# nirschl-lab/stain2stain

Hardware: AMD Instinct MI355X
Metric: paired 256x256 stain tiles/sec (full CFM optimisation step) (higher is better)
Workload: dtype bf16

## Files before the change

include/stain2stain_hip.h:

```cpp
#ifndef STAIN2STAIN_HIP_H
#define STAIN2STAIN_HIP_H

#ifdef __cplusplus
extern "C" {
#endif

#define S2S_OK 0
#define S2S_ERR_SHAPE (-1)
#define S2S_ERR_ALIGN (-2)
#define S2S_ERR_DTYPE (-3)
#define S2S_ERR_LAUNCH (-4)
#define S2S_ERR_NULL (-5)

#define S2S_BF16 0
#define S2S_F32 1

int s2s_conv3x3_stat_blocks(int dtype, int B, int H, int W, int Cout);
int s2s_conv3x3_nhwc(int dtype, const void* x0, int ld0, int c0, const void* x1, int ld1, int c1,
                     const void* w_packed, const float* bias, void* y, int ldy, float* stat_part,
                     const float* ep_scale, const float* ep_shift, int relu, int B, int H, int W, int Cout,
                     void* stream);

int s2s_conv3x3_ksplit(int dtype, int B, int H, int W, int Cout, int cin);
int s2s_conv3x3_nhwc_k(int dtype, const void* x0, int ld0, int c0, const void* x1, int ld1, int c1,
                       const void* w_packed, const float* bias, void* y, int ldy, float* stat_part,
                       const float* ep_scale, const float* ep_shift, int relu, float* kwork, int B, int H, int W,
                       int Cout, void* stream);
int s2s_conv3x3_stat_rows(int dtype, int B, int H, int W, int Cout, int c0, int c1, int ld0, int ld1, int has_bias);
int s2s_conv3x3_staged(int dtype, int B, int H, int W, int Cout, int c0, int c1, int ld0, int ld1, int ldy, int stats);
int s2s_conv3x3_family(int dtype, int B, int H, int W, int Cout, int c0, int c1, int ld0, int ld1, int ldy, int has_bias,
                       int has_affine, int stats, int stat_rows, int kwork);
int s2s_conv3x3_nhwc_s(int dtype, const void* x0, int ld0, int c0, const void* x1, int ld1, int c1, const void* w_packed,
                       const float* bias, void* y, int ldy, float* stat_part, int stat_rows, const float* ep_scale,
                       const float* ep_shift, int relu, float* kwork, int B, int H, int W, int Cout, void* stream);
int s2s_debug_conv_clock(long* out_host, int n);

int s2s_conv3x3_wgrad_splits(int dtype, int B, int H, int W, int Cin, int Cout);
int s2s_conv3x3_wgrad_nhwc(int dtype, const void* dy, int lddy, int Cout, const void* x0, int ld0, int c0,
                           const void* x1, int ld1, int c1, float* part, float* grad_oihw, int accumulate,
                           int B, int H, int W, void* stream);
int s2s_conv3x3_wgrad_phase(int dtype, const void* dy, int lddy, int Cout, const void* x0, int ld0, int c0,
                            const void* x1, int ld1, int c1, float* part, float* grad_oihw, int accumulate,
                            int B, int H, int W, int phases, void* stream);

int s2s_stem_stat_blocks(int B, int H, int W);
int s2s_stem_conv3x3_fwd(int dtype, const float* x_nchw, const float* w_oihw, const float* bias, void* y, int ldy,
                         float* stat_part, int B, int H, int W, int Cin, int Cout, void* stream);
int s2s_stem_wgrad_blocks(int B, int H, int W);
int s2s_stem_conv3x3_wgrad(int dtype, const void* dy, int lddy, const float* x_nchw, float* part, float* dw_oihw,
                           float* dbias, int accumulate, int B, int H, int W, int Cin, int Cout, void* stream);
int s2s_head_conv1x1_fwd(int dtype, const void* x, int ldx, const float* w, const float* bias, float* y_nchw, int B,
                         int H, int W, int C, int Cout, void* stream);
int s2s_head_wgrad_blocks(int B, int H, int W);
int s2s_head_conv1x1_bwd(int dtype, const float* dy_nchw, const void* x, int ldx, const float* w, void* dx, int lddx,
                         float* part, float* dw, float* dbias, int accumulate, int B, int H, int W, int C, int Cout,
                         void* stream);

int s2s_head_loss_blocks(int B, int H, int W);
int s2s_head_loss_fused(int dtype, const void* x, int ldx, const float* w, const float* bias, const float* u_nchw,
                        float* v_nchw, void* dx, int lddx, float grad_scale, float* part, double* lpart, float* dw,
                        float* dbias, float* loss, int accumulate, int B, int H, int W, int C, int Cout, void* stream);

int s2s_bn_finalize(const float* part, int nblk, int C, long count, const float* gamma, const float* beta,
                    float* running_mean, float* running_var, long* num_batches_tracked, float momentum, float eps,
                    float* mean, float* invstd, float* scale, float* shift, void* stream);
int s2s_bn_finalize_b(const float* part, int nblk, int C, long count, const float* gamma, const float* beta,
                      float* running_mean, float* running_var, long* num_batches_tracked, float momentum, float eps,
                      float* mean, float* invstd, float* scale, float* shift, const float* conv_bias, void* stream);
int s2s_bn_eval_prepare(int C, const float* gamma, const float* beta, const float* running_mean,
                        const float* running_var, float eps, float* scale, float* shift, void* stream);
int s2s_bn_relu_apply(int dtype, const void* x, int ldx, const float* scale, const float* shift, void* y, int ldy,
                      void* pool, int ldp, int B, int H, int W, int C, void* stream);
int s2s_maxpool2(int dtype, const void* x, int ldx, void* pool, int ldp, int B, int H, int W, int C, void* stream);
int s2s_bn_bwd_blocks(int B, int H, int W, int C);
int s2s_bn_relu_bwd(int dtype, const void* g1, int ldg1, const void* gp, int ldgp, const float* scale,
                    const float* shift, const void* x, int ldx, const float* mean, const float* invstd, const float* gamma, float* dgamma,
                    float* dbeta, float* dbias_conv, int accumulate, void* dx, int lddx, float* work, int B, int H,
                    int W, int C, void* stream);
int s2s_bn_partial_sums(const float* part, int nblk, int C, float* sums, void* stream);
int s2s_bn_relu_bwd_phase(int dtype, const void* g1, int ldg1, const void* gp, int ldgp, const float* scale,
                          const float* shift, const void* x, int ldx, const float* mean, const float* invstd,
                          const float* gamma, float* dgamma, float* dbeta, float* dbias_conv, int accumulate, void* dx,
                          int lddx, float* work, int B, int H, int W, int C, long count_total, int phases, void* stream);

int s2s_upsample2x_bilinear_ac_fwd(int dtype, const void* x, int ldx, const float* bias_nc, void* y, int ldy, int B,
                                   int Hin, int Win, int Hout, int Wout, int C, void* stream);
int s2s_upsample2x_bilinear_ac_bwd(int dtype, const void* dy, int lddy, void* dx, int lddx, int B, int Hin, int Win,
                                   int Hout, int Wout, int C, void* stream);
int s2s_pixel_sum(int dtype, const void* x, int ldx, float* out_nc, int B, int HW, int C, int accumulate,
                  void* stream);

int s2s_time_embedding(const float* t, float* out, int B, int dim, void* stream);
int s2s_linear_fwd(const float* x, const float* w, const float* bias, float* y, int B, int K, int N, void* stream);
int s2s_linear_bwd(const float* dy, const float* x, const float* w, float* dx, float* dw, float* db, int accumulate,
                   int B, int K, int N, void* stream);
int s2s_silu_fwd(const float* h, float* a, int n, void* stream);
int s2s_silu_bwd(const float* h, const float* da, float* dh, int n, void* stream);
int s2s_cfm_sample(const float* x0, const float* x1, const float* t, const float* eps, float sigma, float* xt,
                   float* ut, int B, long per_sample, void* stream);
int s2s_mse_loss(const float* v, const float* u, float* dv, float grad_scale, float* loss, double* work, long count,
                 void* stream);
int s2s_ode_error_norm(const float* e, const float* y0, const float* y1, float atol, float rtol, float* out,
                       double* work, long n, void* stream);
int s2s_axpy(float* x, const float* y, float a, long n, void* stream);
int s2s_dp_partials(long n);
int s2s_dp_init(int phase, const float* y, const float* k1, const float* fa, double* state, double* part, float* out,
                float* t_out, int* status, float atol, float rtol, int B, long n, void* stream);
int s2s_dp_stage(int i, const float* y, const float* k1, const float* k2, const float* k3, const float* k4,
                 const float* k5, const float* k6, const double* state, float* out, float* t_out, int B, long n,
                 void* stream);
int s2s_dp_error(const float* k1, const float* k2, const float* k3, const float* k4, const float* k5, const float* k6,
                 const float* k7, const float* y, const float* y_new, const double* state, double* part, float atol,
                 float rtol, int B, long n, void* stream);
int s2s_dp_control(double* state, const double* part, int* status, int max_steps, int B, long n, void* stream);
int s2s_dp_commit(float* y, const float* y_new, float* k1, const float* k7, const double* state, int B, long n,
                  void* stream);
int s2s_rk_stage(const float* x, const float* k1, const float* k2, const float* k3, float c1, float c2, float c3, int nk,
                 float* out, float* t_out, const float* table, const int* counter, int stages, int stage, int table_len,
                 int B, long n, void* stream);
int s2s_rk_combine(float* x, const float* k1, const float* k2, const float* k3, const float* k4, float c1, float c2,
                   float c3, float c4, int nk, int* counter, int B, long n, void* stream);
int s2s_fill_f32(float* x, float v, long n, void* stream);
int s2s_euler_tick(float* t, int n, const float* table, int* counter, void* stream);

int s2s_adam_step(float* p, const float* g, float* m, float* v, long n, int step, float lr, float beta1, float beta2,
                  float eps, float weight_decay, float grad_scale, void* stream);
int s2s_adam_step_dev(float* p, const float* g, float* m, float* v, long n, const float* hyper, void* stream);
long s2s_adam_multi_blocks(long n);
int s2s_adam_multi(const void* desc, int ntensors, long total, int step, float lr, float beta1, float beta2, float eps,
                   float weight_decay, float grad_scale, void* stream);
int s2s_adam_ema_step(float* p, const float* g, float* m, float* v, float* ema, long n, int step, float lr, float beta1,
                      float beta2, float eps, float weight_decay, float grad_scale, float ema_weight, void* stream);
int s2s_adam_ema_step_dev(float* p, const float* g, float* m, float* v, float* ema, long n, const float* hyper,
                          const float* ema_weight, void* stream);
long s2s_ema_multi_blocks(long n);
int s2s_ema_multi(const void* desc, int ntensors, long total, const float* weight, void* stream);
long s2s_pack_conv3x3_fwd_elems(int Cout, int Cin);
long s2s_pack_conv3x3_dgrad_elems(int Cout, int Cin);
int s2s_pack_conv3x3(int dtype, const float* w_oihw, void* w_fwd, void* w_dgrad, int Cout, int Cin, void* stream);
int s2s_pack_conv3x3_batched(int dtype, const void* desc, int nlayers, long total, void* stream);
int s2s_nchw_to_nhwc(int dtype, const float* x_nchw, void* y, int ldy, int B, int C, int H, int W, void* stream);
int s2s_nhwc_to_nchw(int dtype, const void* x, int ldx, float* y_nchw, int accumulate, int B, int C, int H, int W,
                     void* stream);

int s2s_paired_crop_flip_normalize(const void* src_u8, const void* tgt_u8, const int* params, float* out_src,
                                   float* out_tgt, int B, int Hs, int Ws, int S, void* stream);
int s2s_pil_resize_bilinear_normalize(const void* src_u8, void* tmp_u8, const int* bounds_h, const int* kk_h,
                                      int ksize_h, const int* bounds_v, const int* kk_v, int ksize_v, void* out_u8,
                                      float* out_f, int B, int Hs, int Ws, int Ho, int Wo, void* stream);

int s2s_region_gather(const void* img_u8, long pitch, int H, int W, int band_top, int band_h, const int* origins,
                      float* out, int B, int T, void* stream);
int s2s_region_blend(const float* tiles, int c0, const float* tiles1, int c1, const int* origins, int n, int T,
                     int overlap, float* acc, int band_rows, int H, int W, int r0, int r1, void* stream);
int s2s_region_finalize(float* acc, int band_rows, int W, int C, int r0, int r1, void* out_u8, long pitch_u8,
                        float* out_f, long pitch_f, int out_top, void* stream);

int s2s_region_tissue_count(const void* img_u8, long pitch, int H, int W, int band_top, int band_h, const int* origins,
                            int n, int T, int white, int black, int* counts, void* stream);
int s2s_region_skip_weight(const int* origins, int n, int T, int overlap, float* ws, int band_rows, int H, int W,
                           int r0, int r1, void* stream);
int s2s_region_finalize_mixed(float* acc, float* ws, int band_rows, int W, int C, int r0, int r1, const void* src_u8,
                              long src_pitch, int src_top, void* out_u8, long pitch_u8, float* out_f, long pitch_f,
                              int out_top, void* stream);

int s2s_seg_loss(const float* z, const float* g, float* dz, float* out, double* work, long n, float smooth,
                 float dice_weight, float grad_scale, void* stream);
int s2s_seg_loss_multiclass(const float* z, const long* target, float* dz, float* out, double* work, long B, long HW,
                            int C, int ignore_index, float smooth, float dice_weight, float grad_scale, void* stream);

int s2s_seg_eval_binary(const float* z, const float* g, float* out, long* counts, double* work, long n, float smooth,
                        float dice_weight, void* stream);
int s2s_seg_eval_multiclass(const float* z, const long* target, float* out, long* counts, double* work, long B,
                            long HW, int C, int ignore_index, float smooth, float dice_weight, void* stream);
int s2s_head_mse_eval_blocks(int B, int H, int W, int C);
int s2s_head_mse_eval(int dtype, const void* x, int ldx, const float* w, const float* bias, const float* u_nchw,
                      float* loss, double* lpart, int B, int H, int W, int C, int Cout, void* stream);

int s2s_image_quality_blocks(int H, int W, int win);
int s2s_image_quality_f32(const float* a, const float* b, int B, int C, int H, int W, int quantize, int win,
                          const float* taps, float k1, float k2, double* part, void* stream);
int s2s_image_quality_u8(const void* a, long pitch_a, long img_a, const void* b, long pitch_b, long img_b, int B,
                         int band_top, int band_h, int H, int W, int by0, int nby, int win, const float* taps, float k1,
                         float k2, double* part, void* stream);
int s2s_image_quality_finalize(const double* part, int B, int C, int H, int W, int win, float range, float* out,
                               void* stream);

int s2s_stain_quant_chunks(int cell_h, int cell_w);
int s2s_stain_quant_u8(const void* a, long pitch_a, long img_a, const void* b, long pitch_b, long img_b, int paired,
                       int B, int band_top, int band_h, int H, int W, int cell_h, int cell_w, int g0, int ng,
                       const float* od_table, const float* unmix, int white, int black, int stain, double* part,
                       void* stream);
int s2s_stain_quant_f32(const float* a, const float* b, int paired, int B, int H, int W, const float* od_table,
                        const float* unmix, int white, int black, int stain, double* part, void* stream);
int s2s_stain_quant_finalize(const double* part, long owners, int nchunk, int paired, long* counts, double* sums,
                             float* out, void* stream);
int s2s_stain_separate(const void* img, int is_f32, long pitch, long img_stride, int B, int H, int W,
                       const float* od_table, const float* unmix, float* out, void* stream);

int s2s_weighted_mse(const float* v, const float* u, const float* mask, float* dv, float* out, double* work, long B,
                     int C, long HW, float roi_lambda, float grad_scale, void* stream);
int s2s_charbonnier_roi(const float* pred, const float* truth, const float* mask, float* out, double* work, long B,
                        int C, long HW, float eps_charb, float eps_area, void* stream);
int s2s_class_embed_add(const float* temb, const float* table, const long* y, float* out, int B, int dim,
                        void* stream);
int s2s_class_embed_bwd(const float* dout, const long* y, float* dtable, int accumulate, int B, int dim,
                        int num_classes, void* stream);

int s2s_instnorm_blocks(int B, int H, int W, int C);
int s2s_instnorm_lrelu_fwd(int dtype, const void* x, int ldx, const float* gamma, const float* beta, void* y, int ldy,
                           float* work, float* stats, int B, int H, int W, int C, float eps, float slope,
                           void* stream);
int s2s_instnorm_lrelu_bwd(int dtype, const void* g, int ldg, const void* x, int ldx, const float* stats, void* dx,
                           int lddx, float* dgamma, float* dbeta, int accumulate, float* work, int B, int H, int W,
                           int C, float slope, void* stream);

int s2s_conv2x2_stat_blocks(int B, int H, int W, int Cout);
int s2s_conv2x2_nhwc(int dtype, const void* x, int ldx, int cin, const void* w_packed, const float* bias, void* y,
                     int ldy, float* stat_part, int B, int H, int W, int Cout, int pad, void* stream);
int s2s_space_to_depth_pad1(int dtype, const void* x, int ldx, void* xs, int ldxs, int inverse, int B, int H, int W,
                            int C, void* stream);
int s2s_channel_sum_blocks(long npix, int C);
int s2s_channel_sum(int dtype, const void* x, int ldx, float* work, float* out, long npix, int C, int accumulate,
                    void* stream);
int s2s_pack_conv4x4(const float* w_oihw, void* wf, void* wd, int Cout, int Cin, int stride, void* stream);
int s2s_conv4x4s1_nhwc(int dtype, const void* x, int ldx, int cin, const void* w_packed, const float* bias, void* y,
                       int ldy, float* stat_part, int B, int H, int W, int Cout, int pad, void* stream);
int s2s_conv4x4s1_wgrad_splits(int B, int H, int W, int Cin, int Cout);
int s2s_conv4x4s1_wgrad_nhwc(int dtype, const void* dy, int lddy, int Cout, const void* x, int ldx, int cin,
                             float* part, float* grad16, int accumulate, int B, int H, int W, void* stream);
int s2s_conv2x2_wgrad_splits(int B, int H, int W, int Cin, int Cout);
int s2s_conv2x2_wgrad_nhwc(int dtype, const void* dy, int lddy, int Cout, const void* x, int ldx, int cin, float* part,
                           float* grad2, int accumulate, int B, int H, int W, void* stream);

int s2s_convkxk_stat_blocks(int dtype, int B, int H, int W, int Cout, int ks);
int s2s_convkxk_nhwc(int dtype, const void* x, int ldx, int cin, const void* w_packed, const float* bias, int bias_mod,
                     void* y, int ldy, void* y2, int ldy2, int act, float act_slope, float* stat_part, float* kwork, int B,
                     int H, int W, int Cout, int ks, int pad, void* stream);
int s2s_convkxk_ksplit(int dtype, int B, int H, int W, int Cout, int cin, int ks);
int s2s_convkxk_wgrad_splits(int dtype, int B, int H, int W, int Cin, int Cout, int ks);
int s2s_convkxk_wgrad_nhwc(int dtype, const void* dy, int lddy, int Cout, const void* x, int ldx, int cin, float* part,
                           float* grad, int layout, int accumulate, int B, int H, int W, int ks, int x_plain, void* stream);
int s2s_conv4x4s2_ksplit(int B, int H, int W, int Cout, int Cin);
int s2s_conv4x4s2_nhwc(int dtype, const void* x, int ldx, int Cin, const void* wf, const float* bias, void* y, int ldy,
                       void* y2, int ldy2, int act, float act_slope, float* kwork, int B, int H, int W, int Cout,
                       void* stream);
int s2s_convt4x4s2_ksplit(int B, int h, int w, int C, int Cin);
int s2s_convt4x4s2_nhwc(int dtype, const void* x, int ldx, int Cin, const void* wd, const float* bias, void* y, int ldy,
                        float* kwork, int B, int h, int w, int C, void* stream);
int s2s_convsm_ok(int dtype, int mode, int B, int h, int w, int Cin, int Cout);
int s2s_convsm_nhwc(int dtype, int mode, const void* x, int ldx, int Cin, const void* w_packed, const float* bias, int epi,
                    int act, float slope, float eps, void* raw, int ldraw, void* y, int ldy, void* y2, int ldy2,
                    float* stats, const float* stats_in, const void* z, int ldz, const void* g2, int ldg2, int bwd_c0,
                    int B, int h, int w, int Cout, void* stream);
int s2s_instnorm_lrelu_fwd2(int dtype, const void* x, int ldx, const float* gamma, const float* beta, void* y, int ldy,
                            void* y2, int ldy2, float* work, float* stats, int B, int H, int W, int C, float eps,
                            float slope, void* stream);
int s2s_instnorm_lrelu_bwd2(int dtype, const void* g, int ldg, const void* g2, int ldg2, const void* x, int ldx,
                            const float* stats, void* dx, int lddx, float* dgamma, float* dbeta, int accumulate,
                            float* work, int B, int H, int W, int C, float slope, void* stream);
int s2s_instnorm_split_ok(int dtype, int H, int W, int C);
int s2s_instnorm_lrelu_fwd_split(int dtype, const float* slabs, int S, const float* bias, void* raw, int ldraw, void* y,
                                 int ldy, void* y2, int ldy2, float* stats, int B, int H, int W, int C, float eps,
                                 float slope, void* stream);
int s2s_instnorm_lrelu_bwd_split(int dtype, const float* gslabs, int S, const void* g2, int ldg2, const void* x, int ldx,
                                 const float* stats, void* dx, int lddx, int B, int H, int W, int C, float slope,
                                 void* stream);
int s2s_pack_conv4x4_t(int dtype, const float* w_oihw, void* wf, void* wd, int Cout, int Cin, int stride, void* stream);
long s2s_pack_conv4x4_blocks(int Cout, int Cin, int stride);
int s2s_pack_conv4x4_batched(int dtype, const void* desc, int nlayers, long total, void* stream);
int s2s_p2p_pack_input(int dtype, const float* a_nchw, int ca, const float* b_nchw, int cb, void* out, int ldo, int B,
                       int H, int W, void* stream);
int s2s_p2p_unpack(int dtype, const void* in, int ldi, int c0, int C, float* out_nchw, int B, int H, int W, void* stream);
int s2s_p2p_tanh_l1_blocks(int B, int H, int W);
int s2s_p2p_tanh_l1_fwd(int dtype, const void* h, int ldh, const float* src_nchw, const float* tgt_nchw, void* d_in,
                        int ldd, float* fake_nchw, float* l1_out, void* work, int B, int H, int W, int C, void* stream);
int s2s_p2p_tanh_l1_bwd(int dtype, const void* h, int ldh, const float* tgt_nchw, const void* gd, int ldg, float l1_scale,
                        void* dh, int lddh, int B, int H, int W, int C, void* stream);
int s2s_p2p_bce_logits(int dtype, const void* z, int ldz, int n_real, float w_real, float w_fake, void* dz, int lddz,
                       float* out2, int N, int HW, void* stream);
int s2s_p2p_bce_blocks(int N, int HW);
int s2s_p2p_bce_logits_w(int dtype, const void* z, int ldz, int n_real, float w_real, float w_fake, void* dz, int lddz,
                         float* out2, double* work, int N, int HW, void* stream);
int s2s_p2p_act_bwd_blocks(long npix, int C);
int s2s_p2p_act_bwd(int dtype, const void* g, int ldg, const void* g2, int ldg2, const void* a, int lda, float slope,
                    void* dz, int lddz, float* work, float* dbias, int accumulate, long npix, int C, void* stream);

int s2s_stream_create_cu_mask(const unsigned* mask_words, int n_words, long* out_stream);
int s2s_stream_destroy(void* stream);
int s2s_event_create(int timing_only, long* out_event);
int s2s_event_record(void* event, void* stream);
int s2s_event_elapsed_ms(void* start, void* stop, float* out_ms);
int s2s_event_synchronize(void* event);
int s2s_event_destroy(void* event);

#ifdef __cplusplus
}
#endif
#endif
```

stain2stain_amd/csrc/conv_edge.hip:

```cpp
#include "common.h"

namespace {

constexpr int STEM_MAX_CIN = 8;

typedef __attribute__((address_space(3))) s16x4 lds_s16x4;

__device__ __forceinline__ bf16x8 tr_frag8(const char* p) {
  s16x4 lo = __builtin_amdgcn_ds_read_tr16_b64_v4i16((lds_s16x4*)(p));
  s16x4 hi = __builtin_amdgcn_ds_read_tr16_b64_v4i16((lds_s16x4*)(p + 4 * 64));
  bf16x4 l4 = __builtin_bit_cast(bf16x4, lo), h4 = __builtin_bit_cast(bf16x4, hi);
  bf16x8 r;
#pragma unroll
  for (int i = 0; i < 4; ++i) { r[i] = l4[i]; r[4 + i] = h4[i]; }
  return r;
}

template <int NIMG>
__device__ __forceinline__ void split_store(char* base, int img_stride, int off, const float* v8) {
  bf16x8 h, m, l;
#pragma unroll
  for (int i = 0; i < 8; ++i) {
    h[i] = (bf16_t)v8[i];
    const float r1 = v8[i] - (float)h[i];
// ... 302 lines not shown
        for (int k = 0; k < 8; ++k) ab[k] = (bf16_t)a.v[k];
        *reinterpret_cast<bf16x8*>(al + threadIdx.x * AS + c8) = ab;
#pragma unroll
        for (int o = 0; o < HEAD_MAX_COUT; ++o)
          if (o < Cout)
#pragma unroll
            for (int k = 0; k < 8; ++k) vv[o] = fmaf(a.v[k], wl[o * C + c8 + k], vv[o]);
      }
      const long n = p / HW, q = p - n * HW;
#pragma unroll
      for (int o = 0; o < HEAD_MAX_COUT; ++o)
        if (o < Cout) {
          const float vo = vv[o] + (bias ? bias[o] : 0.f);
          const long idx = (n * Cout + o) * HW + q;
          if (v_out) v_out[idx] = vo;
          const float d = vo - u[idx];
          lsum += (double)(d * d);
          g[o] = coef * d;
        }
      for (int c8 = 0; c8 < C; c8 += 8) {
        f32x8 da;
#pragma unroll
        for (int k = 0; k < 8; ++k) {
          float s = 0.f;
#pragma unroll
          for (int o = 0; o < HEAD_MAX_COUT; ++o)
            if (o < Cout) s = fmaf(g[o], wl[o * C + c8 + k], s);
          da.v[k] = s;
        }
        store8(dx + p * lddx + c8, da);
      }
    } else {
      for (int c8 = 0; c8 < C; c8 += 8) {
        bf16x8 z;
#pragma unroll
        for (int k = 0; k < 8; ++k) z[k] = (bf16_t)0.f;
        *reinterpret_cast<bf16x8*>(al + threadIdx.x * AS + c8) = z;
      }
    }
#pragma unroll
    for (int o = 0; o < HEAD_MAX_COUT; ++o) gl[threadIdx.x * HEAD_MAX_COUT + o] = g[o];
    __syncthreads();
#pragma unroll
    for (int i = 0; i < 4; ++i) {
      const int id = threadIdx.x + i * 256;
      if (id < nout) {
        const int o = id / (C + 1), c = id - o * (C + 1);
        float a = acc[i];
        if (c < C) for (int pp = 0; pp < 256; ++pp) a = fmaf(gl[pp * HEAD_MAX_COUT + o], (float)al[pp * AS + c], a);
        else for (int pp = 0; pp < 256; ++pp) a += gl[pp * HEAD_MAX_COUT + o];
        acc[i] = a;
      }
    }
    __syncthreads();
  }
#pragma unroll
  for (int i = 0; i < 4; ++i) {
    const int id = threadIdx.x + i * 256;
    if (id < nout) part[(long)blockIdx.x * nout + id] = acc[i];
  }
  lred[threadIdx.x] = lsum;
  __syncthreads();
  for (int o = 128; o > 0; o >>= 1) {
    if (threadIdx.x < o) lred[threadIdx.x] += lred[threadIdx.x + o];
    __syncthreads();
  }
  if (threadIdx.x == 0) lpart[blockIdx.x] = lred[0];
}

template <typename T, int PCB>
__global__ __launch_bounds__(256) void head_loss_lanes_kernel(const T* __restrict__ x, int ldx,
                                                              const float* __restrict__ w,
                                                              const float* __restrict__ bias,
                                                              const float* __restrict__ u, float* __restrict__ v_out,
                                                              T* __restrict__ dx, int lddx, float coef,
                                                              float* __restrict__ part, double* __restrict__ lpart,
                                                              long npix, int HW, int Cout) {
  constexpr int C = PCB * 8, PPB = 256 / PCB, MO = HEAD_MAX_COUT;
  __shared__ float fold[256][MO * 8 + 1];
  __shared__ float dbf[PPB][MO];
  __shared__ double lred[256];
  const int tid = threadIdx.x, pc = tid & (PCB - 1), slot = tid / PCB;
  const int lane = tid & 63, grp0 = lane & ~(PCB - 1);
  float wr[MO][8], bo[MO];
#pragma unroll
  for (int o = 0; o < MO; ++o) {
    bo[o] = (o < Cout && bias) ? bias[o] : 0.f;
#pragma unroll
    for (int k = 0; k < 8; ++k) wr[o][k] = o < Cout ? w[o * C + pc * 8 + k] : 0.f;
  }
  float dwacc[MO][8], dbacc[MO];
#pragma unroll
  for (int o = 0; o < MO; ++o) {
    dbacc[o] = 0.f;
#pragma unroll
    for (int k = 0; k < 8; ++k) dwacc[o][k] = 0.f;
  }
  double lsum = 0.0;
  const int np = (int)npix, stride = (int)gridDim.x * PPB;
  f32x8 a_next;
  {
    const int pf = (int)blockIdx.x * PPB + slot;
#pragma unroll
    for (int k = 0; k < 8; ++k) a_next.v[k] = 0.f;
    if (pf < np) a_next = load8(x + (long)pf * ldx + pc * 8);
  }
  for (int p0 = (int)blockIdx.x * PPB; p0 < np; p0 += stride) {
    const int p = p0 + slot;
    const bool ok = p < np;
    const f32x8 a = a_next;
    {
      const int pn = p + stride;
#pragma unroll
      for (int k = 0; k < 8; ++k) a_next.v[k] = 0.f;
      if (p0 + stride < np && pn < np) a_next = load8(x + (long)pn * ldx + pc * 8);
    }
    float vv[MO];
#pragma unroll
    for (int o = 0; o < MO; ++o) {
      float t = 0.f;
#pragma unroll
      for (int k = 0; k < 8; ++k) t = fmaf(a.v[k], wr[o][k], t);
#pragma unroll
      for (int m = 1; m < PCB; m <<= 1) t += __shfl_xor(t, m, 64);
      vv[o] = t + bo[o];
    }
    const int n = p / HW, q = p - n * HW;
    float gm[MO];
#pragma unroll
    for (int o = 0; o < MO; ++o) {
      gm[o] = 0.f;
      if (ok && o < Cout && (o & (PCB - 1)) == pc) {
        const long idx = ((long)n * Cout + o) * HW + q;
        if (v_out) v_out[idx] = vv[o];
        const float d = vv[o] - u[idx];
        lsum += (double)(d * d);
        gm[o] = coef * d;
      }
    }
    float g[MO];
#pragma unroll
    for (int o = 0; o < MO; ++o) g[o] = __shfl(gm[o], grp0 + (o & (PCB - 1)), 64);
    if (ok) {
      f32x8 da;
#pragma unroll
      for (int k = 0; k < 8; ++k) {
        float t = 0.f;
#pragma unroll
        for (int o = 0; o < MO; ++o) t = fmaf(g[o], wr[o][k], t);
        da.v[k] = t;
      }
      store8(dx + (long)p * lddx + pc * 8, da);
    }
#pragma unroll
    for (int o = 0; o < MO; ++o) {
      if (pc == 0) dbacc[o] += g[o];
#pragma unroll
      for (int k = 0; k < 8; ++k) dwacc[o][k] = fmaf(g[o], a.v[k], dwacc[o][k]);
    }
  }
#pragma unroll
  for (int o = 0; o < MO; ++o) {
#pragma unroll
    for (int k = 0; k < 8; ++k) fold[tid][o * 8 + k] = dwacc[o][k];
    if (pc == 0) dbf[slot][o] = dbacc[o];
  }
  lred[tid] = lsum;
  __syncthreads();
  const int nout = Cout * (C + 1);
  for (int id = tid; id < nout; id += 256) {
    const int o = id / (C + 1), c = id - o * (C + 1);
    float t = 0.f;
    if (c < C) {
      const int cp = c >> 3, k = c & 7;
      for (int sl = 0; sl < PPB; ++sl) t += fold[sl * PCB + cp][o * 8 + k];
    } else {
      for (int sl = 0; sl < PPB; ++sl) t += dbf[sl][o];
    }
    part[(long)blockIdx.x * nout + id] = t;
  }
  for (int o = 128; o > 0; o >>= 1) {
    if (tid < o) lred[tid] += lred[tid + o];
    __syncthreads();
  }
  if (tid == 0) lpart[blockIdx.x] = lred[0];
}

template <typename T, int PCB, bool FWD>
__global__ __launch_bounds__(256) void head_lanes_kernel(const T* __restrict__ x, int ldx, const float* __restrict__ w,
                                                         const float* __restrict__ bias, const float* __restrict__ dy,
                                                         float* __restrict__ v_out, T* __restrict__ dx, int lddx,
                                                         float* __restrict__ part, long npix, int HW, int Cout) {
  constexpr int C = PCB * 8, PPB = 256 / PCB, MO = HEAD_MAX_COUT;
  __shared__ float fold[FWD ? 1 : 256][MO * 8 + 1];
  __shared__ float dbf[PPB][MO];
  const int tid = threadIdx.x, pc = tid & (PCB - 1), slot = tid / PCB;
  const int lane = tid & 63, grp0 = lane & ~(PCB - 1);
  float wr[MO][8], bo[MO];
#pragma unroll
  for (int o = 0; o < MO; ++o) {
    bo[o] = (o < Cout && bias) ? bias[o] : 0.f;
#pragma unroll
    for (int k = 0; k < 8; ++k) wr[o][k] = o < Cout ? w[o * C + pc * 8 + k] : 0.f;
  }
  float dwacc[MO][8], dbacc[MO];
#pragma unroll
  for (int o = 0; o < MO; ++o) {
    dbacc[o] = 0.f;
#pragma unroll
    for (int k = 0; k < 8; ++k) dwacc[o][k] = 0.f;
  }
  const int np = (int)npix, stride = (int)gridDim.x * PPB;
  f32x8 a_next;
  {
    const int pf = (int)blockIdx.x * PPB + slot;
#pragma unroll
    for (int k = 0; k < 8; ++k) a_next.v[k] = 0.f;
    if (pf < np) a_next = load8(x + (long)pf * ldx + pc * 8);
  }
  for (int p0 = (int)blockIdx.x * PPB; p0 < np; p0 += stride) {
    const int p = p0 + slot;
    const bool ok = p < np;
    const f32x8 a = a_next;
    {
      const int pn = p + stride;
#pragma unroll
      for (int k = 0; k < 8; ++k) a_next.v[k] = 0.f;
      if (p0 + stride < np && pn < np) a_next = load8(x + (long)pn * ldx + pc * 8);
    }
    const int n = p / HW, q = p - n * HW;
    if (FWD) {
#pragma unroll
      for (int o = 0; o < MO; ++o) {
        float t = 0.f;
#pragma unroll
        for (int k = 0; k < 8; ++k) t = fmaf(a.v[k], wr[o][k], t);
#pragma unroll
        for (int m = 1; m < PCB; m <<= 1) t += __shfl_xor(t, m, 64);
        if (ok && o < Cout && (o & (PCB - 1)) == pc) v_out[((long)n * Cout + o) * HW + q] = t + bo[o];
      }
    } else {
      float gm[MO], g[MO];
#pragma unroll
      for (int o = 0; o < MO; ++o) {
        gm[o] = 0.f;
        if (ok && o < Cout && (o & (PCB - 1)) == pc) gm[o] = dy[((long)n * Cout + o) * HW + q];
      }
#pragma unroll
      for (int o = 0; o < MO; ++o) g[o] = __shfl(gm[o], grp0 + (o & (PCB - 1)), 64);
      if (ok) {
        f32x8 da;
#pragma unroll
        for (int k = 0; k < 8; ++k) {
          float t = 0.f;
#pragma unroll
          for (int o = 0; o < MO; ++o) t = fmaf(g[o], wr[o][k], t);
          da.v[k] = t;
        }
        store8(dx + (long)p * lddx + pc * 8, da);
      }
#pragma unroll
      for (int o = 0; o < MO; ++o) {
        if (pc == 0) dbacc[o] += g[o];
#pragma unroll
        for (int k = 0; k < 8; ++k) dwacc[o][k] = fmaf(g[o], a.v[k], dwacc[o][k]);
      }
    }
  }
  if (FWD) return;
#pragma unroll
  for (int o = 0; o < MO; ++o) {
#pragma unroll
    for (int k = 0; k < 8; ++k) fold[tid][o * 8 + k] = dwacc[o][k];
    if (pc == 0) dbf[slot][o] = dbacc[o];
  }
  __syncthreads();
  const int nout = Cout * (C + 1);
  for (int id = tid; id < nout; id += 256) {
    const int o = id / (C + 1), c = id - o * (C + 1);
    float t = 0.f;
    if (c < C) {
      const int cp = c >> 3, k = c & 7;
      for (int sl = 0; sl < PPB; ++sl) t += fold[sl * PCB + cp][o * 8 + k];
    } else {
      for (int sl = 0; sl < PPB; ++sl) t += dbf[sl][o];
    }
    part[(long)blockIdx.x * nout + id] = t;
  }
}

template <typename T, bool FWD>
bool launch_head_lanes(const void* x, int ldx, const float* w, const float* bias, const float* dy, float* v, void* dx,
                       int lddx, float* part, int nb, long npix, int HW, int C, int Cout, hipStream_t s) {
  if (Cout > HEAD_MAX_COUT || (C % 8) || npix >= (1L << 31) - (1L << 20)) return false;
#define S2S_HLN(PP)                                                                                                  \
  hipLaunchKernelGGL((head_lanes_kernel<T, PP, FWD>), dim3(nb), dim3(256), 0, s, (const T*)x, ldx, w, bias, dy, v,   \
                     (T*)dx, lddx, part, npix, HW, Cout);                                                            \
  return true;
  switch (C / 8) {
    case 1: S2S_HLN(1) case 2: S2S_HLN(2) case 4: S2S_HLN(4) case 8: S2S_HLN(8) case 16: S2S_HLN(16) case 32: S2S_HLN(32)
    case 64: S2S_HLN(64) default: return false;
  }
#undef S2S_HLN
}

__global__ __launch_bounds__(256) void loss_finalize_kernel(const double* part, int n, double inv_count, float* loss) {
  __shared__ double red[256];
  double s = 0.0;
  for (int i = threadIdx.x; i < n; i += 256) s += part[i];
  red[threadIdx.x] = s;
  __syncthreads();
  for (int o = 128; o > 0; o >>= 1) {
    if (threadIdx.x < o) red[threadIdx.x] += red[threadIdx.x + o];
    __syncthreads();
  }
  if (threadIdx.x == 0) *loss = (float)(red[0] * inv_count);
}

}

int s2s_internal_stem_fwd(int dtype, const float* x_nchw, const float* w_oihw, const float* bias, void* y, int ldy,
                          float* stat_part, int B, int H, int W, int Cin, int Cout, hipStream_t s);

extern "C" int s2s_stem_stat_blocks(int B, int H, int W) {
  if (B <= 0 || H <= 0 || W <= 0) return S2S_ERR_SHAPE;
  return B * cdiv(H, 16) * cdiv(W, 16);
}

extern "C" int s2s_stem_conv3x3_fwd(int dtype, const float* x_nchw, const float* w_oihw, const float* bias, void* y,
                                    int ldy, float* stat_part, int B, int H, int W, int Cin, int Cout, void* stream) {
  if (!x_nchw || !w_oihw || !y) return S2S_ERR_NULL;
  if (B <= 0 || H <= 0 || W <= 0 || Cin <= 0 || Cin > 6 || Cout <= 0 || (Cout % 8) || (ldy % 8))
    return S2S_ERR_SHAPE;
  return s2s_internal_stem_fwd(dtype, x_nchw, w_oihw, bias, y, ldy, stat_part, B, H, W, Cin, Cout,
                               (hipStream_t)stream);
}

extern "C" int s2s_stem_wgrad_blocks(int B, int H, int W) {
  if (B <= 0 || H <= 0 || W <= 0) return S2S_ERR_SHAPE;
  const int nt = B * cdiv(H, 16) * cdiv(W, 16);
  constexpr int cap = 512;
  return nt < cap ? nt : cap;
}

extern "C" int s2s_stem_conv3x3_wgrad(int dtype, const void* dy, int lddy, const float* x_nchw, float* part,
                                      float* dw_oihw, float* dbias, int accumulate, int B, int H, int W, int Cin,
                                      int Cout, void* stream) {
  if (!dy || !x_nchw || !part || !dw_oihw) return S2S_ERR_NULL;
  if (B <= 0 || H <= 0 || W <= 0 || Cin <= 0 || Cin > 6 || Cout <= 0 || (Cout % 8) || (lddy % 8))
    return S2S_ERR_SHAPE;
  const int nb = s2s_stem_wgrad_blocks(B, H, W);
  hipStream_t s = (hipStream_t)stream;
  dim3 grid(nb, cdiv(Cout, 64), cdiv(Cin, 3));
  if (dtype == S2S_BF16) {
    const int lds = 1 * (2 * 256 * 64 + 256 * 64) + 3 * 324 * 4;
    hipLaunchKernelGGL(stem_wgrad_kernel<bf16_t>, grid, dim3(256), lds, s, (const bf16_t*)dy, lddy, x_nchw, part, B,
                       H, W, Cin, Cout, cdiv(H, 16), cdiv(W, 16));
  } else if (dtype == S2S_F32) {
    const int lds = 3 * (2 * 256 * 64 + 256 * 64) + 3 * 324 * 4;
    static unsigned long long attr_devs = 0;
    if (int rc = s2s_allow_dyn_lds(reinterpret_cast<const void*>(stem_wgrad_kernel<float>), lds, &attr_devs)) return rc;
    hipLaunchKernelGGL(stem_wgrad_kernel<float>, grid, dim3(256), lds, s, (const float*)dy, lddy, x_nchw, part, B, H,
                       W, Cin, Cout, cdiv(H, 16), cdiv(W, 16));
  } else return S2S_ERR_DTYPE;
  hipLaunchKernelGGL(stem_wgrad_reduce_kernel, dim3(Cout, cdiv(Cin, 3)), dim3(1024), 0, s, part, 2 * nb, Cout, Cin, dw_oihw, dbias,
                     accumulate);
  S2S_LAUNCH_CHECK();
  return S2S_OK;
}

extern "C" int s2s_head_conv1x1_fwd(int dtype, const void* x, int ldx, const float* w, const float* bias,
                                    float* y_nchw, int B, int H, int W, int C, int Cout, void* stream) {
  if (!x || !w || !y_nchw) return S2S_ERR_NULL;
  if (B <= 0 || H <= 0 || W <= 0 || C <= 0 || (C % 8) || (ldx % 8) || Cout <= 0 || Cout > HEAD_WIDE_COUT)
    return S2S_ERR_SHAPE;
  const long npix = (long)B * H * W;
  long grid = (npix + 255) / 256;
  if (grid > 4096) grid = 4096;
  hipStream_t s = (hipStream_t)stream;
  if (dtype != S2S_BF16 && dtype != S2S_F32) return S2S_ERR_DTYPE;
  {
    const int nbl = (int)(((npix + 255) / 256) < 2048 ? ((npix + 255) / 256) : 2048);
    const bool done = dtype == S2S_BF16
        ? launch_head_lanes<bf16_t, true>(x, ldx, w, bias, nullptr, y_nchw, nullptr, 8, nullptr, nbl, npix, H * W, C, Cout, s)
        : launch_head_lanes<float, true>(x, ldx, w, bias, nullptr, y_nchw, nullptr, 8, nullptr, nbl, npix, H * W, C, Cout, s);
    if (done) { S2S_LAUNCH_CHECK(); return S2S_OK; }
  }
#define S2S_HEAD_FWD(TT, MO)                                                                                        \
  hipLaunchKernelGGL((head_fwd_kernel<TT, MO>), dim3((int)grid), dim3(256), Cout * C * 4, s, (const TT*)x, ldx, w, \
                     bias, y_nchw, npix, H * W, C, Cout)
  if (dtype == S2S_BF16) { if (Cout <= 4) S2S_HEAD_FWD(bf16_t, 4); else S2S_HEAD_FWD(bf16_t, 8); }
  else if (dtype == S2S_F32) { if (Cout <= 4) S2S_HEAD_FWD(float, 4); else S2S_HEAD_FWD(float, 8); }
  else return S2S_ERR_DTYPE;
#undef S2S_HEAD_FWD
  S2S_LAUNCH_CHECK();
  return S2S_OK;
}

extern "C" int s2s_head_wgrad_blocks(int B, int H, int W) {
  if (B <= 0 || H <= 0 || W <= 0) return S2S_ERR_SHAPE;
  const long nb = ((long)B * H * W + 63) / 64;
  return (int)(nb < 512 ? nb : 512);
}

extern "C" int s2s_head_conv1x1_bwd(int dtype, const float* dy_nchw, const void* x, int ldx, const float* w, void* dx,
                                    int lddx, float* part, float* dw, float* dbias, int accumulate, int B, int H, int W,
                                    int C, int Cout, void* stream) {
  if (!dy_nchw || !x || !w || !dx || !part || !dw) return S2S_ERR_NULL;
  if (B <= 0 || H <= 0 || W <= 0 || C <= 0 || (C % 8) || (ldx % 8) || (lddx % 8) || Cout <= 0 || Cout > HEAD_WIDE_COUT)
    return S2S_ERR_SHAPE;
  if (Cout * (C + 1) > 2048) return S2S_ERR_SHAPE;
  const long npix = (long)B * H * W;
  long grid = (npix + 255) / 256;
  if (grid > 4096) grid = 4096;
  const int nb = s2s_head_wgrad_blocks(B, H, W);
  const int mo = Cout <= 4 ? 4 : 8;
  const int lds = (64 * (C + 1) + 64 * mo) * 4;
  hipStream_t s = (hipStream_t)stream;
  if (dtype != S2S_BF16 && dtype != S2S_F32) return S2S_ERR_DTYPE;
  {
    const bool done = dtype == S2S_BF16
        ? launch_head_lanes<bf16_t, false>(x, ldx, w, nullptr, dy_nchw, nullptr, dx, lddx, part, nb, npix, H * W, C, Cout, s)
        : launch_head_lanes<float, false>(x, ldx, w, nullptr, dy_nchw, nullptr, dx, lddx, part, nb, npix, H * W, C, Cout, s);
    if (done) {
      hipLaunchKernelGGL(head_wgrad_reduce_kernel, dim3(cdiv(Cout * (C + 1), 8)), dim3(256), 0, s, part, nb, Cout, C,
                         dw, dbias, accumulate);
      S2S_LAUNCH_CHECK();
      return S2S_OK;
    }
  }
#define S2S_HEAD_BWD(TT, MO)                                                                                       \
  hipLaunchKernelGGL((head_bwd_data_kernel<TT, MO>), dim3((int)grid), dim3(256), Cout * C * 4, s, dy_nchw, w,      \
                     (TT*)dx, lddx, npix, H * W, C, Cout);                                                         \
  hipLaunchKernelGGL((head_wgrad_kernel<TT, MO>), dim3(nb), dim3(256), lds, s, dy_nchw, (const TT*)x, ldx, part,   \
                     npix, H * W, C, Cout);
  if (dtype == S2S_BF16) { if (mo == 4) { S2S_HEAD_BWD(bf16_t, 4) } else { S2S_HEAD_BWD(bf16_t, 8) } }
  else if (dtype == S2S_F32) { if (mo == 4) { S2S_HEAD_BWD(float, 4) } else { S2S_HEAD_BWD(float, 8) } }
  else return S2S_ERR_DTYPE;
#undef S2S_HEAD_BWD
  hipLaunchKernelGGL(head_wgrad_reduce_kernel, dim3(cdiv(Cout * (C + 1), 8)), dim3(256), 0, s, part, nb, Cout, C,
                     dw, dbias, accumulate);
  S2S_LAUNCH_CHECK();
  return S2S_OK;
}

extern "C" int s2s_head_loss_blocks(int B, int H, int W) {
  if (B <= 0 || H <= 0 || W <= 0) return S2S_ERR_SHAPE;
  const long nb = ((long)B * H * W + 255) / 256;
  return (int)(nb < 1024 ? nb : 1024);
}

extern "C" int s2s_head_loss_fused(int dtype, const void* x, int ldx, const float* w, const float* bias,
                                   const float* u_nchw, float* v_nchw, void* dx, int lddx, float grad_scale,
                                   float* part, double* lpart, float* dw, float* dbias, float* loss, int accumulate,
                                   int B, int H, int W, int C, int Cout, void* stream) {
  if (!x || !w || !u_nchw || !dx || !part || !lpart || !dw || !loss) return S2S_ERR_NULL;
  if (B <= 0 || H <= 0 || W <= 0 || C <= 0 || (C % 8) || (ldx % 8) || (lddx % 8) || Cout <= 0 || Cout > HEAD_MAX_COUT)
    return S2S_ERR_SHAPE;
  if (Cout * (C + 1) > 1024) return S2S_ERR_SHAPE;
  const long npix = (long)B * H * W;
  if (npix >= (1L << 31) - (1L << 20)) return S2S_ERR_SHAPE;
  const double count = (double)npix * Cout;
  const int nb = s2s_head_loss_blocks(B, H, W);
  const int lds = (HEAD_MAX_COUT * C + 256 * HEAD_MAX_COUT) * 4 + 256 * (C + 8) * 2;
  if (lds > 60 * 1024) return S2S_ERR_SHAPE;
  hipStream_t s = (hipStream_t)stream;
  const float coef = (float)(2.0 * (double)grad_scale / count);
  if (dtype != S2S_BF16 && dtype != S2S_F32) return S2S_ERR_DTYPE;
  const int pcb = C / 8;
  bool done = false;
#define S2S_HL(TT, PP)                                                                                              \
  hipLaunchKernelGGL((head_loss_lanes_kernel<TT, PP>), dim3(nb), dim3(256), 0, s, (const TT*)x, ldx, w, bias, u_nchw, \
                     v_nchw, (TT*)dx, lddx, coef, part, lpart, npix, H * W, Cout);                                 \
  done = true;
#define S2S_HL_T(TT)                                                                                    \
  switch (pcb) {                                                                                        \
    case 1: { S2S_HL(TT, 1) } break;  case 2: { S2S_HL(TT, 2) } break;  case 4: { S2S_HL(TT, 4) } break;    \
    case 8: { S2S_HL(TT, 8) } break;  case 16: { S2S_HL(TT, 16) } break; case 32: { S2S_HL(TT, 32) } break;  \
    case 64: { S2S_HL(TT, 64) } break; default: break;                                                  \
  }
  if (dtype == S2S_BF16) { S2S_HL_T(bf16_t) } else { S2S_HL_T(float) }
#undef S2S_HL_T
#undef S2S_HL
  if (!done) {
    if (dtype == S2S_BF16)
      hipLaunchKernelGGL(head_loss_fused_kernel<bf16_t>, dim3(nb), dim3(256), lds, s, (const bf16_t*)x, ldx, w, bias,
                         u_nchw, v_nchw, (bf16_t*)dx, lddx, coef, part, lpart, npix, H * W, C, Cout);
    else
      hipLaunchKernelGGL(head_loss_fused_kernel<float>, dim3(nb), dim3(256), lds, s, (const float*)x, ldx, w, bias,
                         u_nchw, v_nchw, (float*)dx, lddx, coef, part, lpart, npix, H * W, C, Cout);
  }
  hipLaunchKernelGGL(head_wgrad_reduce_kernel, dim3(cdiv(Cout * (C + 1), 8)), dim3(256), 0, s, part, nb, Cout, C,
                     dw, dbias, accumulate);
  hipLaunchKernelGGL(loss_finalize_kernel, dim3(1), dim3(256), 0, s, lpart, nb, 1.0 / count, loss);
  S2S_LAUNCH_CHECK();
  return S2S_OK;
}
```

stain2stain_amd/csrc/norm_act.hip:

```cpp
#include "common.h"
#include <type_traits>

namespace {

constexpr int RED_ROWS = 8;

constexpr int PRE_R = 16;
__global__ __launch_bounds__(1024) void prereduce_rows_kernel(float* __restrict__ part, int nrows, int ncols) {
  __shared__ double s1[32][33];
  const int cl = threadIdx.x & 31, rg = threadIdx.x >> 5;
  const int c = blockIdx.x * 32 + cl, r = blockIdx.y;
  double a = 0.0;
  if (c < ncols)
    for (int i = r + PRE_R * rg; i < nrows; i += PRE_R * 32) a += (double)part[(long)i * ncols + c];
  s1[rg][cl] = a;
  __syncthreads();
  if (rg == 0 && c < ncols) {
    for (int k = 1; k < 32; ++k) a += s1[k][cl];
    part[(long)r * ncols + c] = (float)a;
  }
}

inline int prereduce(float* part, int nrows, int ncols, hipStream_t s) {
  if (nrows <= 4 * PRE_R) return nrows;
// ... 86 lines not shown
  const int cp = C >> 3;
  const int Hw = (H + 1) >> 1, Ww = (W + 1) >> 1, Hp = H >> 1, Wp = W >> 1;
  const long total = (long)B * Hw * Ww * cp;
  for (long i = (long)blockIdx.x * blockDim.x + threadIdx.x; i < total; i += (long)gridDim.x * blockDim.x) {
    const int c8 = (int)(i % cp) * 8;
    long t = i / cp;
    const int wx = (int)(t % Ww); t /= Ww;
    const int wy = (int)(t % Hw);
    const int n = (int)(t / Hw);
    float sc[8], sh[8], mx[8];
#pragma unroll
    for (int k = 0; k < 8; ++k) { sc[k] = scale[c8 + k]; sh[k] = shift[c8 + k]; mx[k] = 0.f; }
#pragma unroll
    for (int dy = 0; dy < 2; ++dy)
#pragma unroll
      for (int dx = 0; dx < 2; ++dx) {
        const int yy = wy * 2 + dy, xx = wx * 2 + dx;
        if (yy < H && xx < W) {
          const long pix = ((long)n * H + yy) * W + xx;
          f32x8 v = load8(x + pix * ldx + c8);
#pragma unroll
          for (int k = 0; k < 8; ++k) {
            v.v[k] = fmaxf(fmaf(v.v[k], sc[k], sh[k]), 0.f);
            const float st = to_f32(from_f32<T>(v.v[k]));
            mx[k] = fmaxf(mx[k], st);
          }
          store8(y + pix * ldy + c8, v);
        }
      }
    if (pool && wy < Hp && wx < Wp) {
      f32x8 m;
#pragma unroll
      for (int k = 0; k < 8; ++k) m.v[k] = mx[k];
      store8(pool + (((long)n * Hp + wy) * Wp + wx) * ldp + c8, m);
    }
  }
}

template <typename T>
__global__ void maxpool2_kernel(const T* __restrict__ x, int ldx, T* __restrict__ pool, int ldp, int B, int H,
                                int W, int C) {
  const int cp = C >> 3, Hp = H >> 1, Wp = W >> 1;
  const long total = (long)B * Hp * Wp * cp;
  for (long i = (long)blockIdx.x * blockDim.x + threadIdx.x; i < total; i += (long)gridDim.x * blockDim.x) {
    const int c8 = (int)(i % cp) * 8;
    long t = i / cp;
    const int wx = (int)(t % Wp); t /= Wp;
    const int wy = (int)(t % Hp);
    const int n = (int)(t / Hp);
    f32x8 m;
#pragma unroll
    for (int k = 0; k < 8; ++k) m.v[k] = -INFINITY;
#pragma unroll
    for (int dy = 0; dy < 2; ++dy)
#pragma unroll
      for (int dx = 0; dx < 2; ++dx) {
        const long pix = ((long)n * H + wy * 2 + dy) * W + wx * 2 + dx;
        const f32x8 v = load8(x + pix * ldx + c8);
#pragma unroll
        for (int k = 0; k < 8; ++k) m.v[k] = fmaxf(m.v[k], v.v[k]);
      }
    store8(pool + (((long)n * Hp + wy) * Wp + wx) * ldp + c8, m);
  }
}

typedef __attribute__((ext_vector_type(8))) float f32x8v;
template <typename T> struct Vec8;
template <> struct Vec8<bf16_t> { typedef bf16x8 type; };
template <> struct Vec8<float> { typedef f32x8v type; };

__device__ __forceinline__ bf16x8 vload8(const bf16_t* p) { return *reinterpret_cast<const bf16x8*>(p); }
__device__ __forceinline__ f32x8v vload8(const float* p) {
  const f32x4 a = *reinterpret_cast<const f32x4*>(p), b = *reinterpret_cast<const f32x4*>(p + 4);
  return __builtin_shufflevector(a, b, 0, 1, 2, 3, 4, 5, 6, 7);
}
__device__ __forceinline__ void vstore8(bf16_t* p, bf16x8 v) { *reinterpret_cast<bf16x8*>(p) = v; }
__device__ __forceinline__ void vstore8(float* p, f32x8v v) {
  *reinterpret_cast<f32x4*>(p) = __builtin_shufflevector(v, v, 0, 1, 2, 3);
  *reinterpret_cast<f32x4*>(p + 4) = __builtin_shufflevector(v, v, 4, 5, 6, 7);
}

template <typename T>
struct WindowGrad {
  typedef typename Vec8<T>::type V;
  V x0, x1, x2, x3, g0, g1v, g2, g3, pr;
  int okmask;
  __device__ __forceinline__ void load(const T* __restrict__ g1, int ldg1, const T* __restrict__ gp, int ldgp,
                                       const T* __restrict__ x, int ldx, int n, int wy, int wx, int H, int W,
                                       int c8) {
    const int Hp = H >> 1, Wp = W >> 1;
    const V zero = {};
    const int yy = wy * 2, xx = wx * 2;
    const bool r1 = yy + 1 < H, c1 = xx + 1 < W;
    okmask = 1 | (c1 ? 2 : 0) | (r1 ? 4 : 0) | ((r1 && c1) ? 8 : 0);
    const long p00 = ((long)n * H + yy) * W + xx;
    x0 = vload8(x + p00 * ldx + c8);
    x1 = c1 ? vload8(x + (p00 + 1) * ldx + c8) : zero;
    x2 = r1 ? vload8(x + (p00 + W) * ldx + c8) : zero;
    x3 = (r1 && c1) ? vload8(x + (p00 + W + 1) * ldx + c8) : zero;
    if (g1) {
      g0 = vload8(g1 + p00 * ldg1 + c8);
      g1v = c1 ? vload8(g1 + (p00 + 1) * ldg1 + c8) : zero;
      g2 = r1 ? vload8(g1 + (p00 + W) * ldg1 + c8) : zero;
      g3 = (r1 && c1) ? vload8(g1 + (p00 + W + 1) * ldg1 + c8) : zero;
    } else {
      g0 = zero; g1v = zero; g2 = zero; g3 = zero;
    }
    const bool pooled = gp && wy < Hp && wx < Wp;
    okmask |= pooled ? 16 : 0;
    pr = pooled ? vload8(gp + (((long)n * Hp + wy) * Wp + wx) * ldgp + c8) : zero;
  }
  __device__ __forceinline__ bool ok(int q) const { return (okmask >> q) & 1; }
  __device__ __forceinline__ void eval(int k, float sc, float sh, float mu, float is, float (&dz)[4],
                                       float (&xh)[4]) const {
    const float b[4] = {(float)x0[k], (float)x1[k], (float)x2[k], (float)x3[k]};
    dz[0] = (float)g0[k]; dz[1] = (float)g1v[k]; dz[2] = (float)g2[k]; dz[3] = (float)g3[k];
    float yv[4];
#pragma unroll
    for (int q = 0; q < 4; ++q) {
      yv[q] = ok(q) ? to_f32(from_f32<T>(fmaxf(fmaf(b[q], sc, sh), 0.f))) : 0.f;
      xh[q] = ok(q) ? (b[q] - mu) * is : 0.f;
    }
    if (okmask & 16) {
      int best = 0;
      float bv = yv[0];
#pragma unroll
      for (int q = 1; q < 4; ++q)
        if (yv[q] > bv) { bv = yv[q]; best = q; }
      const float p = (float)pr[k];
#pragma unroll
      for (int q = 0; q < 4; ++q) dz[q] += (q == best) ? p : 0.f;
    }
#pragma unroll
    for (int q = 0; q < 4; ++q)
      if (!(yv[q] > 0.f)) dz[q] = 0.f;
  }
};

__device__ __forceinline__ int pcb_of(int C) {
  int p = 1;
  while (p < 32 && p * 8 < C) p <<= 1;
  return p;
}

template <typename T>
__global__ __launch_bounds__(256) void bn_relu_bwd_reduce_kernel(const T* g1, int ldg1, const T* gp, int ldgp, const float* scale, const float* shift,
                                          const T* x, int ldx, const float* mean, const float* invstd,
                                          float* part, int B, int H, int W, int C) {
  const int Hw = (H + 1) >> 1, Ww = (W + 1) >> 1;
  const long nwin = (long)B * Hw * Ww;
  const int PCB = pcb_of(C), WL = 256 / PCB;
  const int pc = threadIdx.x & (PCB - 1), wl = threadIdx.x / PCB;
  const int c8 = (blockIdx.x * PCB + pc) * 8;
  using Acc = typename std::conditional<std::is_same<T, float>::value, double, float>::type;
  Acc s1[8], s2[8];
#pragma unroll
  for (int k = 0; k < 8; ++k) { s1[k] = 0; s2[k] = 0; }
  __shared__ float kc[4][256];
  for (int i = threadIdx.x; i < PCB * 8; i += 256) {
    const int c = blockIdx.x * PCB * 8 + i;
    const bool in = c < C;
    kc[0][i] = in ? scale[c] : 0.f; kc[1][i] = in ? shift[c] : 0.f;
    kc[2][i] = in ? mean[c] : 0.f;  kc[3][i] = in ? invstd[c] : 0.f;
  }
  __syncthreads();
  if (c8 < C) {
    for (int w = blockIdx.y * WL + wl; w < (int)nwin; w += gridDim.y * WL) {
      const int t1 = w / Ww, wx = w - t1 * Ww;
      const int n = t1 / Hw, wy = t1 - n * Hw;
      WindowGrad<T> wg;
      wg.load(g1, ldg1, gp, ldgp, x, ldx, n, wy, wx, H, W, c8);
#pragma unroll
      for (int k = 0; k < 8; ++k) {
        float dz[4], xh[4];
        const int ci = pc * 8 + k;
        wg.eval(k, kc[0][ci], kc[1][ci], kc[2][ci], kc[3][ci], dz, xh);
        float a = 0.f, b = 0.f;
#pragma unroll
        for (int q = 0; q < 4; ++q) { a += dz[q]; b += dz[q] * xh[q]; }
        s1[k] += (Acc)a;
        s2[k] += (Acc)b;
        __builtin_amdgcn_sched_barrier(0);
      }
    }
  }
  __shared__ Acc red[2][2304];
  const int rowlen = PCB * 8 + 1;
#pragma unroll
  for (int k = 0; k < 8; ++k) { red[0][wl * rowlen + pc * 8 + k] = s1[k]; red[1][wl * rowlen + pc * 8 + k] = s2[k]; }
  __syncthreads();
  for (int i = threadIdx.x; i < 2 * PCB * 8; i += 256) {
    const int which = i / (PCB * 8), cl = i - which * (PCB * 8);
    Acc s = 0;
    for (int r = 0; r < WL; ++r) s += red[which][r * rowlen + cl];
    const int c = blockIdx.x * PCB * 8 + cl;
    if (c < C) part[((long)which * C + c) * gridDim.y + blockIdx.y] = (float)s;
  }
}

template <int TPC>
__global__ __launch_bounds__(256) void bn_bwd_finalize_kernel(const float* part, int nblk, int C, double count, float* dgamma,
                                       float* dbeta, int accumulate, float* c1, float* c2, float* zero_out) {
  const int c = blockIdx.x * (256 / TPC) + threadIdx.x / TPC, li = threadIdx.x % TPC;
  if (c >= C) return;
  double a, b;
  channel_sums<TPC>(part, nblk, C, c, li, a, b);
  if (li == 0) {
    dbeta[c] = accumulate ? dbeta[c] + (float)a : (float)a;
    dgamma[c] = accumulate ? dgamma[c] + (float)b : (float)b;
    c1[c] = (float)(a / count);
    c2[c] = (float)(b / count);
    if (zero_out) zero_out[c] = 0.f;
  }
}

template <typename T>
__global__ __launch_bounds__(256) void bn_relu_bwd_apply_kernel(const T* g1, int ldg1, const T* gp, int ldgp, const float* scale, const float* shift,
                                         const T* x, int ldx, const float* mean, const float* invstd,
                                         const float* gamma, const float* c1, const float* c2, T* dx, int lddx,
                                         float* dxsum_part, int B, int H, int W, int C) {
  const int Hw = (H + 1) >> 1, Ww = (W + 1) >> 1;
  const long nwin = (long)B * Hw * Ww;
  const int PCB = pcb_of(C), WL = 256 / PCB;
  const int pc = threadIdx.x & (PCB - 1), wl = threadIdx.x / PCB;
  const int c8 = (blockIdx.x * PCB + pc) * 8;
  float s[8];
#pragma unroll
  for (int k = 0; k < 8; ++k) s[k] = 0.f;
  __shared__ float kc[7][256];
  for (int i = threadIdx.x; i < PCB * 8; i += 256) {
    const int c = blockIdx.x * PCB * 8 + i;
    const bool in = c < C;
    kc[0][i] = in ? scale[c] : 0.f; kc[1][i] = in ? shift[c] : 0.f;
    kc[2][i] = in ? mean[c] : 0.f;  kc[3][i] = in ? invstd[c] : 0.f;
    kc[4][i] = in ? gamma[c] * invstd[c] : 0.f;
    kc[5][i] = in ? c1[c] : 0.f;    kc[6][i] = in ? c2[c] : 0.f;
  }
  __syncthreads();
  if (c8 < C) {
    for (int w = blockIdx.y * WL + wl; w < (int)nwin; w += gridDim.y * WL) {
      const int t1 = w / Ww, wx = w - t1 * Ww;
      const int n = t1 / Hw, wy = t1 - n * Hw;
      WindowGrad<T> wg;
      wg.load(g1, ldg1, gp, ldgp, x, ldx, n, wy, wx, H, W, c8);
      typename Vec8<T>::type o0, o1, o2, o3;
#pragma unroll
      for (int k = 0; k < 8; ++k) {
        float dz[4], xh[4];
        const int ci = pc * 8 + k;
        wg.eval(k, kc[0][ci], kc[1][ci], kc[2][ci], kc[3][ci], dz, xh);
        const float gak = kc[4][ci], k1k = kc[5][ci], k2k = kc[6][ci];
        float v[4];
#pragma unroll
        for (int q = 0; q < 4; ++q) {
          v[q] = gak * (dz[q] - k1k - xh[q] * k2k);
          if (wg.ok(q)) s[k] += v[q];
        }
        o0[k] = from_f32<T>(v[0]); o1[k] = from_f32<T>(v[1]); o2[k] = from_f32<T>(v[2]); o3[k] = from_f32<T>(v[3]);
        __builtin_amdgcn_sched_barrier(0);
      }
      T* const d00 = dx + (((long)n * H + wy * 2) * W + wx * 2) * lddx + c8;
      vstore8(d00, o0);
      if (wg.ok(1)) vstore8(d00 + lddx, o1);
      if (wg.ok(2)) vstore8(d00 + (long)W * lddx, o2);
      if (wg.ok(3)) vstore8(d00 + (long)(W + 1) * lddx, o3);
    }
  }
  if (dxsum_part) {
    __shared__ float red[2304];
    const int rowlen = PCB * 8 + 1;
#pragma unroll
    for (int k = 0; k < 8; ++k) red[wl * rowlen + pc * 8 + k] = s[k];
    __syncthreads();
    for (int cl = threadIdx.x; cl < PCB * 8; cl += 256) {
      float t = 0.f;
      for (int r = 0; r < WL; ++r) t += red[r * rowlen + cl];
      const int c = blockIdx.x * PCB * 8 + cl;
      if (c < C) dxsum_part[(long)blockIdx.y * C + c] = t;
    }
  }
}

template <typename T>
__global__ __launch_bounds__(256) void bn_relu_bwd_reduce_flat_kernel(const T* __restrict__ g1, int ldg1, const float* __restrict__ scale, const float* __restrict__ shift,
                                               const T* __restrict__ x, int ldx, const float* mean, const float* invstd,
                                               float* part, long npix, int C) {
  const int PCB = pcb_of(C), WL = 256 / PCB;
  const int pc = threadIdx.x & (PCB - 1), wl = threadIdx.x / PCB;
  const int c8 = (blockIdx.x * PCB + pc) * 8;
  using Acc = typename std::conditional<std::is_same<T, float>::value, double, float>::type;
  Acc s1[8], s2[8];
#pragma unroll
  for (int k = 0; k < 8; ++k) { s1[k] = 0; s2[k] = 0; }
  if (c8 < C) {
    float mu[8], is[8], sc[8], sh[8];
#pragma unroll
    for (int k = 0; k < 8; ++k) { mu[k] = mean[c8 + k]; is[k] = invstd[c8 + k]; sc[k] = scale[c8 + k]; sh[k] = shift[c8 + k]; }
    for (long p = (long)blockIdx.y * WL + wl; p < npix; p += (long)gridDim.y * WL) {
      const f32x8 g = load8(g1 + p * ldg1 + c8);
      const f32x8 b = load8(x + p * ldx + c8);
#pragma unroll
      for (int k = 0; k < 8; ++k) {
        const float dz = fmaf(b.v[k], sc[k], sh[k]) > 0.f ? g.v[k] : 0.f;
        s1[k] += (Acc)dz;
        s2[k] += (Acc)(dz * ((b.v[k] - mu[k]) * is[k]));
      }
    }
  }
  __shared__ Acc red[2][2304];
  const int rowlen = PCB * 8 + 1;
#pragma unroll
  for (int k = 0; k < 8; ++k) { red[0][wl * rowlen + pc * 8 + k] = s1[k]; red[1][wl * rowlen + pc * 8 + k] = s2[k]; }
  __syncthreads();
  for (int i = threadIdx.x; i < 2 * PCB * 8; i += 256) {
    const int which = i / (PCB * 8), cl = i - which * (PCB * 8);
    Acc s = 0;
    for (int r = 0; r < WL; ++r) s += red[which][r * rowlen + cl];
    const int c = blockIdx.x * PCB * 8 + cl;
    if (c < C) part[((long)which * C + c) * gridDim.y + blockIdx.y] = (float)s;
  }
}

template <typename T>
__global__ __launch_bounds__(256) void bn_relu_bwd_apply_flat_kernel(const T* __restrict__ g1, int ldg1, const float* __restrict__ scale, const float* __restrict__ shift,
                                              const T* __restrict__ x, int ldx, const float* mean, const float* invstd,
                                              const float* gamma, const float* c1, const float* c2, T* __restrict__ dx,
                                              int lddx, float* dxsum_part, long npix, int C, int rev) {
  const int PCB = pcb_of(C), WL = 256 / PCB;
  const int pc = threadIdx.x & (PCB - 1), wl = threadIdx.x / PCB;
  const int c8 = (blockIdx.x * PCB + pc) * 8;
  float s[8];
#pragma unroll
  for (int k = 0; k < 8; ++k) s[k] = 0.f;
  if (c8 < C) {
    float ga[8], k1[8], k2[8], mu[8], is[8], sc[8], sh[8];
#pragma unroll
    for (int k = 0; k < 8; ++k) {
      mu[k] = mean[c8 + k]; is[k] = invstd[c8 + k]; sc[k] = scale[c8 + k]; sh[k] = shift[c8 + k];
      ga[k] = gamma[c8 + k] * is[k]; k1[k] = c1[c8 + k]; k2[k] = c2[c8 + k];
    }
    const long p0 = (long)blockIdx.y * WL + wl, pstep = (long)gridDim.y * WL;
    const long nit = p0 < npix ? (npix - p0 + pstep - 1) / pstep : 0;
    for (long it = 0; it < nit; ++it) {
      const long p = p0 + (rev ? nit - 1 - it : it) * pstep;
      const f32x8 g = load8(g1 + p * ldg1 + c8);
      const f32x8 b = load8(x + p * ldx + c8);
      f32x8 o;
#pragma unroll
      for (int k = 0; k < 8; ++k) {
        const float dz = fmaf(b.v[k], sc[k], sh[k]) > 0.f ? g.v[k] : 0.f;
        o.v[k] = ga[k] * (dz - k1[k] - ((b.v[k] - mu[k]) * is[k]) * k2[k]);
        s[k] += o.v[k];
      }
      store8(dx + p * lddx + c8, o);
    }
  }
  if (dxsum_part) {
    __shared__ float red[2304];
    const int rowlen = PCB * 8 + 1;
#pragma unroll
    for (int k = 0; k < 8; ++k) red[wl * rowlen + pc * 8 + k] = s[k];
    __syncthreads();
    for (int cl = threadIdx.x; cl < PCB * 8; cl += 256) {
      float t = 0.f;
      for (int r = 0; r < WL; ++r) t += red[r * rowlen + cl];
      const int c = blockIdx.x * PCB * 8 + cl;
      if (c < C) dxsum_part[(long)blockIdx.y * C + c] = t;
    }
  }
}

__global__ __launch_bounds__(1024) void colsum_finalize_kernel(const float* part, int nblk, int C, float* out, int accumulate) {
  __shared__ double s1[32][33];
  const int cl = threadIdx.x & 31, rg = threadIdx.x >> 5;
  const int c = blockIdx.x * 32 + cl;
  double a = 0.0;
  if (c < C)
    for (int i = rg; i < nblk; i += 32) a += (double)part[(long)i * C + c];
  s1[rg][cl] = a;
  __syncthreads();
  if (rg == 0 && c < C) {
    for (int k = 1; k < 32; ++k) a += s1[k][cl];
    out[c] = accumulate ? out[c] + (float)a : (float)a;
  }
}

inline int ew_grid(long total) {
  long b = (total + 255) / 256;
  if (b > 2048 * 4) b = 2048 * 4;
  if (b < 1) b = 1;
  return (int)b;
}

inline int host_pcb(int C) {
  int p = 1;
  while (p < 32 && p * 8 < C) p <<= 1;
  return p;
}

inline int red_blocks(int B, int H, int W, int C) {
  const long nwin = (long)B * ((H + 1) / 2) * ((W + 1) / 2);
  const int pcb = host_pcb(C), wl = 256 / pcb;
  long want = 1536 / cdiv(C / 8, pcb);
  if (want < 1) want = 1;
  long nb = (nwin + wl - 1) / wl;
  if (nb > want) nb = want;
  if (nb < 1) nb = 1;
  return (int)nb;
}

}

extern "C" int s2s_bn_finalize_b(const float* part, int nblk, int C, long count, const float* gamma,
                                 const float* beta, float* running_mean, float* running_var, long* num_batches,
                                 float momentum, float eps, float* mean, float* invstd, float* scale, float* shift,
                                 const float* conv_bias, void* stream) {
  if (!part || !gamma || !beta || !mean || !invstd || !scale || !shift) return S2S_ERR_NULL;
  if (nblk <= 0 || C <= 0 || count <= 0) return S2S_ERR_SHAPE;
  if (finalize_tpc(nblk) == 256)
    hipLaunchKernelGGL(bn_finalize_kernel<256>, dim3(C), dim3(256), 0, (hipStream_t)stream, part, nblk, C,
                       (double)count, gamma, beta, running_mean, running_var, num_batches, momentum, eps, mean,
                       invstd, scale, shift, conv_bias);
  else
    hipLaunchKernelGGL(bn_finalize_kernel<64>, dim3(cdiv(C, 4)), dim3(256), 0, (hipStream_t)stream, part, nblk, C,
                       (double)count, gamma, beta, running_mean, running_var, num_batches, momentum, eps, mean,
                       invstd, scale, shift, conv_bias);
  S2S_LAUNCH_CHECK();
  return S2S_OK;
}

extern "C" int s2s_bn_finalize(const float* part, int nblk, int C, long count, const float* gamma,
                               const float* beta, float* running_mean, float* running_var, long* num_batches,
                               float momentum, float eps, float* mean, float* invstd, float* scale, float* shift,
                               void* stream) {
  return s2s_bn_finalize_b(part, nblk, C, count, gamma, beta, running_mean, running_var, num_batches, momentum, eps, mean,
                           invstd, scale, shift, nullptr, stream);
}

extern "C" int s2s_bn_partial_sums(const float* part, int nblk, int C, float* sums, void* stream) {
  if (!part || !sums) return S2S_ERR_NULL;
  if (nblk <= 0 || C <= 0) return S2S_ERR_SHAPE;
  if (finalize_tpc(nblk) == 256)
    hipLaunchKernelGGL(bn_partial_sums_kernel<256>, dim3(C), dim3(256), 0, (hipStream_t)stream, part, nblk, C, sums);
  else
    hipLaunchKernelGGL(bn_partial_sums_kernel<64>, dim3(cdiv(C, 4)), dim3(256), 0, (hipStream_t)stream, part, nblk, C, sums);
  S2S_LAUNCH_CHECK();
  return S2S_OK;
}

extern "C" int s2s_bn_eval_prepare(int C, const float* gamma, const float* beta, const float* rmean,
                                   const float* rvar, float eps, float* scale, float* shift, void* stream) {
  if (!gamma || !beta || !rmean || !rvar || !scale || !shift) return S2S_ERR_NULL;
  if (C <= 0) return S2S_ERR_SHAPE;
  hipLaunchKernelGGL(bn_eval_prepare_kernel, dim3(cdiv(C, 256)), dim3(256), 0, (hipStream_t)stream, C, gamma, beta,
                     rmean, rvar, eps, scale, shift);
  S2S_LAUNCH_CHECK();
  return S2S_OK;
}

extern "C" int s2s_bn_relu_apply(int dtype, const void* x, int ldx, const float* scale, const float* shift, void* y,
                                 int ldy, void* pool, int ldp, int B, int H, int W, int C, void* stream) {
  if (!x || !scale || !shift || !y) return S2S_ERR_NULL;
  if (B <= 0 || H <= 0 || W <= 0 || C <= 0 || (C % 8) || (ldx % 8) || (ldy % 8) || (pool && (ldp % 8)))
    return S2S_ERR_SHAPE;
  const long total = (long)B * ((H + 1) / 2) * ((W + 1) / 2) * (C / 8);
  hipStream_t s = (hipStream_t)stream;
  if (dtype == S2S_BF16)
    hipLaunchKernelGGL(bn_relu_apply_kernel<bf16_t>, dim3(ew_grid(total)), dim3(256), 0, s, (const bf16_t*)x, ldx,
                       scale, shift, (bf16_t*)y, ldy, (bf16_t*)pool, ldp, B, H, W, C);
  else if (dtype == S2S_F32)
    hipLaunchKernelGGL(bn_relu_apply_kernel<float>, dim3(ew_grid(total)), dim3(256), 0, s, (const float*)x, ldx,
                       scale, shift, (float*)y, ldy, (float*)pool, ldp, B, H, W, C);
  else return S2S_ERR_DTYPE;
  S2S_LAUNCH_CHECK();
  return S2S_OK;
}

extern "C" int s2s_maxpool2(int dtype, const void* x, int ldx, void* pool, int ldp, int B, int H, int W, int C,
                            void* stream) {
  if (!x || !pool) return S2S_ERR_NULL;
  if (B <= 0 || H < 2 || W < 2 || C <= 0 || (C % 8) || (ldx % 8) || (ldp % 8)) return S2S_ERR_SHAPE;
  const long total = (long)B * (H / 2) * (W / 2) * (C / 8);
  hipStream_t s = (hipStream_t)stream;
  if (dtype == S2S_BF16)
    hipLaunchKernelGGL(maxpool2_kernel<bf16_t>, dim3(ew_grid(total)), dim3(256), 0, s, (const bf16_t*)x, ldx,
                       (bf16_t*)pool, ldp, B, H, W, C);
  else if (dtype == S2S_F32)
    hipLaunchKernelGGL(maxpool2_kernel<float>, dim3(ew_grid(total)), dim3(256), 0, s, (const float*)x, ldx,
                       (float*)pool, ldp, B, H, W, C);
  else return S2S_ERR_DTYPE;
  S2S_LAUNCH_CHECK();
  return S2S_OK;
}

extern "C" int s2s_bn_bwd_blocks(int B, int H, int W, int C) {
  if (B <= 0 || H <= 0 || W <= 0 || C <= 0) return S2S_ERR_SHAPE;
  return red_blocks(B, H, W, C);
}

extern "C" int s2s_bn_relu_bwd_phase(int dtype, const void* g1, int ldg1, const void* gp, int ldgp, const float* scale,
                               const float* shift, const void* x, int ldx, const float* mean, const float* invstd, const float* gamma,
                               float* dgamma, float* dbeta, float* dbias_conv, int accumulate, void* dx, int lddx,
                               float* work, int B, int H, int W, int C, long count_total, int phases, void* stream) {
  if (phases < 1 || phases > 3 || count_total < (long)B * H * W) return S2S_ERR_SHAPE;
  if ((!g1 && !gp) || !scale || !shift || !x || !mean || !invstd || !gamma || !dgamma || !dbeta || !dx || !work) return S2S_ERR_NULL;
  if (B <= 0 || H <= 0 || W <= 0 || C <= 0 || (C % 8) || (ldx % 8) || (lddx % 8) ||
      (g1 && (ldg1 % 8)) || (gp && (ldgp % 8)))
    return S2S_ERR_SHAPE;
  if ((long)B * ((H + 1) / 2) * ((W + 1) / 2) >= (1L << 31) - (1 << 20)) return S2S_ERR_SHAPE;
  const int nb = red_blocks(B, H, W, C);
  float* part = work;
  float* part2 = work + (long)nb * 2 * C;
  float* c1 = part2 + (long)nb * 2 * C;
  float* c2 = c1 + C;
  const double count = (double)count_total;
  hipStream_t s = (hipStream_t)stream;
  float* const dbias_zero = (dbias_conv && !accumulate) ? dbias_conv : nullptr;
  dbias_conv = nullptr;
  dim3 grid(cdiv(C / 8, host_pcb(C)), nb);
  constexpr int bn_rev = 1;
#define S2S_BN_BWD(TT)                                                                                             \
  if (!(phases & 1)) {                                                                                             \
  } else if (gp) {                                                                                                 \
    hipLaunchKernelGGL(bn_relu_bwd_reduce_kernel<TT>, grid, dim3(256), 0, s, (const TT*)g1, ldg1, (const TT*)gp,   \
                       ldgp, scale, shift, (const TT*)x, ldx, mean, invstd, part, B, H, W, C);                \
  } else {                                                                                                         \
    hipLaunchKernelGGL(bn_relu_bwd_reduce_flat_kernel<TT>, grid, dim3(256), 0, s, (const TT*)g1, ldg1,             \
                       scale, shift, (const TT*)x, ldx, mean, invstd, part, (long)B * H * W, C);              \
  }                                                                                                                \
  if (!(phases & 1)) {                                                                                             \
  } else if (finalize_tpc(nb) == 256)                                                                              \
    hipLaunchKernelGGL(bn_bwd_finalize_kernel<256>, dim3(C), dim3(256), 0, s, part, nb, C, count, dgamma, dbeta,   \
                       accumulate, c1, c2, dbias_zero);                                                            \
  else                                                                                                             \
    hipLaunchKernelGGL(bn_bwd_finalize_kernel<64>, dim3(cdiv(C, 4)), dim3(256), 0, s, part, nb, C, count, dgamma,  \
                       dbeta, accumulate, c1, c2, dbias_zero);                                                     \
  if (!(phases & 2)) {                                                                                             \
  } else if (gp) {                                                                                                 \
    hipLaunchKernelGGL(bn_relu_bwd_apply_kernel<TT>, grid, dim3(256), 0, s, (const TT*)g1, ldg1, (const TT*)gp,    \
                       ldgp, scale, shift, (const TT*)x, ldx, mean, invstd, gamma, c1, c2, (TT*)dx, lddx,     \
                       dbias_conv ? part2 : nullptr, B, H, W, C);                                                  \
  } else {                                                                                                         \
    hipLaunchKernelGGL(bn_relu_bwd_apply_flat_kernel<TT>, grid, dim3(256), 0, s, (const TT*)g1, ldg1,              \
                       scale, shift, (const TT*)x, ldx, mean, invstd, gamma, c1, c2, (TT*)dx, lddx,           \
                       dbias_conv ? part2 : nullptr, (long)B * H * W, C, bn_rev);                                  \
  }
  if (dtype == S2S_BF16) { S2S_BN_BWD(bf16_t) }
  else if (dtype == S2S_F32) { S2S_BN_BWD(float) }
  else return S2S_ERR_DTYPE;
#undef S2S_BN_BWD
  if (dbias_conv && (phases & 2))
    hipLaunchKernelGGL(colsum_finalize_kernel, dim3(cdiv(C, 32)), dim3(1024), 0, s, part2, prereduce(part2, nb, C, s),
                       C, dbias_conv, accumulate);
  S2S_LAUNCH_CHECK();
  return S2S_OK;
}

extern "C" int s2s_bn_relu_bwd(int dtype, const void* g1, int ldg1, const void* gp, int ldgp, const float* scale,
                               const float* shift, const void* x, int ldx, const float* mean, const float* invstd, const float* gamma,
                               float* dgamma, float* dbeta, float* dbias_conv, int accumulate, void* dx, int lddx,
                               float* work, int B, int H, int W, int C, void* stream) {
  return s2s_bn_relu_bwd_phase(dtype, g1, ldg1, gp, ldgp, scale, shift, x, ldx, mean, invstd, gamma, dgamma, dbeta,
                               dbias_conv, accumulate, dx, lddx, work, B, H, W, C, (long)B * H * W, 3, stream);
}
```

stain2stain_amd/engine.py:

```python
from __future__ import annotations

from dataclasses import dataclass, field
from typing import Dict, List, Optional, Sequence, Tuple

import contextlib
import threading

import torch
import torch.distributed as dist

from . import ops

BN_EPS = 1e-5
BN_MOMENTUM = 0.1


class SyncBNExchange:

    def __init__(self, process_group=None):
        if not (dist.is_available() and dist.is_initialized()):
            raise RuntimeError("stain2stain_amd: SyncBatchNorm needs an initialised torch.distributed process group")
        self.pg = process_group
        self.world = dist.get_world_size(process_group)
        self._host = dist.get_backend(process_group) != "nccl"

    def __call__(self, t: torch.Tensor) -> None:
        if self._host and t.is_cuda:
            h = t.cpu()
            dist.all_reduce(h, op=dist.ReduceOp.SUM, group=self.pg)
            t.copy_(h)
        else:
            dist.all_reduce(t, op=dist.ReduceOp.SUM, group=self.pg)


sync_bn: Optional[SyncBNExchange] = None
_module_exchanges: Dict[int, SyncBNExchange] = {}


def _module_exchange(bn: torch.nn.Module) -> Optional[SyncBNExchange]:
    if not isinstance(bn, torch.nn.SyncBatchNorm) or not (dist.is_available() and dist.is_initialized()):
        return None
    pg = bn.process_group
    import os
    if dist.get_world_size(pg) < 2 and os.environ.get("S2S_FORCE_DDP") != "1":
        return None
    key = id(pg) if pg is not None else 0
    ex = _module_exchanges.get(key)
    if ex is None or ex.pg is not pg:
        ex = _module_exchanges[key] = SyncBNExchange(pg)
    return ex


@contextlib.contextmanager
def sync_batchnorm(exchange: Optional[SyncBNExchange]):
    global sync_bn
    prev, sync_bn = sync_bn, exchange
    try:
        yield
    finally:
        sync_bn = prev


mutation_epoch = [0]


class ConvBN:

    def __init__(self, prefix: str, i_conv: str, i_bn: str, seq: torch.nn.Sequential):
        self.prefix = prefix
        self.idx = (i_conv, i_bn)
        self._seq = seq
        self._pack: Dict[torch.dtype, Tuple] = {}
        self._pack_key: Dict[torch.dtype, Tuple] = {}
        self._eval_key, self._eval_ss = None, None

    @property
    def conv(self) -> torch.nn.Conv2d:
        return self._seq._modules[self.idx[0]]

    @property
    def bn(self) -> torch.nn.BatchNorm2d:
        return self._seq._modules[self.idx[1]]

    @property
    def cout(self) -> int:
        return self.conv.weight.shape[0]

    @property
    def cin(self) -> int:
        return self.conv.weight.shape[1]

    def packed(self, dtype: torch.dtype):
        w = self.conv.weight
        key = (w.data_ptr(), w._version, w.device)
        if self._pack_key.get(dtype) != key:
            old = self._pack.get(dtype)
            reuse = old if (old is not None and old[0].device == w.device) else None
            self._pack[dtype] = ops.pack_conv3x3(w.detach(), dtype, want_dgrad=True, out=reuse)
            self._pack_key[dtype] = key
        return self._pack[dtype]

    def invalidate(self) -> None:
        self._pack_key.clear()

    def eval_affine(self):
        bn = self.bn
        ts = (bn.weight, bn.bias, bn.running_mean, bn.running_var)
        key = (mutation_epoch[0],) + tuple((t.data_ptr(), t._version) for t in ts)
        if self._eval_key != key:
            self._eval_ss = ops.bn_eval_prepare(bn.weight.detach(), bn.bias.detach(), bn.running_mean,
                                                bn.running_var, bn.eps)
            self._eval_key = key
        return self._eval_ss

    def ensure_buffers(self, dtype: torch.dtype):
        old = self._pack.get(dtype)
        w = self.conv.weight
        if old is None or old[0].device != w.device:
            L = ops._L()
            wf = torch.empty((L.s2s_pack_conv3x3_fwd_elems(self.cout, self.cin),), dtype=dtype, device=w.device)
            wd = torch.empty((L.s2s_pack_conv3x3_dgrad_elems(self.cout, self.cin),), dtype=dtype, device=w.device)
            self._pack[dtype] = (wf, wd)
            self._pack_key.pop(dtype, None)
        return self._pack[dtype]

    def mark_packed(self, dtype: torch.dtype) -> None:
        w = self.conv.weight
        self._pack_key[dtype] = (w.data_ptr(), w._version, w.device)


def _pack_table(cbs: Sequence[ConvBN], dtype: torch.dtype) -> Tuple[torch.Tensor, int]:
    rows, start = [], 0
    for cb in cbs:
        wf, wd = cb.ensure_buffers(dtype)
        rows.append([cb.conv.weight.data_ptr(), wf.data_ptr(), wd.data_ptr(), cb.cout, cb.cin, start])
        start += ((cb.cout + 31) // 32) * ((cb.cin + 31) // 32)
    return torch.tensor(rows, dtype=torch.int64, device=cbs[0].conv.weight.device), start


class Conv3x3Packer:

    def __init__(self, blocks: Sequence[Tuple[ConvBN, ConvBN]], dtype: torch.dtype):
        stem = blocks[0][0]
        self.convs = [cb for pair in blocks for cb in pair
                      if cb is not stem or (dtype == torch.bfloat16 and cb.cin <= 8)]
        self.dtype = dtype
        self.desc, self.total = _pack_table(self.convs, dtype)
        self.repack()

    def repack(self) -> None:
        ops.pack_conv3x3_batched(self.desc, self.total, self.dtype)
        for cb in self.convs:
            cb.mark_packed(self.dtype)


_REPACK_DESC: Dict[tuple, Tuple[torch.Tensor, int]] = {}


def repack_stale(cbs: Sequence[ConvBN], dtype: torch.dtype) -> None:
    stale = []
    for cb in cbs:
        w = cb.conv.weight
        if not w.is_cuda:
            return
        if cb._pack_key.get(dtype) != (w.data_ptr(), w._version, w.device):
            stale.append(cb)
    if len(stale) < 2:
        return
    bufs = [cb.ensure_buffers(dtype) for cb in stale]
    key = (dtype,) + tuple((cb.conv.weight.data_ptr(), b[0].data_ptr(), b[1].data_ptr(), cb.cout, cb.cin)
                           for cb, b in zip(stale, bufs))
    hit = _REPACK_DESC.get(key)
    if hit is None:
        if len(_REPACK_DESC) > 64:
            _REPACK_DESC.clear()
        hit = _REPACK_DESC[key] = _pack_table(stale, dtype)
    ops.pack_conv3x3_batched(hit[0], hit[1], dtype)
    for cb in stale:
        cb.mark_packed(dtype)


@dataclass
class LayerCtx:
    x0: Optional[torch.Tensor]
    x1: Optional[torch.Tensor]
    raw: torch.Tensor
    act: torch.Tensor
    stats: torch.Tensor
    count: Optional[int] = None
    sync: Optional["SyncBNExchange"] = None


@dataclass
class EncCtx:
    dtype: torch.dtype
    x_nchw: torch.Tensor
    layers: List[Tuple[LayerCtx, LayerCtx]] = field(default_factory=list)
    feats: List[torch.Tensor] = field(default_factory=list)


@dataclass
class DecCtx:
    dtype: torch.dtype
    t_emb: torch.Tensor
    h1: torch.Tensor = None
    a1: torch.Tensor = None
    h2: torch.Tensor = None
    lows: List[torch.Tensor] = field(default_factory=list)
    ups: List[torch.Tensor] = field(default_factory=list)
    skips: List[torch.Tensor] = field(default_factory=list)
    layers: List[Tuple[LayerCtx, LayerCtx]] = field(default_factory=list)
    v: torch.Tensor = None


def _stem_as_conv(x_nchw: torch.Tensor, dtype: torch.dtype) -> bool:
    return dtype == torch.bfloat16 and x_nchw.shape[1] <= 8


def _stem_image(x_nchw: torch.Tensor, dtype: torch.dtype) -> torch.Tensor:
    B, _, H, W = x_nchw.shape
    return ops.p2p_pack_input(x_nchw, None, torch.empty((B, H, W, 8), dtype=dtype, device=x_nchw.device))


def _conv_bn_relu(cb: ConvBN, x0, x1, dtype, training: bool, want_pool: bool = False, stem: bool = False):
    bn = cb.bn
    bias = cb.conv.bias.detach() if cb.conv.bias is not None else None
    if training:
        late_bias = None
        if stem and _stem_as_conv(x0, dtype):
            raw, stat = ops.conv3x3(_stem_image(x0, dtype), None, cb.packed(dtype)[0], None, cb.cout, want_stats=True)
            late_bias = bias
        elif stem:
            raw, stat = ops.stem_fwd(x0, cb.conv.weight.detach(), bias, dtype, want_stats=True)
        elif dtype == torch.bfloat16 and bias is not None:
            raw, stat = ops.conv3x3(x0, x1, cb.packed(dtype)[0], None, cb.cout, want_stats=True)
            late_bias = bias
        else:
            raw, stat = ops.conv3x3(x0, x1, cb.packed(dtype)[0], bias, cb.cout, want_stats=True)
        count = raw.shape[0] * raw.shape[1] * raw.shape[2]
        sx = sync_bn if sync_bn is not None else _module_exchange(bn)
        if sx is not None:
            sums = ops.bn_partial_sums(stat)
            sx(sums)
            stat = sums.view(2, -1, 1)
            count *= sx.world
        if count <= 1:
            raise ValueError(f"Expected more than 1 value per channel when training, got input size "
                             f"{[raw.shape[0], raw.shape[3], raw.shape[1], raw.shape[2]]}")
        track = bn.track_running_stats and bn.running_mean is not None
        mutation_epoch[0] += 1
        st = ops.bn_finalize(stat, count, bn.weight.detach(), bn.bias.detach(),
                             bn.running_mean if track else None, bn.running_var if track else None,
                             bn.num_batches_tracked if track else None,
                             BN_MOMENTUM if bn.momentum is None else bn.momentum, bn.eps, conv_bias=late_bias)
        act, pooled = ops.bn_relu_apply(raw, st[2], st[3], want_pool=want_pool)
        return LayerCtx(x0, x1, raw, act, st, count if sx is not None else None, sx), act, pooled
    ss = cb.eval_affine()
    if stem and _stem_as_conv(x0, dtype):
        act, _ = ops.conv3x3(_stem_image(x0, dtype), None, cb.packed(dtype)[0], bias, cb.cout, scale=ss[0], shift=ss[1], relu=True)
        pooled = ops.maxpool2(act) if want_pool else None
    elif stem:
        raw, _ = ops.stem_fwd(x0, cb.conv.weight.detach(), bias, dtype, want_stats=False)
        act, pooled = ops.bn_relu_apply(raw, ss[0], ss[1], want_pool=want_pool)
    else:
        act, _ = ops.conv3x3(x0, x1, cb.packed(dtype)[0], bias, cb.cout, scale=ss[0], shift=ss[1], relu=True)
        pooled = ops.maxpool2(act) if want_pool else None
    return None, act, pooled


class _SideState(threading.local):
    stream: Optional[torch.cuda.Stream] = None
    keep: Optional[List[torch.Tensor]] = None


_side = _SideState()


@contextlib.contextmanager
def side_scope(stream: Optional[torch.cuda.Stream]):
    prev = _side.stream, _side.keep
    _side.stream, _side.keep = stream, []
    try:
        yield
    finally:
        try:
            join_side(stream)
        finally:
            _side.stream, _side.keep = prev


def current_side() -> Optional[torch.cuda.Stream]:
    return _side.stream


def run_on_side(fn, keep=()) -> None:
    side = _side.stream
    if side is None:
        fn()
        return
    ev = torch.cuda.Event()
    ev.record()
    with torch.cuda.stream(side):
        side.wait_event(ev)
        fn()
    _side.keep.extend(t for t in keep if t is not None)


def join_side(side: Optional[torch.cuda.Stream]) -> None:
    if side is not None:
        torch.cuda.current_stream().wait_stream(side)


def _g(grads: Dict[str, torch.Tensor], name: str) -> torch.Tensor:
    try:
        return grads[name]
    except KeyError as e:
        raise RuntimeError(f"stain2stain_amd: no gradient buffer for parameter {name!r}") from e


def _conv_bn_relu_bwd(cb: ConvBN, lc: LayerCtx, g1, gp, grads, accumulate: bool, need_dx: bool, stem: bool = False):
    p = cb.prefix
    i_conv, i_bn = cb.idx
    dgamma = _g(grads, f"{p}.{i_bn}.weight")
    dbeta = _g(grads, f"{p}.{i_bn}.bias")
    dbias = _g(grads, f"{p}.{i_conv}.bias") if cb.conv.bias is not None else None
    draw = ops.bn_relu_bwd(g1, gp, lc.raw, lc.stats, cb.bn.weight.detach(), dgamma, dbeta, dbias, accumulate,
                           exchange=lc.sync, count_total=lc.count)
    dw = _g(grads, f"{p}.{i_conv}.weight")
    if stem:
        run_on_side(lambda: ops.stem_wgrad(draw, lc.x0, dw, None, accumulate), (draw,))
        return None
    run_on_side(lambda: ops.conv3x3_wgrad(draw, lc.x0, lc.x1, dw, accumulate), (draw,))
    if not need_dx:
        return None
    dx, _ = ops.conv3x3(draw, None, cb.packed(draw.dtype)[1], None, cb.cin)
    return dx


def encoder_forward(blocks: Sequence[Tuple[ConvBN, ConvBN]], x_nchw: torch.Tensor, dtype: torch.dtype,
                    training: bool) -> EncCtx:
    ctx = EncCtx(dtype, x_nchw)
    nlev = len(blocks)
    repack_stale([cb for l, pair in enumerate(blocks) for j, cb in enumerate(pair)
                  if (l, j) != (0, 0) or _stem_as_conv(x_nchw, dtype)], dtype)
    inp = x_nchw
    for l, (c1, c2) in enumerate(blocks):
        lc1, a1, _ = _conv_bn_relu(c1, inp, None, dtype, training, stem=(l == 0))
        lc2, a2, pooled = _conv_bn_relu(c2, a1, None, dtype, training, want_pool=(l + 1 < nlev))
        ctx.layers.append((lc1, lc2))
        ctx.feats.append(a2)
        inp = pooled
    return ctx


def encoder_backward(blocks: Sequence[Tuple[ConvBN, ConvBN]], ctx: EncCtx, dfeats: Sequence[Optional[torch.Tensor]],
                     grads: Dict[str, torch.Tensor], accumulate: bool = False, on_group_done=None) -> None:
    gpool = None
    nlev = len(blocks)
    for l in range(len(blocks) - 1, -1, -1):
        c1, c2 = blocks[l]
        lc1, lc2 = ctx.layers[l]
        g1 = dfeats[l]
        if g1 is None and gpool is None:
            raise RuntimeError("stain2stain_amd: encoder level without any incoming gradient")
        ga1 = _conv_bn_relu_bwd(c2, lc2, g1, gpool, grads, accumulate, need_dx=True)
        if on_group_done is not None:
            on_group_done()
        gpool = _conv_bn_relu_bwd(c1, lc1, ga1, None, grads, accumulate, need_dx=(l > 0), stem=(l == 0))
        if on_group_done is not None:
            on_group_done()


def decoder_forward(dec, bottleneck: torch.Tensor, skips: Sequence[torch.Tensor], t_emb: torch.Tensor,
                    dtype: torch.dtype, training: bool, with_head: bool = True) -> DecCtx:
    ctx = DecCtx(dtype, t_emb)
    repack_stale([cb for pair in dec.up_blocks for cb in pair], dtype)
    tbias = None
    if getattr(dec, "time_mlp", None) is not None:
        l0, l2 = dec.time_mlp[0], dec.time_mlp[2]
        ctx.h1 = ops.linear_fwd(t_emb, l0.weight.detach(), l0.bias.detach())
        ctx.a1 = ops.silu_fwd(ctx.h1)
        ctx.h2 = ops.linear_fwd(ctx.a1, l2.weight.detach(), l2.bias.detach())
        tbias = ops.linear_fwd(ctx.h2, dec.time_proj.weight.detach(), dec.time_proj.bias.detach())
    x = bottleneck
    for i, ((c1, c2), skip) in enumerate(zip(dec.up_blocks, skips)):
        B, Hs, Ws, _ = skip.shape
        up = torch.empty((B, Hs, Ws, x.shape[3]), dtype=dtype, device=x.device)
        ops.upsample2x_fwd(x, up, tbias if i == 0 else None)
        lc1, a1, _ = _conv_bn_relu(c1, skip, up, dtype, training)
        lc2, a2, _ = _conv_bn_relu(c2, a1, None, dtype, training)
        ctx.lows.append(x); ctx.ups.append(up); ctx.skips.append(skip); ctx.layers.append((lc1, lc2))
        x = a2
    ctx.lows.append(x)
    if not with_head:
        return ctx
    ctx.v = ops.head_fwd(x, dec.outc.weight.detach(), dec.outc.bias.detach() if dec.outc.bias is not None else None)
    return ctx


def decoder_backward(dec, ctx: DecCtx, dv: Optional[torch.Tensor], grads: Dict[str, torch.Tensor],
                     accumulate: bool = False, need_dt_emb: bool = False, on_group_done=None,
                     g_head: Optional[torch.Tensor] = None):
    if g_head is not None:
        g = g_head
    else:
        g = ops.head_bwd(dv, ctx.lows[-1], dec.outc.weight.detach(), _g(grads, "outc.weight"),
                         _g(grads, "outc.bias") if dec.outc.bias is not None else None, accumulate)
    if on_group_done is not None:
        on_group_done()
    nup = len(ctx.layers)
    dskips: List[torch.Tensor] = [None] * len(ctx.layers)
    for i in range(len(ctx.layers) - 1, -1, -1):
        c1, c2 = dec.up_blocks[i]
        lc1, lc2 = ctx.layers[i]
        ga1 = _conv_bn_relu_bwd(c2, lc2, g, None, grads, accumulate, need_dx=True)
        if on_group_done is not None:
            on_group_done()
        dcat = _conv_bn_relu_bwd(c1, lc1, ga1, None, grads, accumulate, need_dx=True)
        cs = ctx.skips[i].shape[3]
        dskips[i] = dcat[..., :cs]
        low = ctx.lows[i]
        g = ops.upsample2x_bwd(dcat[..., cs:], low.shape[1], low.shape[2])
        if on_group_done is not None:
            on_group_done()
    dbott = g
    if getattr(dec, "time_mlp", None) is None:
        return dbott, dskips, None
    dtb = ops.pixel_sum(g)
    l0, l2 = dec.time_mlp[0], dec.time_mlp[2]
    dh2 = ops.linear_bwd(dtb, ctx.h2, dec.time_proj.weight.detach(), _g(grads, "time_proj.weight"),
                         _g(grads, "time_proj.bias"), True, accumulate)
    da1 = ops.linear_bwd(dh2, ctx.a1, l2.weight.detach(), _g(grads, "time_mlp.2.weight"),
                         _g(grads, "time_mlp.2.bias"), True, accumulate)
    dh1 = ops.silu_bwd(ctx.h1, da1)
    dt_emb = ops.linear_bwd(dh1, ctx.t_emb, l0.weight.detach(), _g(grads, "time_mlp.0.weight"),
                            _g(grads, "time_mlp.0.bias"), need_dt_emb, accumulate)
    if on_group_done is not None:
        on_group_done()
    return dbott, dskips, dt_emb
```

stain2stain_amd/multitask_trainer.py:

```python
from __future__ import annotations

from typing import Dict, List, Optional, Tuple

import torch
import torch.distributed as dist

from . import engine, evaluation, ops
from .components import FlowMatchingDecoder, SegmentationDecoder, SharedEncoder
from .ddp import all_reduce_mean_scalar
from .ema import TrainerEMA
from .fused_step import FlatParams


def _layer_groups(named: Dict[str, torch.nn.Parameter], prefix: str, owner: str) -> List[List[Tuple[str, torch.nn.Parameter]]]:
    out = []
    for idx in (("3.", "4."), ("0.", "1.")):
        out.append([(f"{owner}.{n}", p) for n, p in named.items() if any(n.startswith(prefix + i) for i in idx)])
    return out


def _decoder_groups(dec, owner: str) -> List[List[Tuple[str, torch.nn.Parameter]]]:
    named = dict(dec.named_parameters())
    groups = [[(f"{owner}.{n}", p) for n, p in named.items() if n.startswith("outc.")]]
    for i in range(len(dec.ups) - 1, -1, -1):
        groups += _layer_groups(named, f"ups.{i}.conv.double_conv.", owner)
    if getattr(dec, "time_mlp", None) is not None:
        groups.append([(f"{owner}.{n}", p) for n, p in named.items() if n.startswith("time_")])
    return groups


def _encoder_groups(enc, owner: str) -> List[List[Tuple[str, torch.nn.Parameter]]]:
    named = dict(enc.named_parameters())
    groups = []
    for i in range(len(enc.downs) - 1, -1, -1):
        groups += _layer_groups(named, f"downs.{i}.maxpool_conv.1.double_conv.", owner)
    return groups + _layer_groups(named, "inc.double_conv.", owner)


class MultiTaskTrainer:

    def __init__(self, encoder: SharedEncoder, flow_decoder: FlowMatchingDecoder, seg_decoder: SegmentationDecoder,
                 time_emb_dim: int = 256, lr: float = 1e-4, weight_decay: float = 1e-5,
                 betas: Tuple[float, float] = (0.9, 0.999), eps: float = 1e-8, seg_loss_weight: float = 1.0,
                 dice_weight: float = 0.5, dice_smooth: float = 1.0, num_classes: Optional[int] = None,
                 ignore_index: int = -100, sigma: float = 0.0, bucket_mb: float = 4.0, process_group=None,
                 sync_loss: bool = True, max_bucket_mb: float = 16.0, sharded_optimizer: bool = False,
                 ema_decay: Optional[float] = None, ema_buffers: bool = True):
        dev = next(encoder.parameters()).device
        if dev.type != "cuda":
            raise RuntimeError("stain2stain_amd: MultiTaskTrainer needs the networks on a GPU (HIP-only implementation)")
        if not (encoder.compute_dtype == flow_decoder.compute_dtype == seg_decoder.compute_dtype):
            raise ValueError("encoder and decoders must share one precision")
        self.encoder, self.flow_decoder, self.seg_decoder = encoder, flow_decoder, seg_decoder
        self.time_emb_dim, self.sigma = time_emb_dim, sigma
        self.lr, self.wd, self.betas, self.eps = lr, weight_decay, tuple(betas), eps
        self.seg_loss_weight, self.dice_weight, self.dice_smooth = seg_loss_weight, dice_weight, dice_smooth
        self.num_classes, self.ignore_index = num_classes, ignore_index
        self.pg, self.sync_loss = process_group, sync_loss
        self._dtype = encoder.compute_dtype
        groups = _decoder_groups(seg_decoder, "seg_decoder") + _decoder_groups(flow_decoder, "flow_decoder") \
            + _encoder_groups(encoder, "encoder")
        n_named = sum(1 for m in (encoder, flow_decoder, seg_decoder) for _ in m.parameters())
        if sum(len(g) for g in groups) != n_named or any(not g for g in groups):
            raise RuntimeError("parameter grouping does not cover the networks")
        self.fp = FlatParams(groups, bucket_mb, process_group, max_bucket_mb, sharded_optimizer)
        gr = self.fp.grads
        self.grads_enc = {k[len("encoder."):]: v for k, v in gr.items() if k.startswith("encoder.")}
        self.grads_flow = {k[len("flow_decoder."):]: v for k, v in gr.items() if k.startswith("flow_decoder.")}
        self.grads_seg = {k[len("seg_decoder."):]: v for k, v in gr.items() if k.startswith("seg_decoder.")}
        from .ddp import broadcast_from_rank0
        broadcast_from_rank0([b for m in (encoder, flow_decoder, seg_decoder) for b in m.buffers()], process_group)
        self.packer = engine.Conv3x3Packer(list(encoder._blocks) + list(flow_decoder.up_blocks)
                                           + list(seg_decoder.up_blocks), self._dtype)
        self._side = ops.side_stream_for(dev)
        self.overlap_wgrad = True
        self._group = 0
        self._eval_owner = object()
        self._generation = evaluation.GenerationEval()
        self._ema = None
        if ema_decay is not None:
            self.fp.enable_ema(ema_decay)
            self._ema = TrainerEMA(self.fp, [encoder, flow_decoder, seg_decoder], ema_buffers)

    @property
    def step_count(self) -> int:
        return self.fp.step_count

    def _group_done(self) -> None:
        self.fp.bucketer.mark_ready_ordered(self._group, self._side if self.overlap_wgrad else None)
        self._group += 1

    def forward_backward(self, source: torch.Tensor, target: torch.Tensor, mask: torch.Tensor,
                         t: Optional[torch.Tensor] = None, want_outputs: bool = False):
        enc, fdec, sdec = self.encoder, self.flow_decoder, self.seg_decoder
        dt = self._dtype
        x0, x1 = source.float().contiguous(), target.float().contiguous()
        B = x0.shape[0]
        if t is None:
            t = torch.rand(B, device=x0.device, dtype=torch.float32)
        t = t.float().contiguous()
        eps_noise = torch.randn_like(x0) if self.sigma != 0.0 else None
        xt, ut = ops.cfm_sample(x0, x1, t, self.sigma, eps_noise)
        ectx1 = engine.encoder_forward(enc._blocks, xt, dt, True)
        temb = ops.time_embedding(t, self.time_emb_dim)
        f1 = ectx1.feats
        dctx_f = engine.decoder_forward(fdec, f1[-1], f1[:-1][::-1], temb, dt, True, with_head=False)
        ectx2 = engine.encoder_forward(enc._blocks, x0, dt, True)
        f2 = ectx2.feats
        dctx_s = engine.decoder_forward(sdec, f2[-1], f2[:-1][::-1], None, dt, True)
        logits = dctx_s.v
        flow, g_head, v = ops.head_loss_fused(dctx_f.lows[-1], fdec.outc.weight.detach(),
                                              fdec.outc.bias.detach() if fdec.outc.bias is not None else None, ut,
                                              self.grads_flow["outc.weight"], self.grads_flow.get("outc.bias"),
                                              want_v=want_outputs)
        w = float(self.seg_loss_weight)
        if self.num_classes is not None:
            tgt = mask[:, 0] if (mask.dim() == 4 and mask.shape[1] == 1) else mask
            seg3, dz = ops.seg_loss_multiclass(logits, tgt.long(), self.ignore_index, self.dice_smooth, self.dice_weight,
                                               want_grad=True, grad_scale=w, validate=False)
        else:
            seg3, dz = ops.seg_loss(logits, mask.float().reshape(logits.shape), self.dice_smooth, self.dice_weight,
                                    want_grad=True, grad_scale=w)
        total = flow + w * seg3[0]
        self.fp.bucketer.start_step()
        self._group = 0
        with engine.side_scope(self._side if self.overlap_wgrad else None):
            L = len(f1) - 1
            dbs, dss, _ = engine.decoder_backward(sdec, dctx_s, dz, self.grads_seg, on_group_done=self._group_done)
            dbf, dsf, _ = engine.decoder_backward(fdec, dctx_f, None, self.grads_flow, g_head=g_head,
                                                  on_group_done=self._group_done)
            engine.encoder_backward(enc._blocks, ectx2, [dss[L - 1 - l] for l in range(L)] + [dbs], self.grads_enc)
            engine.encoder_backward(enc._blocks, ectx1, [dsf[L - 1 - l] for l in range(L)] + [dbf], self.grads_enc,
                                    accumulate=True, on_group_done=self._group_done)
        second = "seg_ce" if self.num_classes is not None else "seg_bce"
        losses = {"total": total, "flow": flow, "seg": seg3[0], "seg_dice": seg3[1], second: seg3[2]}
        return losses, ({"v": v, "logits": logits} if want_outputs else None)

    def optimizer_step(self) -> None:
        engine.join_side(self._side)
        self.fp.adam(self.lr, self.betas, self.eps, self.wd)
        if self._ema is not None:
            self._ema.update_buffers()
        self.packer.repack()
        engine.mutation_epoch[0] += 1
        if self._ema is not None:
            self._ema.after_step()

    def _ema_on(self) -> TrainerEMA:
        if self._ema is None:
            raise RuntimeError("stain2stain_amd: this trainer keeps no EMA (construct it with ema_decay=...)")
        return self._ema

    def ema_model(self) -> Tuple[SharedEncoder, FlowMatchingDecoder, SegmentationDecoder]:
        return tuple(self._ema_on().modules())

    def _ema_container(self) -> torch.nn.ModuleDict:
        enc, fdec, sdec = self._ema_on().copies
        return torch.nn.ModuleDict(dict(encoder=enc, flow_decoder=fdec, seg_decoder=sdec))

    def ema_state_dict(self) -> Dict[str, torch.Tensor]:
        ema = self._ema_on()
        ema.modules()
        return ema.state_dict(self._ema_container().state_dict())

    def load_ema_state_dict(self, sd: Dict[str, torch.Tensor]) -> None:
        self._ema_on().load_state_dict(sd, self._ema_container())

    def step(self, source: torch.Tensor, target: torch.Tensor, mask: torch.Tensor,
             t: Optional[torch.Tensor] = None) -> torch.Tensor:
        losses, _ = self.forward_backward(source, target, mask, t)
        total = losses["total"]
        work = all_reduce_mean_scalar(total, self.pg) if self.sync_loss else None
        self.optimizer_step()
        if work is not None:
            work.wait()
            total = total / dist.get_world_size(self.pg)
        return total

    def evaluate(self, source: torch.Tensor, target: torch.Tensor, mask: torch.Tensor, t: Optional[torch.Tensor] = None,
                 accumulator: Optional[evaluation.EvalAccumulator] = None,
                 use_ema: bool = False) -> Dict[str, torch.Tensor]:
        with ops.workspace_owner(self._eval_owner), evaluation.eval_grad_mode():
            x0, x1 = source.float().contiguous(), target.float().contiguous()
            if t is None:
                t = torch.rand(x0.shape[0], device=x0.device, dtype=torch.float32)
            t = t.float().contiguous()
            eps_noise = torch.randn_like(x0) if self.sigma != 0.0 else None
            xt, ut = ops.cfm_sample(x0, x1, t, self.sigma, eps_noise)
            enc, fdec, sdec = self.ema_model() if use_ema else (self.encoder, self.flow_decoder, self.seg_decoder)
            flow = evaluation.flow_loss(enc, fdec, self.time_emb_dim, xt, t, ut)
            logits = evaluation.mask_logits(enc, sdec, x0)
            d = evaluation.segmentation_values(logits, mask, self.num_classes, self.ignore_index, self.dice_smooth,
                                               self.dice_weight)
            second = "seg_ce" if self.num_classes is not None else "seg_bce"
            out = {"loss": flow + float(self.seg_loss_weight) * d["seg"], "flow_loss": flow, "seg_loss": d["seg"],
                   "seg_dice": d["seg_dice"], second: d[second], "dice_coef": d["dice_coef"], "iou": d["iou"]}
        if accumulator is not None:
            accumulator.add(out, x0.shape[0])
        return out

    def evaluate_generation(self, source: torch.Tensor, target: torch.Tensor, num_steps: int = 50,
                            method: str = "euler", graph: bool = False, use_ema: bool = False,
                            accumulator: Optional[evaluation.EvalAccumulator] = None,
                            quantize: bool = True, stain: Optional[dict] = None) -> Dict[str, torch.Tensor]:
        enc, fdec, _ = self.ema_model() if use_ema else (self.encoder, self.flow_decoder, self.seg_decoder)
        with ops.workspace_owner(self._eval_owner), evaluation.eval_grad_mode():
            return evaluation.generation_values(self._generation, bool(use_ema), enc, fdec, self.time_emb_dim, source,
                                                target, num_steps, method, graph, quantize, accumulator, stain)

    def close(self) -> None:
        self._generation.close()
        ops.release_workspaces(self._eval_owner)

    def __del__(self):
        try:
            self.close()
        except Exception:
            pass
```

stain2stain_amd/ops.py:

```python
from __future__ import annotations

import contextlib
import ctypes
import os
import sys
from typing import Optional, Tuple

import torch

from . import _native

BF16, F32 = 0, 1


def _dt(t: torch.Tensor) -> int:
    if t.dtype == torch.bfloat16:
        return BF16
    if t.dtype == torch.float32:
        return F32
    raise RuntimeError(f"stain2stain_amd: unsupported activation dtype {t.dtype}")


_raw_stream = getattr(torch._C, "_cuda_getCurrentRawStream", None)
_raw_device = getattr(torch._C, "_cuda_getDevice", None)
# ... 69 lines not shown

    def __exit__(self, *exc):
        global _WS_OWNER
        _WS_OWNER = self.prev
        return False


def release_workspaces(owner) -> None:
    k = id(owner)
    for key in [key for key in _WORKSPACE if key[3] == k]:
        del _WORKSPACE[key]


def _workspace(device: torch.device, numel: int, tag: str) -> torch.Tensor:
    key = (device.index if device.index is not None else torch.cuda.current_device(), tag, _stream(), _WS_OWNER)
    buf = _WORKSPACE.get(key)
    if buf is None or buf.numel() < numel:
        buf = torch.empty((max(numel, 1 << 20),), dtype=torch.float32, device=device)
        _WORKSPACE[key] = buf
    return buf[:numel]


_PROFILE: Optional[list] = None
_PROFILE_ONLY: Optional[set] = None
PROFILE_TAG = ""


@contextlib.contextmanager
def profile_tag(tag: str):
    global PROFILE_TAG
    prev, PROFILE_TAG = PROFILE_TAG, tag
    try:
        yield
    finally:
        PROFILE_TAG = prev


def profile_start(only=None) -> None:
    global _PROFILE, _PROFILE_ONLY
    _PROFILE = []
    _PROFILE_ONLY = set(only) if only else None


def cu_masked_stream(device, spec: str) -> torch.cuda.Stream:
    k, m = (int(v) for v in spec.split(":"))
    if not 0 < k <= m:
        raise ValueError("CU mask spec K:M needs 0 < K <= M")
    dev = torch.device(device)
    key = (dev.index if dev.index is not None else torch.cuda.current_device(), k, m)
    if key in _MASKED_STREAMS:
        return _MASKED_STREAMS[key]
    n = torch.cuda.get_device_properties(dev).multi_processor_count
    words = (ctypes.c_uint32 * ((n + 31) // 32))()
    for i in range(n):
        if i % m < k:
            words[i // 32] |= 1 << (i % 32)
    out = ctypes.c_long(0)
    with torch.cuda.device(dev):
        _native.check(_L().s2s_stream_create_cu_mask(ctypes.addressof(words), len(words), ctypes.addressof(out)),
                      "stream_create_cu_mask")
    stream = torch.cuda.ExternalStream(out.value, device=dev)
    _MASKED_STREAMS[key] = stream
    return stream


_MASKED_STREAMS = {}


def side_stream_for(device) -> Optional[torch.cuda.Stream]:
    import os
    if os.environ.get("S2S_WGRAD_STREAM", "1") == "0":
        return None
    spec = os.environ.get("S2S_WGRAD_CUS", "")
    if spec and spec != "0":
        return cu_masked_stream(device, spec)
    return torch.cuda.Stream(device=device)


_SHARED_SIDE = {}


def shared_side_stream(device) -> Optional[torch.cuda.Stream]:
    dev = torch.device(device)
    key = dev.index if dev.index is not None else torch.cuda.current_device()
    if key not in _SHARED_SIDE:
        _SHARED_SIDE[key] = side_stream_for(dev)
    return _SHARED_SIDE[key]


class TimingEvent:

    def __init__(self):
        out = ctypes.c_long(0)
        _native.check(_L().s2s_event_create(1, ctypes.addressof(out)), "event_create")
        self._e = out.value

    def record(self) -> None:
        _native.check(_L().s2s_event_record(self._e, _stream()), "event_record")

    def elapsed_time(self, end: "TimingEvent") -> float:
        ms = ctypes.c_float(0.0)
        _native.check(_L().s2s_event_synchronize(end._e), "event_synchronize")
        _native.check(_L().s2s_event_elapsed_ms(self._e, end._e, ctypes.addressof(ms)), "event_elapsed")
        return float(ms.value)

    def __del__(self):
        try:
            if self._e and not sys.is_finalizing():
                _L().s2s_event_destroy(self._e)
        except Exception:
            pass


def _timing_event():
    if os.environ.get("S2S_TIMING_EVENTS", "1") == "0":
        return torch.cuda.Event(enable_timing=True)
    return TimingEvent()


def profile_stop() -> list:
    global _PROFILE
    out, _PROFILE = _PROFILE or [], None
    return out


def _timed(name: str, work_fn=None):
    def deco(fn):
        def wrapped(*args, **kwargs):
            if _PROFILE is None or (_PROFILE_ONLY is not None and name not in _PROFILE_ONLY):
                return fn(*args, **kwargs)
            e0 = _timing_event()
            e1 = _timing_event()
            e0.record()
            out = fn(*args, **kwargs)
            e1.record()
            _PROFILE.append((name + ("@" + PROFILE_TAG if PROFILE_TAG else ""), work_fn(*args, **kwargs) if work_fn else 0.0, e0, e1))
            return out
        wrapped.__name__ = fn.__name__
        wrapped.__doc__ = fn.__doc__
        return wrapped
    return deco


def _conv_flops(x0, x1, w_packed, bias, cout, **kw) -> float:
    B, H, W, c0 = x0.shape
    cin = c0 + (x1.shape[3] if x1 is not None else 0)
    return 2.0 * B * H * W * cout * 9 * cin


def _wgrad_flops(dy, x0, x1, grad_oihw, accumulate=False) -> float:
    B, H, W, cout = dy.shape
    cin = x0.shape[3] + (x1.shape[3] if x1 is not None else 0)
    return 2.0 * B * H * W * cout * 9 * cin


@_timed("conv3x3_mfma", _conv_flops)
def conv3x3(x0: torch.Tensor, x1: Optional[torch.Tensor], w_packed: torch.Tensor, bias: Optional[torch.Tensor],
            cout: int, *, want_stats: bool = False, scale: Optional[torch.Tensor] = None,
            shift: Optional[torch.Tensor] = None, relu: bool = False, out: Optional[torch.Tensor] = None):
    B, H, W, c0 = x0.shape
    dt = _dt(x0)
    p0, ld0 = _nhwc(x0)
    p1, ld1, c1 = 0, 8, 0
    if x1 is not None:
        if x1.shape[:3] != x0.shape[:3] or x1.dtype != x0.dtype:
            raise RuntimeError("stain2stain_amd: conv3x3 sources disagree in shape/dtype")
        p1, ld1 = _nhwc(x1)
        c1 = x1.shape[3]
    if w_packed.dtype != x0.dtype or w_packed.numel() != _L().s2s_pack_conv3x3_fwd_elems(cout, c0 + c1):
        raise RuntimeError("stain2stain_amd: packed weight does not match (cout, cin, dtype)")
    if out is None:
        out = torch.empty((B, H, W, cout), dtype=x0.dtype, device=x0.device)
    elif out.shape != (B, H, W, cout) or out.dtype != x0.dtype:
        raise RuntimeError("stain2stain_amd: conv3x3 output buffer mismatch")
    py, ldy = _nhwc(out)
    stat, nb = None, 0
    if want_stats:
        nb = _L().s2s_conv3x3_stat_rows(dt, B, H, W, cout, c0, c1, ld0, ld1, int(bias is not None))
        _native.check(min(nb, 0), "conv3x3_stat_rows")
        stat = torch.empty((2, cout, nb), dtype=torch.float32, device=x0.device)
    kwork = None
    if not want_stats:
        nsplit = _L().s2s_conv3x3_ksplit(dt, B, H, W, cout, c0 + c1)
        if nsplit > 1:
            kwork = torch.empty((nsplit, B * H * W, cout), dtype=torch.float32, device=x0.device)
    rc = _L().s2s_conv3x3_nhwc_s(dt, p0, ld0, c0, p1, ld1, c1, _ptr(w_packed), _f32(bias), py, ldy, _f32(stat), nb,
                                 _f32(scale), _f32(shift), int(relu), _f32(kwork), B, H, W, cout, _stream())
    _native.check(rc, "conv3x3")
    return out, stat


def conv3x3_wgrad(dy: torch.Tensor, x0: torch.Tensor, x1: Optional[torch.Tensor], grad_oihw: torch.Tensor,
                  accumulate: bool = False) -> None:
    B, H, W, cout = dy.shape
    c0 = x0.shape[3]
    dt = _dt(dy)
    if x0.dtype != dy.dtype or x0.shape[:3] != dy.shape[:3]:
        raise RuntimeError("stain2stain_amd: conv3x3_wgrad operand mismatch")
    pdy, lddy = _nhwc(dy)
    p0, ld0 = _nhwc(x0)
    p1, ld1, c1 = 0, 8, 0
    if x1 is not None:
        p1, ld1 = _nhwc(x1)
        c1 = x1.shape[3]
    if tuple(grad_oihw.shape) != (cout, c0 + c1, 3, 3):
        raise RuntimeError("stain2stain_amd: conv3x3_wgrad gradient buffer has the wrong shape")
    s = _L().s2s_conv3x3_wgrad_splits(dt, B, H, W, c0 + c1, cout)
    part = _workspace(dy.device, s * 9 * cout * (c0 + c1), "wgrad")
    if _PROFILE is not None and (_PROFILE_ONLY is None or "conv3x3_wgrad_mfma" in _PROFILE_ONLY):
        for name, phase, work in (("conv3x3_wgrad_mfma", 1, _wgrad_flops(dy, x0, x1, grad_oihw)), ("wgrad_fold", 2, 0.0)):
            e0 = _timing_event()
            e1 = _timing_event()
            e0.record()
            rc = _L().s2s_conv3x3_wgrad_phase(dt, pdy, lddy, cout, p0, ld0, c0, p1, ld1, c1, _f32(part), _f32(grad_oihw),
                                              int(accumulate), B, H, W, phase, _stream())
            e1.record()
            _native.check(rc, "conv3x3_wgrad")
            _PROFILE.append((name, work, e0, e1))
        return
    rc = _L().s2s_conv3x3_wgrad_nhwc(dt, pdy, lddy, cout, p0, ld0, c0, p1, ld1, c1, _f32(part), _f32(grad_oihw),
                                     int(accumulate), B, H, W, _stream())
    _native.check(rc, "conv3x3_wgrad")


@_timed("stem_fwd")
def stem_fwd(x_nchw: torch.Tensor, w: torch.Tensor, bias: Optional[torch.Tensor], dtype: torch.dtype,
             want_stats: bool = True):
    B, cin, H, W = x_nchw.shape
    cout = w.shape[0]
    if tuple(w.shape) != (cout, cin, 3, 3):
        raise RuntimeError("stain2stain_amd: stem weight shape")
    y = torch.empty((B, H, W, cout), dtype=dtype, device=x_nchw.device)
    stat = None
    if want_stats:
        stat = torch.empty((2, cout, _L().s2s_stem_stat_blocks(B, H, W)), dtype=torch.float32, device=y.device)
    rc = _L().s2s_stem_conv3x3_fwd(_dt(y), _f32(x_nchw), _f32(w), _f32(bias), y.data_ptr(), cout, _f32(stat), B, H, W,
                                   cin, cout, _stream())
    _native.check(rc, "stem_conv3x3_fwd")
    return y, stat


@_timed("stem_wgrad")
def stem_wgrad(dy: torch.Tensor, x_nchw: torch.Tensor, dw: torch.Tensor, dbias: Optional[torch.Tensor],
               accumulate: bool = False) -> None:
    B, H, W, cout = dy.shape
    cin = x_nchw.shape[1]
    pdy, lddy = _nhwc(dy)
    nb = _L().s2s_stem_wgrad_blocks(B, H, W)
    part = torch.empty(((cin + 2) // 3, 2 * nb, cout, 32), dtype=torch.float32, device=dy.device)
    rc = _L().s2s_stem_conv3x3_wgrad(_dt(dy), pdy, lddy, _f32(x_nchw), _f32(part), _f32(dw), _f32(dbias),
                                     int(accumulate), B, H, W, cin, cout, _stream())
    _native.check(rc, "stem_conv3x3_wgrad")


@_timed("head_fwd")
def head_fwd(x: torch.Tensor, w: torch.Tensor, bias: Optional[torch.Tensor]) -> torch.Tensor:
    B, H, W, C = x.shape
    cout = w.shape[0]
    px, ldx = _nhwc(x)
    y = torch.empty((B, cout, H, W), dtype=torch.float32, device=x.device)
    rc = _L().s2s_head_conv1x1_fwd(_dt(x), px, ldx, _f32(w.reshape(cout, C)), _f32(bias), _f32(y), B, H, W, C, cout,
                                   _stream())
    _native.check(rc, "head_conv1x1_fwd")
    return y


@_timed("head_bwd")
def head_bwd(dy_nchw: torch.Tensor, x: torch.Tensor, w: torch.Tensor, dw: torch.Tensor, dbias: Optional[torch.Tensor],
             accumulate: bool = False) -> torch.Tensor:
    B, H, W, C = x.shape
    cout = w.shape[0]
    px, ldx = _nhwc(x)
    dx = torch.empty((B, H, W, C), dtype=x.dtype, device=x.device)
    nb = _L().s2s_head_wgrad_blocks(B, H, W)
    part = torch.empty((nb, cout, C + 1), dtype=torch.float32, device=x.device)
    rc = _L().s2s_head_conv1x1_bwd(_dt(x), _f32(dy_nchw), px, ldx, _f32(w.reshape(cout, C)), dx.data_ptr(), C,
                                   _f32(part), _f32(dw.reshape(cout, C)), _f32(dbias), int(accumulate), B, H, W, C,
                                   cout, _stream())
    _native.check(rc, "head_conv1x1_bwd")
    return dx


@_timed("head_loss_fused")
def head_loss_fused(x: torch.Tensor, w: torch.Tensor, bias: Optional[torch.Tensor], u_nchw: torch.Tensor,
                    dw: torch.Tensor, dbias: Optional[torch.Tensor], want_v: bool = False, grad_scale: float = 1.0,
                    accumulate: bool = False):
    B, H, W, C = x.shape
    cout = w.shape[0]
    px, ldx = _nhwc(x)
    dx = torch.empty((B, H, W, C), dtype=x.dtype, device=x.device)
    v = torch.empty((B, cout, H, W), dtype=torch.float32, device=x.device) if want_v else None
    nb = _L().s2s_head_loss_blocks(B, H, W)
    part = torch.empty((nb, cout, C + 1), dtype=torch.float32, device=x.device)
    lpart = torch.empty((nb,), dtype=torch.float64, device=x.device)
    loss = torch.empty((), dtype=torch.float32, device=x.device)
    rc = _L().s2s_head_loss_fused(_dt(x), px, ldx, _f32(w.reshape(cout, C)), _f32(bias), _f32(u_nchw), _f32(v),
                                  dx.data_ptr(), C, float(grad_scale), _f32(part), lpart.data_ptr(),
                                  _f32(dw.reshape(cout, C)), _f32(dbias), loss.data_ptr(), int(accumulate), B, H, W, C,
                                  cout, _stream())
    _native.check(rc, "head_loss_fused")
    return loss, dx, v


@_timed("bn_finalize")
def bn_finalize(stat: torch.Tensor, count: int, gamma, beta, running_mean, running_var, num_batches,
                momentum: float = 0.1, eps: float = 1e-5, conv_bias: Optional[torch.Tensor] = None):
    _, C, nblk = stat.shape
    dev = stat.device
    out = torch.empty((4, C), dtype=torch.float32, device=dev)
    rc = _L().s2s_bn_finalize_b(_f32(stat), nblk, C, count, _f32(gamma), _f32(beta), _f32(running_mean),
                                _f32(running_var), 0 if num_batches is None else num_batches.data_ptr(), momentum, eps,
                                out[0].data_ptr(), out[1].data_ptr(), out[2].data_ptr(), out[3].data_ptr(),
                                _f32(conv_bias), _stream())
    _native.check(rc, "bn_finalize")
    return out


def bn_partial_sums(stat: torch.Tensor) -> torch.Tensor:
    _, C, nblk = stat.shape
    sums = torch.empty((2, C), dtype=torch.float32, device=stat.device)
    _native.check(_L().s2s_bn_partial_sums(_f32(stat), nblk, C, _f32(sums), _stream()), "bn_partial_sums")
    return sums


def bn_eval_prepare(gamma, beta, rmean, rvar, eps: float = 1e-5):
    C = gamma.numel()
    out = torch.empty((2, C), dtype=torch.float32, device=gamma.device)
    rc = _L().s2s_bn_eval_prepare(C, _f32(gamma), _f32(beta), _f32(rmean), _f32(rvar), eps, out[0].data_ptr(),
                                  out[1].data_ptr(), _stream())
    _native.check(rc, "bn_eval_prepare")
    return out


@_timed("bn_relu_apply")
def bn_relu_apply(x: torch.Tensor, scale: torch.Tensor, shift: torch.Tensor, out: Optional[torch.Tensor] = None,
                  pool: Optional[torch.Tensor] = None, want_pool: bool = False):
    B, H, W, C = x.shape
    px, ldx = _nhwc(x)
    if out is None:
        out = torch.empty((B, H, W, C), dtype=x.dtype, device=x.device)
    py, ldy = _nhwc(out)
    pp, ldp = 0, 8
    if want_pool and pool is None:
        pool = torch.empty((B, H // 2, W // 2, C), dtype=x.dtype, device=x.device)
    if pool is not None:
        pp, ldp = _nhwc(pool)
    rc = _L().s2s_bn_relu_apply(_dt(x), px, ldx, _f32(scale), _f32(shift), py, ldy, pp, ldp, B, H, W, C, _stream())
    _native.check(rc, "bn_relu_apply")
    return out, pool


@_timed("maxpool2")
def maxpool2(x: torch.Tensor) -> torch.Tensor:
    B, H, W, C = x.shape
    px, ldx = _nhwc(x)
    pool = torch.empty((B, H // 2, W // 2, C), dtype=x.dtype, device=x.device)
    rc = _L().s2s_maxpool2(_dt(x), px, ldx, pool.data_ptr(), C, B, H, W, C, _stream())
    _native.check(rc, "maxpool2")
    return pool


@_timed("bn_relu_bwd")
def bn_relu_bwd(g1: Optional[torch.Tensor], gp: Optional[torch.Tensor], x: torch.Tensor,
                stats: torch.Tensor, gamma: torch.Tensor, dgamma: torch.Tensor, dbeta: torch.Tensor,
                dbias_conv: Optional[torch.Tensor], accumulate: bool = False, exchange=None,
                count_total: Optional[int] = None) -> torch.Tensor:
    B, H, W, C = x.shape
    px, ldx = _nhwc(x)
    p1, ld1 = (0, 8) if g1 is None else _nhwc(g1)
    p2, ld2 = (0, 8) if gp is None else _nhwc(gp)
    dx = torch.empty((B, H, W, C), dtype=x.dtype, device=x.device)
    nb = _L().s2s_bn_bwd_blocks(B, H, W, C)
    work = torch.empty((4 * nb * C + 2 * C,), dtype=torch.float32, device=x.device)
    if exchange is not None:
        for phase in (1, 2):
            rc = _L().s2s_bn_relu_bwd_phase(_dt(x), p1, ld1, p2, ld2, stats[2].data_ptr(), stats[3].data_ptr(), px, ldx,
                                            stats[0].data_ptr(), stats[1].data_ptr(),
                                            _f32(gamma), _f32(dgamma), _f32(dbeta), _f32(dbias_conv), int(accumulate),
                                            dx.data_ptr(), C, _f32(work), B, H, W, C,
                                            int(count_total if count_total is not None else B * H * W), phase, _stream())
            _native.check(rc, "bn_relu_bwd")
            if phase == 1:
                exchange(work[4 * nb * C:])
        return dx
    rc = _L().s2s_bn_relu_bwd(_dt(x), p1, ld1, p2, ld2, stats[2].data_ptr(), stats[3].data_ptr(), px, ldx,
                              stats[0].data_ptr(), stats[1].data_ptr(),
                              _f32(gamma), _f32(dgamma), _f32(dbeta), _f32(dbias_conv), int(accumulate),
                              dx.data_ptr(), C, _f32(work), B, H, W, C, _stream())
    _native.check(rc, "bn_relu_bwd")
    return dx


@_timed("upsample2x_fwd")
def upsample2x_fwd(x: torch.Tensor, out: torch.Tensor, bias_nc: Optional[torch.Tensor] = None) -> None:
    B, Hin, Win, C = x.shape
    _, Hout, Wout, Co = out.shape
    if Co != C or out.dtype != x.dtype:
        raise RuntimeError("stain2stain_amd: upsample output slice mismatch")
    px, ldx = _nhwc(x)
    py, ldy = _nhwc(out)
    rc = _L().s2s_upsample2x_bilinear_ac_fwd(_dt(x), px, ldx, _f32(bias_nc), py, ldy, B, Hin, Win, Hout, Wout, C,
                                             _stream())
    _native.check(rc, "upsample2x_fwd")


@_timed("upsample2x_bwd")
def upsample2x_bwd(dy: torch.Tensor, hin: int, win: int) -> torch.Tensor:
    B, Hout, Wout, C = dy.shape
    pdy, lddy = _nhwc(dy)
    dx = torch.empty((B, hin, win, C), dtype=dy.dtype, device=dy.device)
    rc = _L().s2s_upsample2x_bilinear_ac_bwd(_dt(dy), pdy, lddy, dx.data_ptr(), C, B, hin, win, Hout, Wout, C,
                                             _stream())
    _native.check(rc, "upsample2x_bwd")
    return dx


def pixel_sum(x: torch.Tensor) -> torch.Tensor:
    B, H, W, C = x.shape
    px, ldx = _nhwc(x)
    out = torch.empty((B, C), dtype=torch.float32, device=x.device)
    rc = _L().s2s_pixel_sum(_dt(x), px, ldx, _f32(out), B, H * W, C, 0, _stream())
    _native.check(rc, "pixel_sum")
    return out


def time_embedding(t: torch.Tensor, dim: int) -> torch.Tensor:
    t = t.reshape(-1).to(torch.float32).contiguous()
    out = torch.empty((t.numel(), dim), dtype=torch.float32, device=t.device)
    _native.check(_L().s2s_time_embedding(_f32(t), _f32(out), t.numel(), dim, _stream()), "time_embedding")
    return out


def linear_fwd(x: torch.Tensor, w: torch.Tensor, b: Optional[torch.Tensor]) -> torch.Tensor:
    B, K = x.shape
    N = w.shape[0]
    y = torch.empty((B, N), dtype=torch.float32, device=x.device)
    _native.check(_L().s2s_linear_fwd(_f32(x), _f32(w), _f32(b), _f32(y), B, K, N, _stream()), "linear_fwd")
    return y


def linear_bwd(dy: torch.Tensor, x: torch.Tensor, w: torch.Tensor, dw: torch.Tensor, db: Optional[torch.Tensor],
               need_dx: bool = True, accumulate: bool = False) -> Optional[torch.Tensor]:
    B, K = x.shape
    N = w.shape[0]
    dx = torch.empty((B, K), dtype=torch.float32, device=x.device) if need_dx else None
    _native.check(_L().s2s_linear_bwd(_f32(dy), _f32(x), _f32(w), _f32(dx), _f32(dw), _f32(db), int(accumulate), B, K,
                                      N, _stream()), "linear_bwd")
    return dx


def silu_fwd(h: torch.Tensor) -> torch.Tensor:
    a = torch.empty_like(h)
    _native.check(_L().s2s_silu_fwd(_f32(h), _f32(a), h.numel(), _stream()), "silu_fwd")
    return a


def silu_bwd(h: torch.Tensor, da: torch.Tensor) -> torch.Tensor:
    dh = torch.empty_like(h)
    _native.check(_L().s2s_silu_bwd(_f32(h), _f32(da), _f32(dh), h.numel(), _stream()), "silu_bwd")
    return dh


@_timed("cfm_sample")
def cfm_sample(x0: torch.Tensor, x1: torch.Tensor, t: torch.Tensor, sigma: float = 0.0,
               eps: Optional[torch.Tensor] = None):
    xt = torch.empty_like(x0)
    ut = torch.empty_like(x0)
    B = x0.shape[0]
    _native.check(_L().s2s_cfm_sample(_f32(x0), _f32(x1), _f32(t), _f32(eps), float(sigma), _f32(xt), _f32(ut), B,
                                      x0.numel() // B, _stream()), "cfm_sample")
    return xt, ut


@_timed("mse_loss")
def mse_loss(v: torch.Tensor, u: torch.Tensor, want_grad: bool = True, grad_scale: float = 1.0):
    loss = torch.empty((), dtype=torch.float32, device=v.device)
    dv = torch.empty_like(v) if want_grad else None
    work = torch.empty((1024,), dtype=torch.float64, device=v.device)
    _native.check(_L().s2s_mse_loss(_f32(v), _f32(u), _f32(dv), float(grad_scale), loss.data_ptr(), work.data_ptr(),
                                    v.numel(), _stream()), "mse_loss")
    return loss, dv


def seg_loss(z: torch.Tensor, g: torch.Tensor, smooth: float = 1.0, dice_weight: float = 0.5, want_grad: bool = True,
             grad_scale: float = 1.0):
    z = z.contiguous()
    g = g.to(torch.float32).contiguous()
    out = torch.empty((3,), dtype=torch.float32, device=z.device)
    dz = torch.empty_like(z) if want_grad else None
    work = torch.empty((512 * 4 + 4,), dtype=torch.float64, device=z.device)
    _native.check(_L().s2s_seg_loss(_f32(z), _f32(g), _f32(dz), _f32(out), work.data_ptr(), z.numel(), float(smooth),
                                    float(dice_weight), float(grad_scale), _stream()), "seg_loss")
    return out, dz


def seg_loss_multiclass(z: torch.Tensor, target: torch.Tensor, ignore_index: int = -100, smooth: float = 1.0,
                        dice_weight: float = 0.5, want_grad: bool = True, grad_scale: float = 1.0,
                        validate: bool = True):
    if z.dim() != 4 or target.dim() != 3 or target.shape != (z.shape[0], z.shape[2], z.shape[3]):
        raise RuntimeError("stain2stain_amd: seg_loss_multiclass wants logits [B,C,H,W] and target [B,H,W]")
    B, C, H, W = z.shape
    z = z.contiguous()
    target = target.to(torch.int64).contiguous()
    if validate:
        lo, hi = int(target.min()), int(target.max())
        if lo < 0 or hi >= C:
            raise RuntimeError(f"stain2stain_amd: class index out of range [0, {C}) in segmentation target "
                               f"(min {lo}, max {hi})")
    out = torch.empty((3,), dtype=torch.float32, device=z.device)
    dz = torch.empty_like(z) if want_grad else None
    work = torch.empty((513 * 26,), dtype=torch.float64, device=z.device)
    _native.check(_L().s2s_seg_loss_multiclass(_f32(z), target.data_ptr(), _f32(dz), _f32(out), work.data_ptr(), B,
                                               H * W, C, int(ignore_index), float(smooth), float(dice_weight),
                                               float(grad_scale), _stream()), "seg_loss_multiclass")
    return out, dz


EV_BLOCKS = 512


def _gpu_f32_operand(t: torch.Tensor, what: str) -> torch.Tensor:
    if not t.is_cuda:
        raise RuntimeError(f"stain2stain_amd: {what} is not on the GPU (there is no CPU path)")
    if t.dtype != torch.float32:
        raise RuntimeError(f"stain2stain_amd: {what} must be float32, got {t.dtype}")
    return t.contiguous()


def _binary_mask(g: torch.Tensor) -> torch.Tensor:
    if g.dtype in (torch.bool, torch.uint8):
        return g.to(torch.float32).contiguous()
    if g.dtype != torch.float32:
        raise RuntimeError(f"stain2stain_amd: mask must be float32 (0/1), uint8 or bool, got {g.dtype}")
    return g.contiguous()


@_timed("seg_eval_binary")
def seg_eval_binary(z: torch.Tensor, g: torch.Tensor, smooth: float = 1.0, dice_weight: float = 0.5):
    if z.dim() != 4 or z.shape[1] != 1:
        raise RuntimeError(f"stain2stain_amd: seg_eval_binary wants logits [B,1,H,W], got {tuple(z.shape)}")
    if g.dim() == 3:
        g = g.unsqueeze(1)
    if tuple(g.shape) != tuple(z.shape):
        raise RuntimeError(f"stain2stain_amd: mask shape {tuple(g.shape)} does not match logits {tuple(z.shape)}")
    if g.device != z.device:
        raise RuntimeError("stain2stain_amd: logits and mask are on different devices")
    z, g = _gpu_f32_operand(z, "logits"), _binary_mask(g)
    out = torch.empty((5,), dtype=torch.float32, device=z.device)
    counts = torch.empty((4,), dtype=torch.int64, device=z.device)
    work = _workspace(z.device, 2 * EV_BLOCKS * 8, "seg_eval").view(torch.float64)
    _native.check(_L().s2s_seg_eval_binary(_f32(z), _f32(g), _f32(out), counts.data_ptr(), work.data_ptr(), z.numel(),
                                           float(smooth), float(dice_weight), _stream()), "seg_eval_binary")
    return out, counts


@_timed("seg_eval_multiclass")
def seg_eval_multiclass(z: torch.Tensor, target: torch.Tensor, ignore_index: int = -100, smooth: float = 1.0,
                        dice_weight: float = 0.5):
    if z.dim() != 4:
        raise RuntimeError(f"stain2stain_amd: seg_eval_multiclass wants logits [B,C,H,W], got {tuple(z.shape)}")
    B, C, H, W = z.shape
    if not 2 <= C <= 8:
        raise RuntimeError(f"stain2stain_amd: seg_eval_multiclass supports 2 <= C <= 8 classes, got {C}")
    if target.dim() == 4 and target.shape[1] == 1:
        target = target[:, 0]
    if tuple(target.shape) != (B, H, W):
        raise RuntimeError(f"stain2stain_amd: target shape {tuple(target.shape)} does not match logits {tuple(z.shape)}")
    if target.dtype.is_floating_point or target.dtype == torch.bool or target.dtype.is_complex:
        raise RuntimeError(f"stain2stain_amd: target must hold integer class indices, got {target.dtype}")
    if target.device != z.device:
        raise RuntimeError("stain2stain_amd: logits and target are on different devices")
    z = _gpu_f32_operand(z, "logits")
    target = target.to(torch.int64).contiguous()
    out = torch.empty((5,), dtype=torch.float32, device=z.device)
    counts = torch.empty((32,), dtype=torch.int64, device=z.device)
    work = _workspace(z.device, 2 * EV_BLOCKS * 58, "seg_eval").view(torch.float64)
    _native.check(_L().s2s_seg_eval_multiclass(_f32(z), target.data_ptr(), _f32(out), counts.data_ptr(),
                                               work.data_ptr(), B, H * W, C, int(ignore_index), float(smooth),
                                               float(dice_weight), _stream()), "seg_eval_multiclass")
    return out, counts.view(4, 8)[:, :C]


@_timed("head_mse_eval")
def head_mse_eval(x: torch.Tensor, w: torch.Tensor, bias: Optional[torch.Tensor], u_nchw: torch.Tensor) -> torch.Tensor:
    if x.dim() != 4:
        raise RuntimeError("stain2stain_amd: head_mse_eval wants an NHWC activation [B,H,W,C]")
    B, H, W, C = x.shape
    cout = w.shape[0]
    if w.numel() != cout * C:
        raise RuntimeError(f"stain2stain_amd: head weight {tuple(w.shape)} does not match {C} input channels")
    if not 1 <= cout <= 8 or C % 8:
        raise RuntimeError(f"stain2stain_amd: head_mse_eval supports C % 8 == 0 and 1 <= Cout <= 8 (C={C}, Cout={cout})")
    if tuple(u_nchw.shape) != (B, cout, H, W):
        raise RuntimeError(f"stain2stain_amd: target shape {tuple(u_nchw.shape)} != {(B, cout, H, W)}")
    if bias is not None and bias.numel() != cout:
        raise RuntimeError("stain2stain_amd: head bias does not match its weight")
    px, ldx = _nhwc(x)
    u = _gpu_f32_operand(u_nchw, "flow target")
    nb = _L().s2s_head_mse_eval_blocks(B, H, W, C)
    _native.check(nb if nb < 0 else 0, "head_mse_eval_blocks")
    lpart = _workspace(x.device, 2 * nb, "head_mse_eval").view(torch.float64)
    loss = torch.empty((), dtype=torch.float32, device=x.device)
    _native.check(_L().s2s_head_mse_eval(_dt(x), px, ldx, _f32(w.detach().reshape(cout, C).contiguous()),
                                         _f32(None if bias is None else bias.detach().contiguous()), _f32(u),
                                         loss.data_ptr(), lpart.data_ptr(), B, H, W, C, cout, _stream()),
                  "head_mse_eval")
# ... 1054 lines not shown
```

stain2stain_amd/trainer.py:

```python
from __future__ import annotations

from typing import Dict, List, Optional, Tuple

import torch
import torch.distributed as dist

from . import engine, evaluation, ops
from .components import FlowUNet
from .ema import TrainerEMA
from .ddp import all_reduce_mean_scalar, broadcast_from_rank0
from .fused_step import CapturedStep, FlatParams


def _param_groups(net: FlowUNet) -> List[List[Tuple[str, str, torch.nn.Parameter]]]:
    dec, enc = net.flow_decoder, net.encoder
    dnamed = dict(dec.named_parameters())
    enamed = dict(enc.named_parameters())
    groups: List[List[Tuple[str, str, torch.nn.Parameter]]] = []

    def layer(owner, named, prefix):
        for idx in (("3.", "4."), ("0.", "1.")):
            groups.append([(owner, n, p) for n, p in named.items()
                           if any(n.startswith(prefix + i) for i in idx)])

    groups.append([("dec", n, p) for n, p in dnamed.items() if n.startswith("outc.")])
    for i in range(len(dec.ups) - 1, -1, -1):
        layer("dec", dnamed, f"ups.{i}.conv.double_conv.")
    groups.append([("dec", n, p) for n, p in dnamed.items() if n.startswith("time_")])
    for i in range(len(enc.downs) - 1, -1, -1):
        layer("enc", enamed, f"downs.{i}.maxpool_conv.1.double_conv.")
    layer("enc", enamed, "inc.double_conv.")
    groups = [g for g in groups if g] if getattr(dec, "time_mlp", None) is None else groups
    seen = sum(len(g) for g in groups)
    if seen != len(dnamed) + len(enamed) or any(not g for g in groups):
        raise RuntimeError("parameter grouping does not cover the network")
    return groups


class FusedAdamHandle(torch.optim.Optimizer):

    def __init__(self, trainer: "CFMTrainer", lr, betas, eps, weight_decay):
        self._trainer = trainer
        super().__init__([trainer.fp.p], dict(lr=lr, betas=tuple(betas), eps=eps, weight_decay=weight_decay))

    @torch.no_grad()
    def step(self, closure=None):
        loss = closure() if closure is not None else None
        self._trainer.optimizer_step()
        return loss

    def zero_grad(self, set_to_none: bool = False) -> None:
        pass

    def state_dict(self):
        return self._trainer.optimizer_state_dict()

    def load_state_dict(self, state_dict) -> None:
        self._trainer.load_optimizer_state_dict(state_dict)


class CFMTrainer:
    def __init__(self, net: FlowUNet, lr: float = 1e-4, weight_decay: float = 1e-5,
                 betas: Tuple[float, float] = (0.9, 0.999), eps: float = 1e-8, sigma: float = 0.0,
                 bucket_mb: float = 4.0, process_group=None, sync_loss: bool = True, max_bucket_mb: float = 16.0,
                 sharded_optimizer: bool = False, sync_batchnorm: bool = False, graph: bool = False,
                 ema_decay: Optional[float] = None, ema_buffers: bool = True):
        dev = next(net.parameters()).device
        if dev.type != "cuda":
            raise RuntimeError("stain2stain_amd: CFMTrainer needs the network on a GPU (HIP-only implementation)")
        self.net = net
        self.sigma = sigma
        self.pg = process_group
        self.sync_loss = sync_loss
        groups = [[(f"{owner}.{name}", p) for owner, name, p in g] for g in _param_groups(net)]
        self.fp = FlatParams(groups, bucket_mb, process_group, max_bucket_mb, sharded_optimizer)
        self.grads_enc = {k[len("enc."):]: v for k, v in self.fp.grads.items() if k.startswith("enc.")}
        self.grads_dec = {k[len("dec."):]: v for k, v in self.fp.grads.items() if k.startswith("dec.")}
        names = {id(p): name for g in groups for name, p in g}
        self._names = [names[id(p)] for p in net.parameters()]
        self.optimizer = FusedAdamHandle(self, lr, betas, eps, weight_decay)
        self.n_params = sum(p.numel() for g in groups for _, p in g)
        self._group = 0
        self._sync_bn = engine.SyncBNExchange(process_group) if sync_batchnorm and self.bucketer.enabled else None
        broadcast_from_rank0(list(net.buffers()), process_group)
        self._dtype = net.encoder.compute_dtype
        self.packer = engine.Conv3x3Packer(list(net.encoder._blocks) + list(net.flow_decoder.up_blocks), self._dtype)
        self._side = ops.side_stream_for(dev)
        self.overlap_wgrad = True
        self.graph = graph
        self._graph_step = CapturedStep()
        self._ema = None
        if ema_decay is not None:
            self.fp.enable_ema(ema_decay)
            self._ema = TrainerEMA(self.fp, [net], ema_buffers)
        self._eval_owner = object()
        self._generation = evaluation.GenerationEval()

    step_count = property(lambda self: self.fp.step_count)
    bucketer = property(lambda self: self.fp.bucketer)
    flat_p = property(lambda self: self.fp.p)
    flat_g = property(lambda self: self.fp.g)
    _captured = property(lambda self: self._graph_step.graph)

    @property
    def _hp(self):
        return self.optimizer.param_groups[0]

    lr = property(lambda self: self._hp["lr"], lambda self, v: self._hp.__setitem__("lr", v))
    wd = property(lambda self: self._hp["weight_decay"], lambda self, v: self._hp.__setitem__("weight_decay", v))
    betas = property(lambda self: self._hp["betas"], lambda self, v: self._hp.__setitem__("betas", tuple(v)))
    eps = property(lambda self: self._hp["eps"], lambda self, v: self._hp.__setitem__("eps", v))

    def forward_backward(self, x0: torch.Tensor, x1: torch.Tensor, t: Optional[torch.Tensor] = None,
                         want_v: bool = True):
        net = self.net
        enc, dec = net.encoder, net.flow_decoder
        dt = enc.compute_dtype
        B = x0.shape[0]
        x0, x1 = x0.float().contiguous(), x1.float().contiguous()
        if t is None:
            t = torch.rand(B, device=x0.device, dtype=torch.float32)
        t = t.float().contiguous()
        eps_noise = torch.randn_like(x0) if self.sigma != 0.0 else None
        xt, ut = ops.cfm_sample(x0, x1, t, self.sigma, eps_noise)
        with engine.sync_batchnorm(self._sync_bn):
            ectx = engine.encoder_forward(enc._blocks, xt, dt, True)
            temb = ops.time_embedding(t, net.time_embedding.dim)
            feats = ectx.feats
            dctx = engine.decoder_forward(dec, feats[-1], feats[:-1][::-1], temb, dt, True, with_head=False)
        loss, g_head, v = ops.head_loss_fused(dctx.lows[-1], dec.outc.weight.detach(),
                                              dec.outc.bias.detach() if dec.outc.bias is not None else None, ut,
                                              self.grads_dec["outc.weight"], self.grads_dec.get("outc.bias"),
                                              want_v=want_v)
        dctx.v = v
        self.bucketer.start_step()
        self._group = 0
        with engine.side_scope(self._side if self.overlap_wgrad else None):
            dbott, dskips, _ = engine.decoder_backward(dec, dctx, None, self.grads_dec, g_head=g_head,
                                                       on_group_done=self._group_done)
            L = len(feats) - 1
            dfeats = [dskips[L - 1 - l] for l in range(L)] + [dbott]
            engine.encoder_backward(enc._blocks, ectx, dfeats, self.grads_enc, on_group_done=self._group_done)
        return loss, dctx.v

    def _group_done(self) -> None:
        self.bucketer.mark_ready_ordered(self._group, self._side if self.overlap_wgrad else None)
        self._group += 1

    def optimizer_step(self) -> None:
        self._enqueue_optimizer(None)
        self._after_step()

    def _after_step(self) -> None:
        engine.mutation_epoch[0] += 1
        if self._ema is not None:
            self._ema.after_step()

    def _enqueue_optimizer(self, hyper_dev: Optional[torch.Tensor]) -> None:
        engine.join_side(self._side)
        self.fp.adam(self.lr, self.betas, self.eps, self.wd, hyper_dev)
        if self._ema is not None:
            self._ema.update_buffers()
        self._repack()

    def _repack(self) -> None:
        self.packer.repack()

    def optimizer_state_dict(self) -> Dict:
        sd = self.fp.state_dict()
        state = {}
        if self.step_count > 0:
            for i, name in enumerate(self._names):
                state[i] = {"step": torch.tensor(float(self.step_count)),
                            "exp_avg": sd["exp_avg"][name], "exp_avg_sq": sd["exp_avg_sq"][name]}
        group = {"lr": self.lr, "betas": tuple(self.betas), "eps": self.eps, "weight_decay": self.wd,
                 "amsgrad": False, "maximize": False, "foreach": None, "capturable": False, "differentiable": False,
                 "fused": None, "params": list(range(len(self._names)))}
        return {"state": state, "param_groups": [group]}

    def load_optimizer_state_dict(self, sd: Dict) -> None:
        groups = sd["param_groups"]
        if len(groups) != 1 or len(groups[0]["params"]) != len(self._names):
            raise ValueError("optimizer state does not match this network (one group over net.parameters() expected)")
        if groups[0].get("amsgrad", False) or groups[0].get("maximize", False):
            raise ValueError("amsgrad / maximize Adam states are not supported")
        g = groups[0]
        self.lr, self.betas, self.eps, self.wd = g["lr"], tuple(g["betas"]), g["eps"], g["weight_decay"]
        steps = set()
        fp = self.fp
        fp.m.zero_()
        fp.v.zero_()
        for i, (p, name) in enumerate(zip(self.net.parameters(), self._names)):
            st = sd["state"].get(i, sd["state"].get(str(i)))
            if st is None:
                continue
            o, n = fp.slot[name]
            if tuple(st["exp_avg"].shape) != tuple(p.shape):
                raise ValueError(f"optimizer state {i}: shape {tuple(st['exp_avg'].shape)} != {tuple(p.shape)}")
            fp.m[o:o + n].copy_(st["exp_avg"].reshape(-1))
            fp.v[o:o + n].copy_(st["exp_avg_sq"].reshape(-1))
            steps.add(int(float(st["step"])))
        if len(steps) > 1:
            raise ValueError("per-parameter step counts differ; the flat Adam kernel keeps one")
        fp.step_count = steps.pop() if steps else 0

    def step(self, x0: torch.Tensor, x1: torch.Tensor, t: Optional[torch.Tensor] = None) -> torch.Tensor:
        with ops.workspace_owner(self):
            if self.graph and ops._PROFILE is None:
                if t is None:
                    t = torch.rand(x0.shape[0], device=x0.device, dtype=torch.float32)
                if self.sigma != 0.0:
                    raise NotImplementedError("graph=True with sigma != 0: the path noise is drawn inside forward_backward")
                loss = self._graph_step.run((tuple(x0.shape), x0.device, self.overlap_wgrad), (x0, x1, t),
                                            self._step_body, [self.fp], (self.lr, self.betas, self.eps, self.wd))
            else:
                loss = self._step_body(x0, x1, t, None)
            self._after_step()
            return loss

    def _step_body(self, x0, x1, t, hyper_dev) -> torch.Tensor:
        loss, _ = self.forward_backward(x0, x1, t, want_v=False)
        work = all_reduce_mean_scalar(loss, self.pg) if self.sync_loss else None
        self._enqueue_optimizer(hyper_dev)
        if work is not None:
            work.wait()
            loss = loss / dist.get_world_size(self.pg)
        return loss

    def _ema_on(self) -> TrainerEMA:
        if self._ema is None:
            raise RuntimeError("stain2stain_amd: this trainer keeps no EMA (construct it with ema_decay=...)")
        return self._ema

    def ema_model(self) -> FlowUNet:
        return self._ema_on().modules()[0]

    def ema_state_dict(self) -> Dict[str, torch.Tensor]:
        return self._ema_on().state_dict(self.ema_model().state_dict())

    def load_ema_state_dict(self, sd: Dict[str, torch.Tensor]) -> None:
        ema = self._ema_on()
        ema.load_state_dict(sd, ema.copies[0])

    def evaluate(self, x0: torch.Tensor, x1: torch.Tensor, t: Optional[torch.Tensor] = None,
                 accumulator: Optional[evaluation.EvalAccumulator] = None,
                 use_ema: bool = False) -> Dict[str, torch.Tensor]:
        net = self.ema_model() if use_ema else self.net
        with ops.workspace_owner(self._eval_owner), evaluation.eval_grad_mode():
            x0, x1 = x0.float().contiguous(), x1.float().contiguous()
            if t is None:
                t = torch.rand(x0.shape[0], device=x0.device, dtype=torch.float32)
            t = t.float().contiguous()
            eps_noise = torch.randn_like(x0) if self.sigma != 0.0 else None
            xt, ut = ops.cfm_sample(x0, x1, t, self.sigma, eps_noise)
            loss = evaluation.flow_loss(net.encoder, net.flow_decoder, net.time_embedding.dim, xt, t, ut)
        out = {"loss": loss}
        if accumulator is not None:
            accumulator.add(out, x0.shape[0])
        return out

    def evaluate_generation(self, x0: torch.Tensor, x1: torch.Tensor, num_steps: int = 50, method: str = "euler",
                            graph: bool = False, use_ema: bool = False,
                            accumulator: Optional[evaluation.EvalAccumulator] = None,
                            quantize: bool = True, stain: Optional[dict] = None) -> Dict[str, torch.Tensor]:
        net = self.ema_model() if use_ema else self.net
        with ops.workspace_owner(self._eval_owner), evaluation.eval_grad_mode():
            return evaluation.generation_values(self._generation, bool(use_ema), net.encoder, net.flow_decoder,
                                                net.time_embedding.dim, x0, x1, num_steps, method, graph, quantize,
                                                accumulator, stain)

    def close(self) -> None:
        self._generation.close()
        self._graph_step.close()
        ops.release_workspaces(self)
        ops.release_workspaces(self._eval_owner)

    def __del__(self):
        try:
            self.close()
        except Exception:
            pass
```

Measured before the change: 2249.

## Fuse last decoder BN-ReLU, 1x1 head and loss into tail kernels

Adds fused tail kernels that apply the final decoder block's BN+ReLU on the fly inside the 1x1 head forward, loss and head weight-gradient pass. The backward BN sums and the dx apply are folded into a second kernel that recomputes the activation from the raw conv output. The goal is to avoid materialising the activated tensor, and to avoid reading and writing it and its gradient separately in the BN apply, head and BN backward passes. In exchange the activation is recomputed, the trainer gains extra code paths, and the fused path is only used when the velocity output is not requested.

After: 2286 (median of 6 runs). 1.6% higher.

```diff
diff --git a/include/stain2stain_hip.h b/include/stain2stain_hip.h
--- a/include/stain2stain_hip.h
+++ b/include/stain2stain_hip.h
@@ -60,6 +60,16 @@
 int s2s_head_loss_fused(int dtype, const void* x, int ldx, const float* w, const float* bias, const float* u_nchw,
                         float* v_nchw, void* dx, int lddx, float grad_scale, float* part, double* lpart, float* dw,
                         float* dbias, float* loss, int accumulate, int B, int H, int W, int C, int Cout, void* stream);
+
+int s2s_tail_blocks(int B, int H, int W);
+int s2s_tail_fwd_loss(int dtype, const void* raw, int ldx, const float* scale, const float* shift, const float* mean,
+                      const float* invstd, const float* w, const float* bias, const float* u_nchw, float* v_nchw,
+                      float* g_nchw, float grad_scale, float* part, double* lpart, float* bnwork, float* dw,
+                      float* dbias, float* loss, float* dgamma, float* dbeta, float* conv_dbias, int accumulate, int B,
+                      int H, int W, int C, int Cout, void* stream);
+int s2s_tail_bwd_apply(int dtype, const void* raw, int ldx, const float* g_nchw, const float* w, const float* scale,
+                       const float* shift, const float* mean, const float* invstd, const float* gamma,
+                       const float* bnwork, void* dx, int lddx, int B, int H, int W, int C, int Cout, void* stream);
 
 int s2s_bn_finalize(const float* part, int nblk, int C, long count, const float* gamma, const float* beta,
                     float* running_mean, float* running_var, long* num_batches_tracked, float momentum, float eps,
diff --git a/stain2stain_amd/csrc/conv_edge.hip b/stain2stain_amd/csrc/conv_edge.hip
--- a/stain2stain_amd/csrc/conv_edge.hip
+++ b/stain2stain_amd/csrc/conv_edge.hip
@@ -628,6 +628,202 @@
     case 64: S2S_HLN(64) default: return false;
   }
 #undef S2S_HLN
+}
+
+template <int CTRL>
+__device__ __forceinline__ float dpp_f32(float v) {
+  return __builtin_bit_cast(float, __builtin_amdgcn_update_dpp(0, __builtin_bit_cast(int, v), CTRL, 0xf, 0xf, true));
+}
+template <int PCB>
+__device__ __forceinline__ float group_sum(float t) {
+  if (PCB >= 2) t += dpp_f32<0xB1>(t);
+  if (PCB >= 4) t += dpp_f32<0x4E>(t);
+  if (PCB >= 8) t += dpp_f32<0x141>(t);
+  if (PCB >= 16) t += dpp_f32<0x140>(t);
+#pragma unroll
+  for (int m = 16; m < PCB; m <<= 1) t += __shfl_xor(t, m, 64);
+  return t;
+}
+
+__device__ __forceinline__ bf16x8 tail_ld(const bf16_t* p) { return *reinterpret_cast<const bf16x8*>(p); }
+__device__ __forceinline__ f32x8 tail_ld(const float* p) { return load8(p); }
+__device__ __forceinline__ float tail_at(const bf16x8& v, int k) { return (float)v[k]; }
+__device__ __forceinline__ float tail_at(const f32x8& v, int k) { return v.v[k]; }
+
+template <typename T, int PCB, int MO>
+__global__ __launch_bounds__(256) void tail_fwd_loss_kernel(const T* __restrict__ raw, int ldx,
+                                                            const float* __restrict__ scale, const float* __restrict__ shift,
+                                                            const float* __restrict__ w, const float* __restrict__ bias,
+                                                            const float* __restrict__ u, float* __restrict__ v_out,
+                                                            float* __restrict__ g_out, float coef,
+                                                            float* __restrict__ part, double* __restrict__ lpart,
+                                                            long npix, int HW, int Cout) {
+  constexpr int C = PCB * 8, PPB = 256 / PCB;
+  __shared__ float fold[256][MO * 8 + 1];
+  __shared__ float dbf[PPB][MO];
+  __shared__ double lred[256];
+  const int tid = threadIdx.x, pc = tid & (PCB - 1), slot = tid / PCB;
+  float wr[MO][8], bo[MO];
+#pragma unroll
+  for (int o = 0; o < MO; ++o) {
+    bo[o] = (o < Cout && bias) ? bias[o] : 0.f;
+#pragma unroll
+    for (int k = 0; k < 8; ++k) wr[o][k] = o < Cout ? w[o * C + pc * 8 + k] : 0.f;
+  }
+  float sc[8], sh[8];
+#pragma unroll
+  for (int k = 0; k < 8; ++k) { sc[k] = scale[pc * 8 + k]; sh[k] = shift[pc * 8 + k]; }
+  float dwacc[MO][8], dbacc[MO];
+#pragma unroll
+  for (int o = 0; o < MO; ++o) {
+    dbacc[o] = 0.f;
+#pragma unroll
+    for (int k = 0; k < 8; ++k) dwacc[o][k] = 0.f;
+  }
+  double lsum = 0.0;
+  const int np = (int)npix, stride = (int)gridDim.x * PPB;
+  struct Stage {
+    decltype(tail_ld((const T*)nullptr)) r;
+    float u[MO];
+    long i;
+  };
+  auto fetch = [&](Stage& st, int pf) {
+    pf = pf < np ? pf : np - 1;
+    st.r = tail_ld(raw + (long)pf * ldx + pc * 8);
+    const int n = pf / HW, q = pf - n * HW;
+    st.i = (long)n * Cout * HW + q;
+#pragma unroll
+    for (int o = 0; o < MO; ++o) st.u[o] = u[st.i + (long)(o < Cout ? o : Cout - 1) * HW];
+  };
+  Stage sa, sb;
+  fetch(sa, (int)blockIdx.x * PPB + slot);
+  fetch(sb, (int)blockIdx.x * PPB + slot + stride);
+  auto step = [&](Stage& st, int p0) {
+    const int p = p0 + slot;
+    const bool ok = p < np;
+    f32x8 r;
+#pragma unroll
+    for (int k = 0; k < 8; ++k) r.v[k] = tail_at(st.r, k);
+    float cu[MO];
+#pragma unroll
+    for (int o = 0; o < MO; ++o) cu[o] = st.u[o];
+    const long i0 = st.i;
+    fetch(st, p + 2 * stride);
+    float a[8];
+#pragma unroll
+    for (int k = 0; k < 8; ++k)
+      a[k] = to_f32(from_f32<T>(fmaxf(fmaf(r.v[k], sc[k], sh[k]), 0.f)));
+    float vv[MO];
+#pragma unroll
+    for (int o = 0; o < MO; ++o) {
+      float t = 0.f;
+#pragma unroll
+      for (int k = 0; k < 8; ++k) t = fmaf(a[k], wr[o][k], t);
+      vv[o] = group_sum<PCB>(t) + bo[o];
+    }
+    float g[MO];
+#pragma unroll
+    for (int o = 0; o < MO; ++o) {
+      const float d = vv[o] - cu[o];
+      g[o] = (ok && o < Cout) ? coef * d : 0.f;
+      if (ok && o < Cout && (o & (PCB - 1)) == pc) {
+        const long idx = i0 + (long)o * HW;
+        if (v_out) v_out[idx] = vv[o];
+        lsum += (double)(d * d);
+        g_out[idx] = g[o];
+      }
+    }
+#pragma unroll
+    for (int o = 0; o < MO; ++o) {
+      if (pc == 0) dbacc[o] += g[o];
+#pragma unroll
+      for (int k = 0; k < 8; ++k) dwacc[o][k] = fmaf(g[o], a[k], dwacc[o][k]);
+    }
+  };
+  for (int p0 = (int)blockIdx.x * PPB; p0 < np; p0 += 2 * stride) {
+    step(sa, p0);
+    if (p0 + stride < np) step(sb, p0 + stride);
+  }
+#pragma unroll
+  for (int o = 0; o < MO; ++o) {
+#pragma unroll
+    for (int k = 0; k < 8; ++k) fold[tid][o * 8 + k] = dwacc[o][k];
+    if (pc == 0) dbf[slot][o] = dbacc[o];
+  }
+  lred[tid] = lsum;
+  __syncthreads();
+  const int nout = Cout * (C + 1);
+  for (int id = tid; id < nout; id += 256) {
+    const int o = id / (C + 1), c = id - o * (C + 1);
+    float t = 0.f;
+    if (c < C) {
+      const int cp = c >> 3, k = c & 7;
+      for (int sl = 0; sl < PPB; ++sl) t += fold[sl * PCB + cp][o * 8 + k];
+    } else {
+      for (int sl = 0; sl < PPB; ++sl) t += dbf[sl][o];
+    }
+    part[(long)blockIdx.x * nout + id] = t;
+  }
+  for (int o = 128; o > 0; o >>= 1) {
+    if (tid < o) lred[tid] += lred[tid + o];
+    __syncthreads();
+  }
+  if (tid == 0) lpart[blockIdx.x] = lred[0];
+}
+
+template <typename T, int PCB, int MO>
+__global__ __launch_bounds__(256) void tail_bwd_apply_kernel(const T* __restrict__ raw, int ldx,
+                                                             const float* __restrict__ g_nchw, const float* __restrict__ w,
+                                                             const float* __restrict__ scale, const float* __restrict__ shift,
+                                                             const float* __restrict__ mean, const float* __restrict__ invstd,
+                                                             const float* __restrict__ gamma, const float* __restrict__ c1,
+                                                             const float* __restrict__ c2, T* __restrict__ dx, int lddx,
+                                                             long npix, int HW, int Cout) {
+  constexpr int C = PCB * 8, PPB = 256 / PCB;
+  const int tid = threadIdx.x, pc = tid & (PCB - 1), slot = tid / PCB;
+  float wr[MO][8];
+#pragma unroll
+  for (int o = 0; o < MO; ++o)
+#pragma unroll
+    for (int k = 0; k < 8; ++k) wr[o][k] = o < Cout ? w[o * C + pc * 8 + k] : 0.f;
+  float ga[8], k1[8], k2[8], mu[8], is[8], sc[8], sh[8];
+#pragma unroll
+  for (int k = 0; k < 8; ++k) {
+    const int c = pc * 8 + k;
+    mu[k] = mean[c]; is[k] = invstd[c]; sc[k] = scale[c]; sh[k] = shift[c];
+    ga[k] = gamma[c] * is[k]; k1[k] = c1[c]; k2[k] = c2[c];
+  }
+  const int np = (int)npix, stride = (int)gridDim.x * PPB;
+  const int first = (int)blockIdx.x * PPB + slot;
+  const int nit = first < np ? (np - first + stride - 1) / stride : 0;
+  f32x8 r_next;
+  float g_next[MO];
+  auto fetch = [&](int p) {
+    r_next = load8(raw + (long)p * ldx + pc * 8);
+    const int n = p / HW, q = p - n * HW;
+#pragma unroll
+    for (int o = 0; o < MO; ++o) g_next[o] = o < Cout ? g_nchw[((long)n * Cout + o) * HW + q] : 0.f;
+  };
+  if (nit > 0) fetch(first + (nit - 1) * stride);
+  for (int it = nit - 1; it >= 0; --it) {
+    const int p = first + it * stride;
+    const f32x8 r = r_next;
+    float g[MO];
+#pragma unroll
+    for (int o = 0; o < MO; ++o) g[o] = g_next[o];
+    if (it > 0) fetch(p - stride);
+    f32x8 out;
+#pragma unroll
+    for (int k = 0; k < 8; ++k) {
+      float t = 0.f;
+#pragma unroll
+      for (int o = 0; o < MO; ++o) t = fmaf(g[o], wr[o][k], t);
+      const float da = to_f32(from_f32<T>(t));
+      const float dz = fmaf(r.v[k], sc[k], sh[k]) > 0.f ? da : 0.f;
+      out.v[k] = ga[k] * (dz - k1[k] - ((r.v[k] - mu[k]) * is[k]) * k2[k]);
+    }
+    store8(dx + (long)p * lddx + pc * 8, out);
+  }
 }
 
 __global__ __launch_bounds__(256) void loss_finalize_kernel(const double* part, int n, double inv_count, float* loss) {
@@ -822,3 +1018,94 @@
   S2S_LAUNCH_CHECK();
   return S2S_OK;
 }
+
+int s2s_internal_tail_bn_sums(int dtype, const void* raw, int ldx, const float* g_nchw, const float* w, const float* scale,
+                              const float* shift, const float* mean, const float* invstd, float* work, float* dgamma,
+                              float* dbeta, float* zero_out, int accumulate, int B, int H, int W, int C, int Cout,
+                              hipStream_t s);
+extern "C" int s2s_bn_bwd_blocks(int B, int H, int W, int C);
+
+namespace {
+inline bool tail_shape_ok(int B, int H, int W, int C, int Cout, int ldx) {
+  if (B <= 0 || H <= 0 || W <= 0 || C < 8 || (C % 8) || (ldx % 8) || Cout <= 0 || Cout > HEAD_MAX_COUT) return false;
+  const int pcb = C / 8;
+  if (pcb > 64 || (pcb & (pcb - 1))) return false;
+  return (long)B * H * W < (1L << 31) - (1L << 20);
+}
+}
+
+extern "C" int s2s_tail_blocks(int B, int H, int W) { return s2s_head_loss_blocks(B, H, W); }
+
+extern "C" int s2s_tail_fwd_loss(int dtype, const void* raw, int ldx, const float* scale, const float* shift,
+                                 const float* mean, const float* invstd, const float* w, const float* bias,
+                                 const float* u_nchw, float* v_nchw, float* g_nchw, float grad_scale, float* part,
+                                 double* lpart, float* bnwork, float* dw, float* dbias, float* loss, float* dgamma,
+                                 float* dbeta, float* conv_dbias, int accumulate, int B, int H, int W, int C, int Cout,
+                                 void* stream) {
+  if (!raw || !scale || !shift || !mean || !invstd || !w || !u_nchw || !g_nchw || !part || !lpart || !bnwork || !dw ||
+      !loss || !dgamma || !dbeta)
+    return S2S_ERR_NULL;
+  if (!tail_shape_ok(B, H, W, C, Cout, ldx)) return S2S_ERR_SHAPE;
+  if (dtype != S2S_BF16 && dtype != S2S_F32) return S2S_ERR_DTYPE;
+  const long npix = (long)B * H * W;
+  const double count = (double)npix * Cout;
+  const int nb = s2s_tail_blocks(B, H, W);
+  hipStream_t s = (hipStream_t)stream;
+  const float coef = (float)(2.0 * (double)grad_scale / count);
+#define S2S_TA(TT, PP)                                                                                               \
+  if (Cout <= 3)                                                                                                     \
+    hipLaunchKernelGGL((tail_fwd_loss_kernel<TT, PP, 3>), dim3(nb), dim3(256), 0, s, (const TT*)raw, ldx, scale,     \
+                       shift, w, bias, u_nchw, v_nchw, g_nchw, coef, part, lpart, npix, H * W, Cout);                \
+  else                                                                                                               \
+  hipLaunchKernelGGL((tail_fwd_loss_kernel<TT, PP, HEAD_MAX_COUT>), dim3(nb), dim3(256), 0, s, (const TT*)raw, ldx, scale, shift,   \
+                     w, bias, u_nchw, v_nchw, g_nchw, coef, part, lpart, npix, H * W, Cout);
+#define S2S_TA_T(TT)                                                                                    \
+  switch (C / 8) {                                                                                      \
+    case 1: { S2S_TA(TT, 1) } break;  case 2: { S2S_TA(TT, 2) } break;  case 4: { S2S_TA(TT, 4) } break;    \
+    case 8: { S2S_TA(TT, 8) } break;  case 16: { S2S_TA(TT, 16) } break; case 32: { S2S_TA(TT, 32) } break;  \
+    default: { S2S_TA(TT, 64) } break;                                                                  \
+  }
+  if (dtype == S2S_BF16) { S2S_TA_T(bf16_t) } else { S2S_TA_T(float) }
+#undef S2S_TA_T
+#undef S2S_TA
+  hipLaunchKernelGGL(head_wgrad_reduce_kernel, dim3(cdiv(Cout * (C + 1), 8)), dim3(256), 0, s, part, nb, Cout, C,
+                     dw, dbias, accumulate);
+  hipLaunchKernelGGL(loss_finalize_kernel, dim3(1), dim3(256), 0, s, lpart, nb, 1.0 / count, loss);
+  if (int rc = s2s_internal_tail_bn_sums(dtype, raw, ldx, g_nchw, w, scale, shift, mean, invstd, bnwork, dgamma, dbeta,
+                                         (conv_dbias && !accumulate) ? conv_dbias : nullptr, accumulate, B, H, W, C,
+                                         Cout, s))
+    return rc;
+  S2S_LAUNCH_CHECK();
+  return S2S_OK;
+}
+
+extern "C" int s2s_tail_bwd_apply(int dtype, const void* raw, int ldx, const float* g_nchw, const float* w,
+                                  const float* scale, const float* shift, const float* mean, const float* invstd,
+                                  const float* gamma, const float* bnwork, void* dx, int lddx, int B, int H, int W,
+                                  int C, int Cout, void* stream) {
+  if (!raw || !g_nchw || !w || !scale || !shift || !mean || !invstd || !gamma || !bnwork || !dx) return S2S_ERR_NULL;
+  if (!tail_shape_ok(B, H, W, C, Cout, ldx) || (lddx % 8) || lddx < C) return S2S_ERR_SHAPE;
+  if (dtype != S2S_BF16 && dtype != S2S_F32) return S2S_ERR_DTYPE;
+  const long npix = (long)B * H * W;
+  const int nb = s2s_tail_blocks(B, H, W);
+  const float* const c1 = bnwork + (long)2 * C * s2s_bn_bwd_blocks(B, H, W, C);
+  hipStream_t s = (hipStream_t)stream;
+#define S2S_TB(TT, PP)                                                                                              \
+  if (Cout <= 3)                                                                                                    \
+    hipLaunchKernelGGL((tail_bwd_apply_kernel<TT, PP, 3>), dim3(nb), dim3(256), 0, s, (const TT*)raw, ldx, g_nchw,  \
+                       w, scale, shift, mean, invstd, gamma, c1, c1 + C, (TT*)dx, lddx, npix, H * W, Cout);         \
+  else                                                                                                              \
+  hipLaunchKernelGGL((tail_bwd_apply_kernel<TT, PP, HEAD_MAX_COUT>), dim3(nb), dim3(256), 0, s, (const TT*)raw, ldx, g_nchw, w,    \
+                     scale, shift, mean, invstd, gamma, c1, c1 + C, (TT*)dx, lddx, npix, H * W, Cout);
+#define S2S_TB_T(TT)                                                                                    \
+  switch (C / 8) {                                                                                      \
+    case 1: { S2S_TB(TT, 1) } break;  case 2: { S2S_TB(TT, 2) } break;  case 4: { S2S_TB(TT, 4) } break;    \
+    case 8: { S2S_TB(TT, 8) } break;  case 16: { S2S_TB(TT, 16) } break; case 32: { S2S_TB(TT, 32) } break;  \
+    default: { S2S_TB(TT, 64) } break;                                                                  \
+  }
+  if (dtype == S2S_BF16) { S2S_TB_T(bf16_t) } else { S2S_TB_T(float) }
+#undef S2S_TB_T
+#undef S2S_TB
+  S2S_LAUNCH_CHECK();
+  return S2S_OK;
+}
diff --git a/stain2stain_amd/csrc/norm_act.hip b/stain2stain_amd/csrc/norm_act.hip
--- a/stain2stain_amd/csrc/norm_act.hip
+++ b/stain2stain_amd/csrc/norm_act.hip
@@ -412,6 +412,61 @@
 #pragma unroll
       for (int k = 0; k < 8; ++k) {
         const float dz = fmaf(b.v[k], sc[k], sh[k]) > 0.f ? g.v[k] : 0.f;
+        s1[k] += (Acc)dz;
+        s2[k] += (Acc)(dz * ((b.v[k] - mu[k]) * is[k]));
+      }
+    }
+  }
+  __shared__ Acc red[2][2304];
+  const int rowlen = PCB * 8 + 1;
+#pragma unroll
+  for (int k = 0; k < 8; ++k) { red[0][wl * rowlen + pc * 8 + k] = s1[k]; red[1][wl * rowlen + pc * 8 + k] = s2[k]; }
+  __syncthreads();
+  for (int i = threadIdx.x; i < 2 * PCB * 8; i += 256) {
+    const int which = i / (PCB * 8), cl = i - which * (PCB * 8);
+    Acc s = 0;
+    for (int r = 0; r < WL; ++r) s += red[which][r * rowlen + cl];
+    const int c = blockIdx.x * PCB * 8 + cl;
+    if (c < C) part[((long)which * C + c) * gridDim.y + blockIdx.y] = (float)s;
+  }
+}
+
+template <typename T>
+__global__ __launch_bounds__(256) void bn_relu_bwd_reduce_tail_kernel(const float* __restrict__ g_nchw, const float* __restrict__ w, int Cout, int HW,
+                                               const float* __restrict__ scale, const float* __restrict__ shift,
+                                               const T* __restrict__ x, int ldx, const float* mean, const float* invstd,
+                                               float* part, long npix, int C) {
+  const int PCB = pcb_of(C), WL = 256 / PCB;
+  const int pc = threadIdx.x & (PCB - 1), wl = threadIdx.x / PCB;
+  const int c8 = (blockIdx.x * PCB + pc) * 8;
+  using Acc = typename std::conditional<std::is_same<T, float>::value, double, float>::type;
+  Acc s1[8], s2[8];
+#pragma unroll
+  for (int k = 0; k < 8; ++k) { s1[k] = 0; s2[k] = 0; }
+  if (c8 < C) {
+    float mu[8], is[8], sc[8], sh[8], wr[4][8];
+#pragma unroll
+    for (int k = 0; k < 8; ++k) { mu[k] = mean[c8 + k]; is[k] = invstd[c8 + k]; sc[k] = scale[c8 + k]; sh[k] = shift[c8 + k]; }
+#pragma unroll
+    for (int o = 0; o < 4; ++o)
+#pragma unroll
+      for (int k = 0; k < 8; ++k) wr[o][k] = o < Cout ? w[o * C + c8 + k] : 0.f;
+    for (long p = (long)blockIdx.y * WL + wl; p < npix; p += (long)gridDim.y * WL) {
+      const int pi = (int)p, n = pi / HW, q = pi - n * HW;
+      float gv[4];
+#pragma unroll
+      for (int o = 0; o < 4; ++o) {
+        const float t = g_nchw[((long)n * Cout + (o < Cout ? o : Cout - 1)) * HW + q];
+        gv[o] = o < Cout ? t : 0.f;
+      }
+      const f32x8 b = load8(x + p * ldx + c8);
+#pragma unroll
+      for (int k = 0; k < 8; ++k) {
+        float t = 0.f;
+#pragma unroll
+        for (int o = 0; o < 4; ++o) t = fmaf(gv[o], wr[o][k], t);
+        const float gk = to_f32(from_f32<T>(t));
+        const float dz = fmaf(b.v[k], sc[k], sh[k]) > 0.f ? gk : 0.f;
         s1[k] += (Acc)dz;
         s2[k] += (Acc)(dz * ((b.v[k] - mu[k]) * is[k]));
       }
@@ -666,6 +721,30 @@
   return S2S_OK;
 }
 
+int s2s_internal_tail_bn_sums(int dtype, const void* raw, int ldx, const float* g_nchw, const float* w, const float* scale,
+                              const float* shift, const float* mean, const float* invstd, float* work, float* dgamma,
+                              float* dbeta, float* zero_out, int accumulate, int B, int H, int W, int C, int Cout,
+                              hipStream_t s) {
+  const int nb = red_blocks(B, H, W, C);
+  float* const c1 = work + (long)2 * C * nb;
+  const long npix = (long)B * H * W;
+  dim3 grid(cdiv(C / 8, host_pcb(C)), nb);
+  if (dtype == S2S_BF16)
+    hipLaunchKernelGGL(bn_relu_bwd_reduce_tail_kernel<bf16_t>, grid, dim3(256), 0, s, g_nchw, w, Cout, H * W, scale, shift,
+                       (const bf16_t*)raw, ldx, mean, invstd, work, npix, C);
+  else if (dtype == S2S_F32)
+    hipLaunchKernelGGL(bn_relu_bwd_reduce_tail_kernel<float>, grid, dim3(256), 0, s, g_nchw, w, Cout, H * W, scale, shift,
+                       (const float*)raw, ldx, mean, invstd, work, npix, C);
+  else return S2S_ERR_DTYPE;
+  if (finalize_tpc(nb) == 256)
+    hipLaunchKernelGGL(bn_bwd_finalize_kernel<256>, dim3(C), dim3(256), 0, s, work, nb, C, (double)npix, dgamma, dbeta,
+                       accumulate, c1, c1 + C, zero_out);
+  else
+    hipLaunchKernelGGL(bn_bwd_finalize_kernel<64>, dim3(cdiv(C, 4)), dim3(256), 0, s, work, nb, C, (double)npix, dgamma,
+                       dbeta, accumulate, c1, c1 + C, zero_out);
+  return S2S_OK;
+}
+
 extern "C" int s2s_bn_relu_bwd(int dtype, const void* g1, int ldg1, const void* gp, int ldgp, const float* scale,
                                const float* shift, const void* x, int ldx, const float* mean, const float* invstd, const float* gamma,
                                float* dgamma, float* dbeta, float* dbias_conv, int accumulate, void* dx, int lddx,
diff --git a/stain2stain_amd/engine.py b/stain2stain_amd/engine.py
--- a/stain2stain_amd/engine.py
+++ b/stain2stain_amd/engine.py
@@ -185,7 +185,7 @@
     x0: Optional[torch.Tensor]
     x1: Optional[torch.Tensor]
     raw: torch.Tensor
-    act: torch.Tensor
+    act: Optional[torch.Tensor]
     stats: torch.Tensor
     count: Optional[int] = None
     sync: Optional["SyncBNExchange"] = None
@@ -211,6 +211,7 @@
     skips: List[torch.Tensor] = field(default_factory=list)
     layers: List[Tuple[LayerCtx, LayerCtx]] = field(default_factory=list)
     v: torch.Tensor = None
+    tail: Optional[Tuple[torch.Tensor, torch.Tensor]] = None
 
 
 def _stem_as_conv(x_nchw: torch.Tensor, dtype: torch.dtype) -> bool:
@@ -222,37 +223,43 @@
     return ops.p2p_pack_input(x_nchw, None, torch.empty((B, H, W, 8), dtype=dtype, device=x_nchw.device))
 
 
-def _conv_bn_relu(cb: ConvBN, x0, x1, dtype, training: bool, want_pool: bool = False, stem: bool = False):
+def _conv_bn_stats(cb: ConvBN, x0, x1, dtype, stem: bool = False):
     bn = cb.bn
     bias = cb.conv.bias.detach() if cb.conv.bias is not None else None
+    late_bias = None
+    if stem and _stem_as_conv(x0, dtype):
+        raw, stat = ops.conv3x3(_stem_image(x0, dtype), None, cb.packed(dtype)[0], None, cb.cout, want_stats=True)
+        late_bias = bias
+    elif stem:
+        raw, stat = ops.stem_fwd(x0, cb.conv.weight.detach(), bias, dtype, want_stats=True)
+    elif dtype == torch.bfloat16 and bias is not None:
+        raw, stat = ops.conv3x3(x0, x1, cb.packed(dtype)[0], None, cb.cout, want_stats=True)
+        late_bias = bias
+    else:
+        raw, stat = ops.conv3x3(x0, x1, cb.packed(dtype)[0], bias, cb.cout, want_stats=True)
+    count = raw.shape[0] * raw.shape[1] * raw.shape[2]
+    sx = sync_bn if sync_bn is not None else _module_exchange(bn)
+    if sx is not None:
+        sums = ops.bn_partial_sums(stat)
+        sx(sums)
+        stat = sums.view(2, -1, 1)
+        count *= sx.world
+    if count <= 1:
+        raise ValueError(f"Expected more than 1 value per channel when training, got input size "
+                         f"{[raw.shape[0], raw.shape[3], raw.shape[1], raw.shape[2]]}")
+    track = bn.track_running_stats and bn.running_mean is not None
+    mutation_epoch[0] += 1
+    st = ops.bn_finalize(stat, count, bn.weight.detach(), bn.bias.detach(),
+                         bn.running_mean if track else None, bn.running_var if track else None,
+                         bn.num_batches_tracked if track else None,
+                         BN_MOMENTUM if bn.momentum is None else bn.momentum, bn.eps, conv_bias=late_bias)
+    return raw, st, count, sx
+
+
+def _conv_bn_relu(cb: ConvBN, x0, x1, dtype, training: bool, want_pool: bool = False, stem: bool = False):
+    bias = cb.conv.bias.detach() if cb.conv.bias is not None else None
     if training:
-        late_bias = None
-        if stem and _stem_as_conv(x0, dtype):
-            raw, stat = ops.conv3x3(_stem_image(x0, dtype), None, cb.packed(dtype)[0], None, cb.cout, want_stats=True)
-            late_bias = bias
-        elif stem:
-            raw, stat = ops.stem_fwd(x0, cb.conv.weight.detach(), bias, dtype, want_stats=True)
-        elif dtype == torch.bfloat16 and bias is not None:
-            raw, stat = ops.conv3x3(x0, x1, cb.packed(dtype)[0], None, cb.cout, want_stats=True)
-            late_bias = bias
-        else:
-            raw, stat = ops.conv3x3(x0, x1, cb.packed(dtype)[0], bias, cb.cout, want_stats=True)
-        count = raw.shape[0] * raw.shape[1] * raw.shape[2]
-        sx = sync_bn if sync_bn is not None else _module_exchange(bn)
-        if sx is not None:
-            sums = ops.bn_partial_sums(stat)
-            sx(sums)
-            stat = sums.view(2, -1, 1)
-            count *= sx.world
-        if count <= 1:
-            raise ValueError(f"Expected more than 1 value per channel when training, got input size "
-                             f"{[raw.shape[0], raw.shape[3], raw.shape[1], raw.shape[2]]}")
-        track = bn.track_running_stats and bn.running_mean is not None
-        mutation_epoch[0] += 1
-        st = ops.bn_finalize(stat, count, bn.weight.detach(), bn.bias.detach(),
-                             bn.running_mean if track else None, bn.running_var if track else None,
-                             bn.num_batches_tracked if track else None,
-                             BN_MOMENTUM if bn.momentum is None else bn.momentum, bn.eps, conv_bias=late_bias)
+        raw, st, count, sx = _conv_bn_stats(cb, x0, x1, dtype, stem)
         act, pooled = ops.bn_relu_apply(raw, st[2], st[3], want_pool=want_pool)
         return LayerCtx(x0, x1, raw, act, st, count if sx is not None else None, sx), act, pooled
     ss = cb.eval_affine()
@@ -337,6 +344,39 @@
     return dx
 
 
+def _conv_bn_tail(cb: ConvBN, x0, dtype):
+    raw, st, count, sx = _conv_bn_stats(cb, x0, None, dtype)
+    if sx is not None:
+        act, _ = ops.bn_relu_apply(raw, st[2], st[3])
+        return LayerCtx(x0, None, raw, act, st, count, sx), act
+    return LayerCtx(x0, None, raw, None, st), None
+
+
+def decoder_tail_loss(dec, ctx: DecCtx, u_nchw: torch.Tensor, grads: Dict[str, torch.Tensor], want_v: bool = False,
+                      accumulate: bool = False):
+    cb = dec.up_blocks[-1][1]
+    lc = ctx.layers[-1][1]
+    p = cb.prefix
+    i_conv, i_bn = cb.idx
+    loss, g, v, work = ops.tail_fwd_loss(
+        lc.raw, lc.stats, dec.outc.weight.detach(), dec.outc.bias.detach() if dec.outc.bias is not None else None,
+        u_nchw, _g(grads, "outc.weight"), _g(grads, "outc.bias") if dec.outc.bias is not None else None,
+        _g(grads, f"{p}.{i_bn}.weight"), _g(grads, f"{p}.{i_bn}.bias"),
+        _g(grads, f"{p}.{i_conv}.bias") if cb.conv.bias is not None else None, want_v=want_v, accumulate=accumulate)
+    ctx.tail = (g, work)
+    ctx.v = v
+    return loss, v
+
+
+def _conv_bn_tail_bwd(dec, cb: ConvBN, lc: LayerCtx, tail, grads, accumulate: bool):
+    g, work = tail
+    draw = ops.tail_bwd_apply(lc.raw, lc.stats, dec.outc.weight.detach(), g, cb.bn.weight.detach(), work)
+    dw = _g(grads, f"{cb.prefix}.{cb.idx[0]}.weight")
+    run_on_side(lambda: ops.conv3x3_wgrad(draw, lc.x0, lc.x1, dw, accumulate), (draw,))
+    dx, _ = ops.conv3x3(draw, None, cb.packed(draw.dtype)[1], None, cb.cin)
+    return dx
+
+
 def encoder_forward(blocks: Sequence[Tuple[ConvBN, ConvBN]], x_nchw: torch.Tensor, dtype: torch.dtype,
                     training: bool) -> EncCtx:
     ctx = EncCtx(dtype, x_nchw)
@@ -372,7 +412,9 @@
 
 
 def decoder_forward(dec, bottleneck: torch.Tensor, skips: Sequence[torch.Tensor], t_emb: torch.Tensor,
-                    dtype: torch.dtype, training: bool, with_head: bool = True) -> DecCtx:
+                    dtype: torch.dtype, training: bool, with_head: bool = True, fuse_tail: bool = False) -> DecCtx:
+    fuse_tail = (fuse_tail and training and not with_head and len(dec.up_blocks) > 0
+                 and ops.tail_fusable(dec.up_blocks[-1][1].cout, dec.outc.weight.shape[0]))
     ctx = DecCtx(dtype, t_emb)
     repack_stale([cb for pair in dec.up_blocks for cb in pair], dtype)
     tbias = None
@@ -388,7 +430,10 @@
         up = torch.empty((B, Hs, Ws, x.shape[3]), dtype=dtype, device=x.device)
         ops.upsample2x_fwd(x, up, tbias if i == 0 else None)
         lc1, a1, _ = _conv_bn_relu(c1, skip, up, dtype, training)
-        lc2, a2, _ = _conv_bn_relu(c2, a1, None, dtype, training)
+        if fuse_tail and i == len(dec.up_blocks) - 1:
+            lc2, a2 = _conv_bn_tail(c2, a1, dtype)
+        else:
+            lc2, a2, _ = _conv_bn_relu(c2, a1, None, dtype, training)
         ctx.lows.append(x); ctx.ups.append(up); ctx.skips.append(skip); ctx.layers.append((lc1, lc2))
         x = a2
     ctx.lows.append(x)
@@ -401,7 +446,9 @@
 def decoder_backward(dec, ctx: DecCtx, dv: Optional[torch.Tensor], grads: Dict[str, torch.Tensor],
                      accumulate: bool = False, need_dt_emb: bool = False, on_group_done=None,
                      g_head: Optional[torch.Tensor] = None):
-    if g_head is not None:
+    if ctx.tail is not None:
+        g = None
+    elif g_head is not None:
         g = g_head
     else:
         g = ops.head_bwd(dv, ctx.lows[-1], dec.outc.weight.detach(), _g(grads, "outc.weight"),
@@ -413,7 +460,10 @@
     for i in range(len(ctx.layers) - 1, -1, -1):
         c1, c2 = dec.up_blocks[i]
         lc1, lc2 = ctx.layers[i]
-        ga1 = _conv_bn_relu_bwd(c2, lc2, g, None, grads, accumulate, need_dx=True)
+        if ctx.tail is not None and i == nup - 1:
+            ga1 = _conv_bn_tail_bwd(dec, c2, lc2, ctx.tail, grads, accumulate)
+        else:
+            ga1 = _conv_bn_relu_bwd(c2, lc2, g, None, grads, accumulate, need_dx=True)
         if on_group_done is not None:
             on_group_done()
         dcat = _conv_bn_relu_bwd(c1, lc1, ga1, None, grads, accumulate, need_dx=True)
diff --git a/stain2stain_amd/multitask_trainer.py b/stain2stain_amd/multitask_trainer.py
--- a/stain2stain_amd/multitask_trainer.py
+++ b/stain2stain_amd/multitask_trainer.py
@@ -74,6 +74,7 @@
                                            + list(seg_decoder.up_blocks), self._dtype)
         self._side = ops.side_stream_for(dev)
         self.overlap_wgrad = True
+        self.fuse_tail = True
         self._group = 0
         self._eval_owner = object()
         self._generation = evaluation.GenerationEval()
@@ -104,15 +105,20 @@
         ectx1 = engine.encoder_forward(enc._blocks, xt, dt, True)
         temb = ops.time_embedding(t, self.time_emb_dim)
         f1 = ectx1.feats
-        dctx_f = engine.decoder_forward(fdec, f1[-1], f1[:-1][::-1], temb, dt, True, with_head=False)
+        dctx_f = engine.decoder_forward(fdec, f1[-1], f1[:-1][::-1], temb, dt, True, with_head=False,
+                                        fuse_tail=self.fuse_tail and not want_outputs)
         ectx2 = engine.encoder_forward(enc._blocks, x0, dt, True)
         f2 = ectx2.feats
         dctx_s = engine.decoder_forward(sdec, f2[-1], f2[:-1][::-1], None, dt, True)
         logits = dctx_s.v
-        flow, g_head, v = ops.head_loss_fused(dctx_f.lows[-1], fdec.outc.weight.detach(),
-                                              fdec.outc.bias.detach() if fdec.outc.bias is not None else None, ut,
-                                              self.grads_flow["outc.weight"], self.grads_flow.get("outc.bias"),
-                                              want_v=want_outputs)
+        if dctx_f.lows[-1] is None:
+            g_head = None
+            flow, v = engine.decoder_tail_loss(fdec, dctx_f, ut, self.grads_flow, want_v=want_outputs)
+        else:
+            flow, g_head, v = ops.head_loss_fused(dctx_f.lows[-1], fdec.outc.weight.detach(),
+                                                  fdec.outc.bias.detach() if fdec.outc.bias is not None else None, ut,
+                                                  self.grads_flow["outc.weight"], self.grads_flow.get("outc.bias"),
+                                                  want_v=want_outputs)
         w = float(self.seg_loss_weight)
         if self.num_classes is not None:
             tgt = mask[:, 0] if (mask.dim() == 4 and mask.shape[1] == 1) else mask
diff --git a/stain2stain_amd/ops.py b/stain2stain_amd/ops.py
--- a/stain2stain_amd/ops.py
+++ b/stain2stain_amd/ops.py
@@ -395,6 +395,54 @@
     return loss, dx, v
 
 
+def tail_fusable(C: int, cout: int) -> bool:
+    pcb = C // 8
+    return C % 8 == 0 and 1 <= pcb <= 64 and pcb & (pcb - 1) == 0 and 1 <= cout <= 4
+
+
+@_timed("tail_fwd_loss")
+def tail_fwd_loss(raw: torch.Tensor, stats: torch.Tensor, w: torch.Tensor, bias: Optional[torch.Tensor],
+                  u_nchw: torch.Tensor, dw: torch.Tensor, dbias: Optional[torch.Tensor], dgamma: torch.Tensor,
+                  dbeta: torch.Tensor, dbias_conv: Optional[torch.Tensor], want_v: bool = False,
+                  grad_scale: float = 1.0, accumulate: bool = False):
+    B, H, W, C = raw.shape
+    cout = w.shape[0]
+    if not tail_fusable(C, cout):
+        raise RuntimeError(f"stain2stain_amd: the fused tail does not take C = {C}, cout = {cout}")
+    px, ldx = _nhwc(raw)
+    dev = raw.device
+    g = torch.empty((B, cout, H, W), dtype=torch.float32, device=dev)
+    v = torch.empty((B, cout, H, W), dtype=torch.float32, device=dev) if want_v else None
+    nb = _L().s2s_tail_blocks(B, H, W)
+    part = torch.empty((nb, cout, C + 1), dtype=torch.float32, device=dev)
+    lpart = torch.empty((nb,), dtype=torch.float64, device=dev)
+    work = torch.empty((2 * C * _L().s2s_bn_bwd_blocks(B, H, W, C) + 2 * C,), dtype=torch.float32, device=dev)
+    loss = torch.empty((), dtype=torch.float32, device=dev)
+    rc = _L().s2s_tail_fwd_loss(_dt(raw), px, ldx, stats[2].data_ptr(), stats[3].data_ptr(), stats[0].data_ptr(),
+                                stats[1].data_ptr(), _f32(w.reshape(cout, C)), _f32(bias), _f32(u_nchw), _f32(v),
+                                _f32(g), float(grad_scale), _f32(part), lpart.data_ptr(), _f32(work),
+                                _f32(dw.reshape(cout, C)), _f32(dbias), loss.data_ptr(), _f32(dgamma), _f32(dbeta),
+                                _f32(dbias_conv), int(accumulate), B, H, W, C, cout, _stream())
+    _native.check(rc, "tail_fwd_loss")
+    return loss, g, v, work
+
+
+@_timed("tail_bwd_apply")
+def tail_bwd_apply(raw: torch.Tensor, stats: torch.Tensor, w: torch.Tensor, g: torch.Tensor, gamma: torch.Tensor,
+                   work: torch.Tensor) -> torch.Tensor:
+    B, H, W, C = raw.shape
+    cout = w.shape[0]
+    px, ldx = _nhwc(raw)
+    if tuple(g.shape) != (B, cout, H, W) or work.numel() != 2 * C * _L().s2s_bn_bwd_blocks(B, H, W, C) + 2 * C:
+        raise RuntimeError("stain2stain_amd: tail_bwd_apply operands do not belong to this tail_fwd_loss")
+    dx = torch.empty((B, H, W, C), dtype=raw.dtype, device=raw.device)
+    rc = _L().s2s_tail_bwd_apply(_dt(raw), px, ldx, _f32(g), _f32(w.reshape(cout, C)), stats[2].data_ptr(),
+                                 stats[3].data_ptr(), stats[0].data_ptr(), stats[1].data_ptr(), _f32(gamma),
+                                 _f32(work), dx.data_ptr(), C, B, H, W, C, cout, _stream())
+    _native.check(rc, "tail_bwd_apply")
+    return dx
+
+
 @_timed("bn_finalize")
 def bn_finalize(stat: torch.Tensor, count: int, gamma, beta, running_mean, running_var, num_batches,
                 momentum: float = 0.1, eps: float = 1e-5, conv_bias: Optional[torch.Tensor] = None):
diff --git a/stain2stain_amd/trainer.py b/stain2stain_amd/trainer.py
--- a/stain2stain_amd/trainer.py
+++ b/stain2stain_amd/trainer.py
@@ -87,6 +87,7 @@
         self.packer = engine.Conv3x3Packer(list(net.encoder._blocks) + list(net.flow_decoder.up_blocks), self._dtype)
         self._side = ops.side_stream_for(dev)
         self.overlap_wgrad = True
+        self.fuse_tail = True
         self.graph = graph
         self._graph_step = CapturedStep()
         self._ema = None
@@ -127,12 +128,17 @@
             ectx = engine.encoder_forward(enc._blocks, xt, dt, True)
             temb = ops.time_embedding(t, net.time_embedding.dim)
             feats = ectx.feats
-            dctx = engine.decoder_forward(dec, feats[-1], feats[:-1][::-1], temb, dt, True, with_head=False)
-        loss, g_head, v = ops.head_loss_fused(dctx.lows[-1], dec.outc.weight.detach(),
-                                              dec.outc.bias.detach() if dec.outc.bias is not None else None, ut,
-                                              self.grads_dec["outc.weight"], self.grads_dec.get("outc.bias"),
-                                              want_v=want_v)
-        dctx.v = v
+            dctx = engine.decoder_forward(dec, feats[-1], feats[:-1][::-1], temb, dt, True, with_head=False,
+                                          fuse_tail=self.fuse_tail and not want_v)
+        if dctx.lows[-1] is None:
+            g_head = None
+            loss, v = engine.decoder_tail_loss(dec, dctx, ut, self.grads_dec, want_v=want_v)
+        else:
+            loss, g_head, v = ops.head_loss_fused(dctx.lows[-1], dec.outc.weight.detach(),
+                                                  dec.outc.bias.detach() if dec.outc.bias is not None else None, ut,
+                                                  self.grads_dec["outc.weight"], self.grads_dec.get("outc.bias"),
+                                                  want_v=want_v)
+            dctx.v = v
         self.bucketer.start_step()
         self._group = 0
         with engine.side_scope(self._side if self.overlap_wgrad else None):
```
